# octree-nn/octfusion

Measured on AMD Instinct MI355X. Metric: denoising-steps/sec (depth-8 octree, batch 8), higher is better.
Workload: dtype f32 storage, fp16x3 products (fp16 hi + lo operand pairs = 22 significand bits, three fp16 MFMAs per product, fp32 accumulate)

## Files before the change

include/ofx.h:

```cpp
#ifndef OFX_H_
#define OFX_H_

#include <stddef.h>
#include <stdint.h>

#ifdef __cplusplus
extern "C" {
#endif

#define OFX_OK 0
#define OFX_EINVAL (-1)
#define OFX_ELAUNCH (-2)
#define OFX_ENODEV (-3)

#define OFX_ACT_NONE 0
#define OFX_ACT_SILU 1
#define OFX_ACT_GELU 2

#define OFX_MAX_DEPTH 16

int ofx_version(void);
const char* ofx_status_string(int status);
int ofx_device_check(void);
const char* ofx_build_hash(void);
// ... 72 lines not shown
int ofx_graphconv_bwd_weight(const float* x, int64_t ldx, int cin, int64_t n_nodes, const int32_t* nbr,
                             const int32_t* seg_ptr, const int32_t* col, const int32_t* nbr_ext,
                             const int32_t* multi_seg, int64_t n_multi, float* aux, const float* type_frac, int64_t ldt,
                             int nt_pad, const float* dy, int64_t ldy, int cout, float* dWp, int64_t Kp, void* ws,
                             size_t ws_bytes, void* stream);
int ofx_gn_backward(const float* x, int64_t ldx, const float* dy, int64_t ldy, int64_t n, int C,
                    const int32_t* batch_id, int batch_size, const float* count, int groups, float count_eps,
                    const float* mean, const float* rstd, const float* w, const float* bias, int act, double* sums,
                    float* coef, float* dx, int64_t lddx, float* dgamma, float* dbeta, void* stream);
int ofx_gemm_tn_f32(const float* P, int64_t ldp, const float* Q, int64_t ldq, int64_t rows, int64_t K, int64_t N,
                    float* out, void* ws, size_t ws_bytes, void* stream);
int ofx_table_reverse_count(const int32_t* nbr, int64_t n_out, int ndir, int64_t n_in, int32_t* rev_cnt, void* stream);
int ofx_table_reverse_fill(const int32_t* nbr, int64_t n_out, int ndir, int64_t n_in, const int32_t* rev_ptr,
                           int32_t* cursor, int32_t* rev_row, float* rev_w, void* stream);
int ofx_seg_primary_w(const int32_t* seg_ptr, const int32_t* col, const float* w, int64_t nseg, int32_t* nbr,
                      void* stream);
int ofx_seg_multi_flag_w(const int32_t* seg_ptr, const float* w, int64_t nseg, int32_t* flag, void* stream);
int ofx_seg_primary_ext_w(const int32_t* seg_ptr, const int32_t* col, const float* w, int64_t nseg, int64_t n_src,
                          const int32_t* rank, int32_t* nbr_ext, int32_t* multi_seg, void* stream);
int ofx_gridconv_bwd_data(const float* dy, int64_t ldy, int cout, int64_t n_out, int64_t n_in, const int32_t* nbr_rev,
                          const int32_t* rev_ptr, const int32_t* rev_row, const float* rev_w,
                          const int32_t* nbr_ext_rev, const int32_t* multi_seg, int64_t n_multi, float* aux,
                          const float* WpT, int cin, float* dx, int64_t ldx, void* ws, size_t ws_bytes, void* stream);
int ofx_gridconv_bwd_weight(const float* x, int64_t ldx, int cin, int64_t n_in, int64_t n_out, const int32_t* nbr27,
                            const int32_t* nbr27_ext, const float* zero_row, const float* dy, int64_t ldy, int cout,
                            float* dWp, void* ws, size_t ws_bytes, void* stream);
int ofx_adamw_step(float* param, const float* grad, float* exp_avg, float* exp_avg_sq, int64_t n, float lr,
                   float beta1, float beta2, float eps, float weight_decay, int step, void* stream);
int ofx_ema_update(float* ema, const float* param, int64_t n, float beta, void* stream);
typedef struct OfxAdamRow {
  float* param;
  const float* grad;
  float* exp_avg;
  float* exp_avg_sq;
  float* ema;
  int64_t n;
} OfxAdamRow;
int ofx_adamw_ema_multi(const OfxAdamRow* rows, int64_t n_rows, float lr, float beta1, float beta2, float eps,
                        float weight_decay, int step, float ema_beta, void* stream);
int ofx_adamw_ema_multi_chunk(void);
int ofx_adamw_ema_multi_rows(void);
int64_t ofx_mse_grad_partials(int64_t n);
int ofx_mse_grad(const float* y, const float* target, float* dy, double* partials, double* loss_out, int64_t n,
                 void* stream);
int ofx_mpu_eval(const ofx_tree_t* tree, int depth_start, int depth_end, const float* pts, int64_t n_pts,
                 const float* code, float* sdf, uint8_t* mask, void* stream);
int ofx_mpu_eval_grid(const ofx_tree_t* tree, int depth_start, int depth_end, const float* code, int size,
                      float step, float bbmin, int batch_index, int64_t head, int64_t count, float* sdf,
                      uint8_t* mask, void* stream);
int ofx_mpu_eval_grad(const ofx_tree_t* tree, int depth_start, int depth_end, const float* pts, int64_t n_pts,
                      const float* code, float* sdf, float* grad, uint8_t* mask, void* stream);
int ofx_mpu_backward(const ofx_tree_t* tree, int depth_start, int depth_end, const float* pts, int64_t n_pts,
                     const float* code, const float* dsdf, const float* dgrad, float* dcode, void* stream);
int ofx_octree_ce(const float* logits, int64_t ld, const int32_t* child, int64_t n, float dscale, double* sums,
                  float* dlogits, int64_t ldd, void* stream);
int ofx_sdf_reg_loss(const float* sdf, const float* grad, const float* sdf_gt, const float* grad_gt, int64_t n,
                     float w_sdf, float w_grad, double* sums, float* dsdf, float* dgrad, void* stream);
int ofx_kl_sample_fwd(const float* params, int64_t ld, const float* noise, int64_t n, int embed_dim, float* z,
                      double* kl_sum, void* stream);
int ofx_kl_sample_bwd(const float* params, int64_t ld, const float* noise, const float* dz, int64_t n,
                      int embed_dim, float kl_scale, float* dparams, int64_t ldp, void* stream);
int ofx_graph_multi_flag(const int32_t* seg_ptr, int64_t n_nodes, int32_t* flag, void* stream);
int ofx_graph_primary_ext(const int32_t* seg_ptr, const int32_t* col, int64_t n_nodes,
                          const int32_t* rank, int32_t* nbr_ext, int32_t* multi_seg, void* stream);
int ofx_graph_type_frac(const int32_t* seg_ptr, const int32_t* col, const uint8_t* node_type,
                        int64_t n_nodes, int nt, float* type_frac, int64_t ld, void* stream);

int ofx_set_precision(int mode);
int ofx_get_precision(void);
int64_t ofx_packed_floats(int64_t Kp, int64_t N);
int64_t ofx_packed_k(int64_t K);
int64_t ofx_graphconv_packed_k(int cin, int nt);
int ofx_pack_weights(const float* W, int64_t sk, int64_t sn, int64_t K, int64_t N,
                     int cin, int nt, float* Wp, int64_t Kp, void* stream);

int ofx_gemm_f32(const float* A, int64_t lda, const int32_t* a_rows, int64_t M, int64_t K,
                 const float* Wp, int64_t Kp, int64_t N, const float* bias,
                 const float* res, int64_t ldr, float* out, int64_t ldc,
                 const int32_t* out_rows, void* ws, size_t ws_bytes, void* stream);
int ofx_gemm_f32_planes(const float* A, int64_t lda, const int32_t* a_rows, int64_t M, int64_t K,
                        const float* Wp, int64_t Kp, int64_t N, const float* bias,
                        const float* res, int64_t ldr, float* out, int64_t ldc,
                        const int32_t* out_rows, void* ws, size_t ws_bytes, int out_mode, void* stream);

int ofx_graphconv_fwd(const float* x, int64_t ldx, int cin, int64_t n_nodes,
                      const int32_t* nbr, const int32_t* seg_ptr, const int32_t* col,
                      const int32_t* nbr_ext, const int32_t* multi_seg, int64_t n_multi, float* aux,
                      const float* type_frac, int64_t ldt, int nt_pad,
                      const float* Wp, int64_t Kp, int cout, const float* bias,
                      const float* emb, int64_t lde, const int32_t* batch_id,
                      const float* res, int64_t ldr, float* out, int64_t ldc,
                      double* stats , int64_t stats_ld,
                      void* ws, size_t ws_bytes, void* stream);

int ofx_graphconv_narrow_in(const float* x, int64_t ldx, int cin, int64_t n_nodes, const int32_t* seg_ptr,
                            const int32_t* col, const uint8_t* node_type, int nt, const float* W, int cout,
                            const float* bias, const int32_t* batch_id, float* out, int64_t ldc,
                            double* stats , int64_t stats_ld, void* ws, size_t ws_bytes, void* stream);
int ofx_graphconv_narrow_in_tab(const float* x, int64_t ldx, int cin, int64_t n_nodes, const int32_t* seg_ptr,
                                const int32_t* col, const int32_t* nbr_ext, const int32_t* multi_seg, int64_t n_multi,
                                void* aux, const uint8_t* node_type, int nt, const float* W, int cout, const float* bias,
                                const int32_t* batch_id, float* out, int64_t ldc, double* stats ,
                                int64_t stats_ld, void* ws, size_t ws_bytes, void* stream);
int ofx_narrow_out_pack(const float* W, int C, int nt, int cout, int pw, float* Wd, void* stream);
int ofx_narrow_out_type_term(const float* type_frac, int64_t ldt, int nt, int64_t n_nodes, const float* W, int C,
                             int cout, const float* bias, float* type_term, void* stream);
int ofx_graphconv_narrow_out(const float* P, int64_t ldp, int cout, int64_t n_nodes, const int32_t* seg_ptr,
                             const int32_t* col, const float* type_term , float* out, int64_t ldc,
                             void* stream);

int ofx_planes_split(const float* x, int64_t ldx, int64_t n, int C, int Cpad, int mode, void* out,
                     int64_t ldo_bytes, void* stream);
int ofx_planes_merge(const void* planes, int64_t ldp_bytes, int64_t n, int C, int mode, float* out, int64_t ldo,
                     void* stream);
int ofx_gn_apply_planes(const float* x, int64_t ldx, int64_t n, int C, const int32_t* batch_id, const float* mean,
                        const float* rstd, const double* sums, const float* count, int groups, float eps,
                        float count_eps, const float* w, const float* bias, int act, int mode, void* out,
                        int64_t ldo_bytes, const int32_t* seg_ptr, const int32_t* col, const int32_t* multi_seg,
                        int64_t n_multi, void* aux , const int32_t* aux_plan ,
                        int64_t aux_left, void* stream);
int ofx_gn_apply_planes_oct(const float* x, int64_t ldx, int64_t n, int C, const int32_t* batch_id, const float* mean,
                            const float* rstd, const double* sums, const float* count, int groups, float eps,
                            float count_eps, const float* w, const float* bias, int act, int mode, void* out,
                            int64_t ldo_bytes, int64_t n_multi, void* aux, const int32_t* oct_ptr,
                            const int32_t* oct_ent, int64_t n_own, int shift, const int32_t* left_head,
                            const int32_t* left_src, int64_t n_left, void* stream);
int ofx_gn_finalize_window(const double* sums, const float* count, int batch_size, int C, int groups, int c_lo,
                           int c_hi, float eps, float count_eps, float* mean, float* rstd, void* stream);
int ofx_gn_apply_planes_window(const float* x, int64_t ldx, int64_t n, int C, int c_lo, int c_hi,
                               const int32_t* batch_id, const float* mean, const float* rstd, const double* sums,
                               const float* count, int groups, float eps, float count_eps, const float* w,
                               const float* bias, int act, int mode, void* out, int64_t ldo_bytes,
                               const int32_t* seg_ptr, const int32_t* col, const int32_t* multi_seg, int64_t n_multi,
                               void* aux, const int32_t* aux_plan, int64_t aux_left, void* stream);
int ofx_gn_apply_planes_oct_window(const float* x, int64_t ldx, int64_t n, int C, int c_lo, int c_hi,
                                   const int32_t* batch_id, const float* mean, const float* rstd, const double* sums,
                                   const float* count, int groups, float eps, float count_eps, const float* w,
                                   const float* bias, int act, int mode, void* out, int64_t ldo_bytes, int64_t n_multi,
                                   void* aux, const int32_t* oct_ptr, const int32_t* oct_ent, int64_t n_own, int shift,
                                   const int32_t* left_head, const int32_t* left_src, int64_t n_left, void* stream);
int ofx_gn_apply_rows(void);
int64_t ofx_planes_packed_ktiles(int cin, int nt, int mode);
int64_t ofx_planes_packed_bytes(int cin, int nt, int cout, int mode);
int ofx_pack_weights_planes(const float* W, int64_t sk, int64_t sn, int cin, int nt, int cout, int mode, void* out,
                            void* stream);
int ofx_graphconv_fwd_planes(const void* xp, int64_t ldx_bytes, int cin, int64_t n_nodes, const int32_t* seg_ptr,
                             const int32_t* col, const int32_t* nbr_ext, const int32_t* multi_seg, int64_t n_multi,
                             void* aux, size_t aux_bytes, const void* tfp, int64_t ldt_bytes, int nt, const void* W2,
                             int cout, const float* bias, const float* emb, int64_t lde, const int32_t* batch_id,
                             const float* res, int64_t ldr, float* out, int64_t ldc, double* stats ,
                             int64_t stats_ld, void* ws, size_t ws_bytes, void* sync , size_t sync_bytes,
                             int mode, int aux_ready, void* stream);
int ofx_graphconv_fwd_planes_cus(const void* xp, int64_t ldx_bytes, int cin, int64_t n_nodes, const int32_t* seg_ptr,
                                 const int32_t* col, const int32_t* nbr_ext, const int32_t* multi_seg, int64_t n_multi,
                                 void* aux, size_t aux_bytes, const void* tfp, int64_t ldt_bytes, int nt,
                                 const void* W2, int cout, const float* bias, const float* emb, int64_t lde,
                                 const int32_t* batch_id, const float* res, int64_t ldr, float* out, int64_t ldc,
                                 double* stats , int64_t stats_ld, void* ws, size_t ws_bytes,
                                 void* sync , size_t sync_bytes, int mode, int aux_ready, int cus,
                                 void* stream);
int ofx_set_gconv_persistent(int on);
int64_t ofx_gemm_planes_packed_bytes(int K, int N, int mode);
int ofx_pack_gemm_planes(const float* W, int64_t sk, int64_t sn, int K, int N, int mode, void* out, void* stream);
int ofx_gemm_planes(const void* ap, int64_t lda_bytes, int64_t n_a, int64_t M, int K, const int32_t* row_tab,
                    const void* W2, int N, const float* bias, float* out, int64_t ldc, int out_mode, void* ws,
                    size_t ws_bytes, void* sync, size_t sync_bytes, int mode, void* stream);
int ofx_set_gconv_cus(int cus);
int ofx_gconv3_plan(int64_t n_rows, int cout, int nkt, int wm, int ni, int cus, int32_t* out, int64_t out_len);
int ofx_set_gconv2_tile(int wm);

int ofx_grid_conv_table(int mode, int depth_out, int batch_size, int32_t pad, int32_t* nbr27,
                        void* stream);
int64_t ofx_conv3d_packed_k(int cin);
int ofx_pack_conv3d(const float* W, int cin, int cout, float* Wp, void* stream);
int ofx_gridconv_fwd(const float* x, int64_t ldx, int cin, int64_t n_in, int64_t n_out,
                     const int32_t* nbr27 ,
                     const int32_t* nbr27_ext ,
                     const float* zero_row ,
                     const float* Wp, int cout, const float* bias, const float* emb, int64_t lde,
                     const int32_t* batch_id, const float* res, int64_t ldr, float* out,
                     int64_t ldc, void* ws, size_t ws_bytes, void* stream);
int ofx_gather_gemm_f32(const float* x, int64_t ldx, int cin, int ntap, int64_t n_src, int64_t n_out, const int32_t* tab,
                        const float* zero_row, const float* Wp, int64_t Kp, int cout, const float* bias,
                        const float* res, int64_t ldr, float* out, int64_t ldc, const int32_t* out_rows, void* ws,
                        size_t ws_bytes, int out_mode, void* stream);
int ofx_set_attention_split(int on);
int ofx_attention(const float* qkv, int64_t ldq, int batch_size, int T, int heads, int ch,
                  float* out, int64_t ldo, void* stream);

int ofx_attention_bwd(const float* qkv, int64_t ldq, const float* dout, int64_t ldo, int batch_size, int T, int heads,
                      int ch, float* rowstat, float* dqkv, int64_t ldd, void* stream);

int ofx_gather_mean(const float* x, int64_t ldx, int cin, int64_t n_nodes,
                    const int32_t* seg_ptr, const int32_t* col, float* col_data,
                    void* stream);

int ofx_gn_stats(const float* x, int64_t ldx, int64_t n, int C, const int32_t* batch_id,
                 int batch_size, double* sums, void* stream);
int ofx_gn_stats_acc(const float* x, int64_t ldx, int64_t n, int C, const int32_t* batch_id, int batch_size,
                     double* sums, void* stream);
int ofx_gn_finalize(const double* sums, const float* count, int batch_size, int C, int groups,
                    float eps, float count_eps, float* mean, float* rstd, void* stream);
int ofx_gn_apply(const float* x, int64_t ldx, int64_t n, int C, const int32_t* batch_id,
                 const float* mean , const float* rstd , const double* sums ,
                 const float* count, int groups, float eps, float count_eps, const float* w, const float* bias,
                 int act, float* out, int64_t ldo, void* stream);

int ofx_gn_fused_rows(const float* x, int64_t ldx, int rows_per_batch, int batch_size, int C, int groups, float eps,
                      float count_eps, const float* w, const float* bias, int act, float* out, int64_t ldo,
                      void* stream);

int ofx_set_gn_rows16(int on);

int ofx_rows_copy(const float* src, int64_t lds, const int32_t* smap, float* dst, int64_t ldd,
                  const int32_t* dmap, int64_t n, int C, void* stream);
int ofx_rows_copy_planes(const float* src, int64_t lds, const int32_t* smap, float* dst, int64_t ldd,
                         const int32_t* dmap, int64_t n, int C, int mode, void* stream);
int ofx_act(const float* x, float* y, int64_t n, int act, void* stream);
int ofx_timestep_embedding(const float* t, int batch_size, int dim, float max_period,
                           float* out, void* stream);
int ofx_learned_sinusoid(const float* t, const float* w, int batch_size, int half, float* out, void* stream);
int ofx_linear_small(const float* a, int64_t lda, int M, int K, const float* W, int64_t ldw, int N, const float* bias,
                     const float* res, int64_t ldr, int act_in, int act_out, float* out, int64_t ldo, void* stream);
int ofx_ddim_eps_update(float* x, const float* eps, const float* coef, float* x0_out, int64_t n,
                        void* stream);
int ofx_ddim_x0_update(float* x, const float* x0, const float* noise, const float* coef,
                       int64_t n, void* stream);

size_t ofx_mc_ws_bytes(int batch, int size);
int ofx_mc_count(const float* sdf, int batch, int size, float level, void* ws, int64_t* counts, void* stream);
int ofx_mc_emit(const float* sdf, int batch, int size, float level, float step, float bbmin, float scale, void* ws,
                const int64_t* vert_off, const int64_t* tri_off, float* verts, int32_t* faces, void* stream);
int ofx_mc_table_host(int8_t* tri_table, uint8_t* ntri);

size_t ofx_fieldmesh_classify_ws_bytes(int batch, int size);
size_t ofx_fieldmesh_ws_bytes(int64_t n_bricks);
int ofx_fieldmesh_classify(const ofx_tree_t* tree, int depth_end, int batch0, int batch, int size, float step,
                           float bbmin, int margin, void* cws, int64_t* counts, void* stream);
int ofx_fieldmesh_count(const ofx_tree_t* tree, int depth_start, int depth_end, const float* code, int batch0,
                        int batch, int size, float step, float bbmin, float level, const void* cws, int64_t n_bricks,
                        void* ws, int64_t* counts, void* stream);
int ofx_fieldmesh_emit(int batch, int size, float level, float step, float bbmin, float scale, const void* cws,
                       int64_t n_bricks, void* ws, const int64_t* vert_off, const int64_t* tri_off, float* verts,
                       int32_t* faces, void* stream);

size_t ofx_mesh_cc_ws_bytes(int64_t total_verts, int64_t total_faces, int batch);
int ofx_mesh_cc_label(const int32_t* faces, const int64_t* vert_off, const int64_t* tri_off, int batch,
                      int64_t total_verts, int64_t total_faces, int32_t* label, void* ws, int32_t* status,
                      void* stream);
int ofx_mesh_cc_table(const int32_t* faces, const int32_t* label, const int64_t* vert_off, const int64_t* tri_off,
                      int batch, int64_t total_verts, int64_t total_faces, int32_t* comp_of_vert, int32_t* comp_off,
                      void* ws, const int32_t* status, void* stream);
int ofx_mesh_cc_stats(const float* verts, const int32_t* faces, const int32_t* label, const int64_t* vert_off,
                      const int64_t* tri_off, int batch, int64_t total_verts, int64_t total_faces, int64_t n_comp,
                      int32_t* table, void* ws, const int32_t* status, void* stream);
int ofx_mesh_cc_select(const float* verts, const int32_t* faces, const int32_t* label, const int64_t* vert_off,
                       const int64_t* tri_off, int batch, int64_t total_verts, int64_t total_faces,
                       int32_t* winner_label, int64_t* keep_counts, void* ws, const int32_t* status, void* stream);
int ofx_mesh_cc_extract(const float* verts, const int32_t* faces, const int64_t* vert_off, const int64_t* tri_off,
                        int batch, int64_t total_verts, int64_t total_faces, const int64_t* new_vert_off,
                        const int64_t* new_tri_off, float* out_verts, int32_t* out_faces, void* ws,
                        const int32_t* status, void* stream);

int ofx_simplify_stages(void);
size_t ofx_simplify_ws_bytes(int64_t total_verts, int64_t total_faces, int batch);
int ofx_simplify_cluster(const float* verts, const int32_t* faces, const int64_t* vert_off, const int64_t* tri_off,
                         int batch, int64_t total_verts, int64_t total_faces, int cells, double cell_size, double reg,
                         int stages, int64_t* counts, void* ws, int32_t* status, void* stream);
// ... 103 lines not shown
```

octfusion_amd/_lib.py:

```python
import ctypes
import os

import torch

_HERE = os.path.dirname(os.path.abspath(__file__))
LIB_PATH = os.environ.get('OFX_LIB', os.path.join(_HERE, 'libofx.so'))

c_p = ctypes.c_void_p
c_i = ctypes.c_int
c_l = ctypes.c_int64
c_f = ctypes.c_float
c_d = ctypes.c_double
c_sz = ctypes.c_size_t
c_u64 = ctypes.c_uint64


class OfxTree(ctypes.Structure):
    _fields_ = [('depth', c_i), ('full_depth', c_i), ('batch_size', c_i),
                ('child_all', c_p), ('key_all', c_p), ('leafrank_all', c_p),
                ('nnum_host', c_p), ('nnum_nempty_host', c_p)]


class OfxAdamRow(ctypes.Structure):
    _fields_ = [('param', c_p), ('grad', c_p), ('exp_avg', c_p), ('exp_avg_sq', c_p), ('ema', c_p), ('n', c_l)]


_SIGS = {
    'ofx_version': (c_i, [], False),
    'ofx_status_string': (ctypes.c_char_p, [c_i], False),
    'ofx_device_check': (c_i, [], False),
    'ofx_build_hash': (ctypes.c_char_p, [], False),
    'ofx_probe_mfma_sustained': (c_i, [c_i, c_i, c_p, c_p, c_p], True),
    'ofx_scan_ws_bytes': (c_sz, [c_l], False),
    'ofx_scan_i32': (c_i, [c_p, c_p, c_l, c_p, c_p], True),
    'ofx_octree_full_layer': (c_i, [c_i, c_i, c_p, c_p, c_p], True),
    'ofx_octree_split': (c_i, [c_p, c_l, c_p, c_p, c_p, c_p], True),
    'ofx_octree_grow': (c_i, [c_p, c_p, c_l, c_p, c_p, c_p], True),
    'ofx_split_small_label0': (c_i, [c_p, c_i, c_i, c_p, c_p], True),
    'ofx_split_small_label1': (c_i, [c_p, c_i, c_i, c_p, c_p, c_p], True),
    'ofx_split_large_label0': (c_i, [c_p, c_l, c_p, c_p], True),
    'ofx_split_large_label1': (c_i, [c_p, c_l, c_p, c_p, c_p], True),
    'ofx_octree2voxel_cf': (c_i, [c_p, c_l, c_i, c_i, c_i, c_p, c_p], True),
    'ofx_voxel2octree_cf': (c_i, [c_p, c_i, c_i, c_i, c_p, c_l, c_p], True),
    'ofx_points_sort_ws_bytes': (c_sz, [c_l], False),
    'ofx_points_keys': (c_i, [c_p, c_l, c_p, c_i, c_l, c_i, c_p, c_p, c_p], True),
    'ofx_points_sort': (c_i, [c_p, c_p, c_l, c_p, c_p, c_p, c_sz, c_p], True),
    'ofx_octree_label_from_points': (c_i, [c_p, c_l, c_p, c_l, c_i, c_i, c_p, c_p], True),
    'ofx_octree_point_features': (c_i, [c_p, c_p, c_l, c_p, c_l, c_p, c_l, c_p, c_l, c_i, c_p, c_p, c_p, c_p], True),
    'ofx_tree_leafrank_ws_bytes': (c_sz, [c_l], False),
    'ofx_tree_leafrank': (c_i, [c_p, c_p, c_i, c_p, c_p, c_p], True),
    'ofx_graph_nodes': (c_i, [ctypes.POINTER(OfxTree), c_i, c_p, c_p, c_p, c_p, c_p], True),
    'ofx_graph_count': (c_i, [ctypes.POINTER(OfxTree), c_i, c_p, c_p], True),
    'ofx_graph_reverse_count': (c_i, [c_p, c_p, c_l, c_p, c_p], True),
    'ofx_graph_reverse_fill': (c_i, [c_p, c_p, c_l, c_p, c_p, c_p, c_p, c_p], True),
    'ofx_graph_primary_w': (c_i, [c_p, c_p, c_p, c_l, c_p, c_p], True),
    'ofx_graph_multi_flag_w': (c_i, [c_p, c_p, c_l, c_p, c_p], True),
    'ofx_graph_primary_ext_w': (c_i, [c_p, c_p, c_p, c_l, c_p, c_p, c_p, c_p], True),
    'ofx_graphconv_bwd_data': (c_i, [c_p, c_l, c_i, c_l, c_p, c_p, c_p, c_p, c_p, c_p, c_l, c_p, c_p, c_l, c_i, c_p,
                                     c_l, c_p, c_sz, c_p], True),
    'ofx_graphconv_bwd_weight': (c_i, [c_p, c_l, c_i, c_l, c_p, c_p, c_p, c_p, c_p, c_l, c_p, c_p, c_l, c_i, c_p, c_l,
                                       c_i, c_p, c_l, c_p, c_sz, c_p], True),
    'ofx_gn_backward': (c_i, [c_p, c_l, c_p, c_l, c_l, c_i, c_p, c_i, c_p, c_i, c_f, c_p, c_p, c_p, c_p, c_i, c_p, c_p,
                              c_p, c_l, c_p, c_p, c_p], True),
    'ofx_gemm_tn_f32': (c_i, [c_p, c_l, c_p, c_l, c_l, c_l, c_l, c_p, c_p, c_sz, c_p], True),
    'ofx_table_reverse_count': (c_i, [c_p, c_l, c_i, c_l, c_p, c_p], True),
    'ofx_table_reverse_fill': (c_i, [c_p, c_l, c_i, c_l, c_p, c_p, c_p, c_p, c_p], True),
    'ofx_seg_primary_w': (c_i, [c_p, c_p, c_p, c_l, c_p, c_p], True),
    'ofx_seg_multi_flag_w': (c_i, [c_p, c_p, c_l, c_p, c_p], True),
    'ofx_seg_primary_ext_w': (c_i, [c_p, c_p, c_p, c_l, c_l, c_p, c_p, c_p, c_p], True),
    'ofx_gridconv_bwd_data': (c_i, [c_p, c_l, c_i, c_l, c_l, c_p, c_p, c_p, c_p, c_p, c_p, c_l, c_p, c_p, c_i, c_p, c_l,
                                    c_p, c_sz, c_p], True),
    'ofx_gridconv_bwd_weight': (c_i, [c_p, c_l, c_i, c_l, c_l, c_p, c_p, c_p, c_p, c_l, c_i, c_p, c_p, c_sz, c_p], True),
    'ofx_attention_bwd': (c_i, [c_p, c_l, c_p, c_l, c_i, c_i, c_i, c_i, c_p, c_p, c_l, c_p], True),
    'ofx_adamw_step': (c_i, [c_p, c_p, c_p, c_p, c_l, c_f, c_f, c_f, c_f, c_f, c_i, c_p], True),
    'ofx_ema_update': (c_i, [c_p, c_p, c_l, c_f, c_p], True),
    'ofx_adamw_ema_multi': (c_i, [c_p, c_l, c_f, c_f, c_f, c_f, c_f, c_i, c_f, c_p], True),
    'ofx_adamw_ema_multi_chunk': (c_i, [], False),
    'ofx_adamw_ema_multi_rows': (c_i, [], False),
    'ofx_mse_grad_partials': (c_l, [c_l], False),
    'ofx_mse_grad': (c_i, [c_p, c_p, c_p, c_p, c_p, c_l, c_p], True),
    'ofx_gn_fused_rows': (c_i, [c_p, c_l, c_i, c_i, c_i, c_i, c_f, c_f, c_p, c_p, c_i, c_p, c_l, c_p], True),
    'ofx_set_gn_rows16': (c_i, [c_i], True),
    'ofx_mpu_eval': (c_i, [ctypes.POINTER(OfxTree), c_i, c_i, c_p, c_l, c_p, c_p, c_p, c_p], True),
    'ofx_mpu_eval_grid': (c_i, [ctypes.POINTER(OfxTree), c_i, c_i, c_p, c_i, c_f, c_f, c_i, c_l, c_l, c_p, c_p, c_p], True),
    'ofx_mpu_eval_grad': (c_i, [ctypes.POINTER(OfxTree), c_i, c_i, c_p, c_l, c_p, c_p, c_p, c_p, c_p], True),
    'ofx_mpu_backward': (c_i, [ctypes.POINTER(OfxTree), c_i, c_i, c_p, c_l, c_p, c_p, c_p, c_p, c_p], True),
    'ofx_octree_ce': (c_i, [c_p, c_l, c_p, c_l, c_f, c_p, c_p, c_l, c_p], True),
    'ofx_sdf_reg_loss': (c_i, [c_p, c_p, c_p, c_p, c_l, c_f, c_f, c_p, c_p, c_p, c_p], True),
    'ofx_kl_sample_fwd': (c_i, [c_p, c_l, c_p, c_l, c_i, c_p, c_p, c_p], True),
    'ofx_kl_sample_bwd': (c_i, [c_p, c_l, c_p, c_p, c_l, c_i, c_f, c_p, c_l, c_p], True),
    'ofx_graph_fill': (c_i, [ctypes.POINTER(OfxTree), c_i, c_p, c_p, c_p], True),
    'ofx_graph_expand': (c_i, [c_p, c_l, c_p, c_p, c_p, c_p, c_p], True),
    'ofx_graph_type_frac': (c_i, [c_p, c_p, c_p, c_l, c_i, c_p, c_l, c_p], True),
    'ofx_set_precision': (c_i, [c_i], True),
    'ofx_set_range_words': (c_i, [c_p], True),
    'ofx_get_precision': (c_i, [], False),
    'ofx_gn_apply_rows': (c_i, [], False),
    'ofx_set_attention_split': (c_i, [c_i], True),
    'ofx_gather_gemm_f32': (c_i, [c_p, c_l, c_i, c_i, c_l, c_l, c_p, c_p, c_p, c_l, c_i, c_p, c_p, c_l, c_p, c_l, c_p, c_p, c_sz, c_i, c_p], True),
    'ofx_graphconv_narrow_in_tab': (c_i, [c_p, c_l, c_i, c_l, c_p, c_p, c_p, c_p, c_l, c_p, c_p, c_i, c_p, c_i, c_p, c_p, c_p, c_l, c_p, c_l,
                                          c_p, c_sz, c_p], True),
    'ofx_graphconv_narrow_in': (c_i, [c_p, c_l, c_i, c_l, c_p, c_p, c_p, c_i, c_p, c_i, c_p, c_p, c_p, c_l, c_p, c_l, c_p, c_sz, c_p], True),
    'ofx_narrow_out_pack': (c_i, [c_p, c_i, c_i, c_i, c_i, c_p, c_p], True),
    'ofx_narrow_out_type_term': (c_i, [c_p, c_l, c_i, c_l, c_p, c_i, c_i, c_p, c_p, c_p], True),
    'ofx_graphconv_narrow_out': (c_i, [c_p, c_l, c_i, c_l, c_p, c_p, c_p, c_p, c_l, c_p], True),
    'ofx_packed_floats': (c_l, [c_l, c_l], False),
    'ofx_packed_k': (c_l, [c_l], False),
    'ofx_graphconv_packed_k': (c_l, [c_i, c_i], False),
    'ofx_pack_weights': (c_i, [c_p, c_l, c_l, c_l, c_l, c_i, c_i, c_p, c_l, c_p], True),
    'ofx_gemm_f32': (c_i, [c_p, c_l, c_p, c_l, c_l, c_p, c_l, c_l, c_p, c_p, c_l, c_p, c_l, c_p, c_p, c_sz, c_p], True),
    'ofx_gemm_f32_planes': (c_i, [c_p, c_l, c_p, c_l, c_l, c_p, c_l, c_l, c_p, c_p, c_l, c_p, c_l, c_p, c_p, c_sz, c_i, c_p], True),
    'ofx_graphconv_fwd': (c_i, [c_p, c_l, c_i, c_l, c_p, c_p, c_p, c_p, c_p, c_l, c_p, c_p, c_l, c_i, c_p, c_l,
                                c_i, c_p, c_p, c_l, c_p, c_p, c_l, c_p, c_l, c_p, c_l, c_p, c_sz, c_p], True),
    'ofx_planes_split': (c_i, [c_p, c_l, c_l, c_i, c_i, c_i, c_p, c_l, c_p], True),
    'ofx_planes_merge': (c_i, [c_p, c_l, c_l, c_i, c_i, c_p, c_l, c_p], True),
    'ofx_gn_apply_planes': (c_i, [c_p, c_l, c_l, c_i, c_p, c_p, c_p, c_p, c_p, c_i, c_f, c_f, c_p, c_p, c_i, c_i, c_p,
                                  c_l, c_p, c_p, c_p, c_l, c_p, c_p, c_l, c_p], True),
    'ofx_gn_apply_planes_oct': (c_i, [c_p, c_l, c_l, c_i, c_p, c_p, c_p, c_p, c_p, c_i, c_f, c_f, c_p, c_p, c_i, c_i, c_p,
                                      c_l, c_l, c_p, c_p, c_p, c_l, c_i, c_p, c_p, c_l, c_p], True),
    'ofx_planes_packed_ktiles': (c_l, [c_i, c_i, c_i], False),
    'ofx_planes_packed_bytes': (c_l, [c_i, c_i, c_i, c_i], False),
    'ofx_pack_weights_planes': (c_i, [c_p, c_l, c_l, c_i, c_i, c_i, c_i, c_p, c_p], True),
    'ofx_graphconv_fwd_planes': (c_i, [c_p, c_l, c_i, c_l, c_p, c_p, c_p, c_p, c_l, c_p, c_sz, c_p, c_l, c_i, c_p, c_i,
                                       c_p, c_p, c_l, c_p, c_p, c_l, c_p, c_l, c_p, c_l, c_p, c_sz, c_p, c_sz, c_i, c_i,
                                       c_p], True),
    'ofx_graphconv_fwd_planes_cus': (c_i, [c_p, c_l, c_i, c_l, c_p, c_p, c_p, c_p, c_l, c_p, c_sz, c_p, c_l, c_i, c_p,
                                           c_i, c_p, c_p, c_l, c_p, c_p, c_l, c_p, c_l, c_p, c_l, c_p, c_sz, c_p, c_sz,
                                           c_i, c_i, c_i, c_p], True),
    'ofx_gn_finalize_window': (c_i, [c_p, c_p, c_i, c_i, c_i, c_i, c_i, c_f, c_f, c_p, c_p, c_p], True),
    'ofx_gn_apply_planes_window': (c_i, [c_p, c_l, c_l, c_i, c_i, c_i, c_p, c_p, c_p, c_p, c_p, c_i, c_f, c_f, c_p, c_p,
                                         c_i, c_i, c_p, c_l, c_p, c_p, c_p, c_l, c_p, c_p, c_l, c_p], True),
    'ofx_gn_apply_planes_oct_window': (c_i, [c_p, c_l, c_l, c_i, c_i, c_i, c_p, c_p, c_p, c_p, c_p, c_i, c_f, c_f, c_p,
                                             c_p, c_i, c_i, c_p, c_l, c_l, c_p, c_p, c_p, c_l, c_i, c_p, c_p, c_l, c_p],
                                       True),
    'ofx_set_gconv_persistent': (c_i, [c_i], True),
    'ofx_set_gconv_cus': (c_i, [c_i], True),
    'ofx_gemm_planes_packed_bytes': (c_l, [c_i, c_i, c_i], False),
    'ofx_pack_gemm_planes': (c_i, [c_p, c_l, c_l, c_i, c_i, c_i, c_p, c_p], True),
    'ofx_gemm_planes': (c_i, [c_p, c_l, c_l, c_l, c_i, c_p, c_p, c_i, c_p, c_p, c_l, c_i, c_p, c_sz, c_p, c_sz, c_i, c_p], False),
    'ofx_gconv3_plan': (c_i, [c_l, c_i, c_i, c_i, c_i, c_i, c_p, c_l], False),
    'ofx_set_gconv2_tile': (c_i, [c_i], True),
    'ofx_graph_multi_flag': (c_i, [c_p, c_l, c_p, c_p], True),
    'ofx_graph_primary_ext': (c_i, [c_p, c_p, c_l, c_p, c_p, c_p, c_p], True),
    'ofx_graph_primary': (c_i, [c_p, c_p, c_l, c_p, c_p], True),
    'ofx_grid_conv_table': (c_i, [c_i, c_i, c_i, c_i, c_p, c_p], True),
    'ofx_conv3d_packed_k': (c_l, [c_i], False),
    'ofx_pack_conv3d': (c_i, [c_p, c_i, c_i, c_p, c_p], True),
    'ofx_gridconv_fwd': (c_i, [c_p, c_l, c_i, c_l, c_l, c_p, c_p, c_p, c_p, c_i, c_p, c_p, c_l, c_p, c_p, c_l, c_p,
                               c_l, c_p, c_sz, c_p], True),
    'ofx_attention': (c_i, [c_p, c_l, c_i, c_i, c_i, c_i, c_p, c_l, c_p], True),
    'ofx_gather_mean': (c_i, [c_p, c_l, c_i, c_l, c_p, c_p, c_p, c_p], True),
    'ofx_gn_stats': (c_i, [c_p, c_l, c_l, c_i, c_p, c_i, c_p, c_p], True),
    'ofx_gn_stats_acc': (c_i, [c_p, c_l, c_l, c_i, c_p, c_i, c_p, c_p], True),
    'ofx_gn_finalize': (c_i, [c_p, c_p, c_i, c_i, c_i, c_f, c_f, c_p, c_p, c_p], True),
    'ofx_gn_apply': (c_i, [c_p, c_l, c_l, c_i, c_p, c_p, c_p, c_p, c_p, c_i, c_f, c_f, c_p, c_p, c_i, c_p, c_l, c_p], True),
    'ofx_rows_copy': (c_i, [c_p, c_l, c_p, c_p, c_l, c_p, c_l, c_i, c_p], True),
    'ofx_rows_copy_planes': (c_i, [c_p, c_l, c_p, c_p, c_l, c_p, c_l, c_i, c_i, c_p], True),
    'ofx_act': (c_i, [c_p, c_p, c_l, c_i, c_p], True),
    'ofx_timestep_embedding': (c_i, [c_p, c_i, c_i, c_f, c_p, c_p], True),
    'ofx_learned_sinusoid': (c_i, [c_p, c_p, c_i, c_i, c_p, c_p], True),
    'ofx_linear_small': (c_i, [c_p, c_l, c_i, c_i, c_p, c_l, c_i, c_p, c_p, c_l, c_i, c_i, c_p, c_l, c_p], True),
    'ofx_ddim_eps_update': (c_i, [c_p, c_p, c_p, c_p, c_l, c_p], True),
    'ofx_ddim_x0_update': (c_i, [c_p, c_p, c_p, c_p, c_l, c_p], True),
    'ofx_mc_ws_bytes': (c_sz, [c_i, c_i], False),
    'ofx_mc_count': (c_i, [c_p, c_i, c_i, c_f, c_p, c_p, c_p], True),
    'ofx_mc_emit': (c_i, [c_p, c_i, c_i, c_f, c_f, c_f, c_f, c_p, c_p, c_p, c_p, c_p, c_p], True),
    'ofx_mc_table_host': (c_i, [c_p, c_p], True),
    'ofx_fieldmesh_classify_ws_bytes': (c_sz, [c_i, c_i], False),
    'ofx_fieldmesh_ws_bytes': (c_sz, [c_l], False),
    'ofx_fieldmesh_classify': (c_i, [ctypes.POINTER(OfxTree), c_i, c_i, c_i, c_i, c_f, c_f, c_i, c_p, c_p, c_p], True),
    'ofx_fieldmesh_count': (c_i, [ctypes.POINTER(OfxTree), c_i, c_i, c_p, c_i, c_i, c_i, c_f, c_f, c_f, c_p, c_l, c_p,
                                  c_p, c_p], True),
    'ofx_fieldmesh_emit': (c_i, [c_i, c_i, c_f, c_f, c_f, c_f, c_p, c_l, c_p, c_p, c_p, c_p, c_p, c_p], True),
    'ofx_mesh_cc_ws_bytes': (c_sz, [c_l, c_l, c_i], False),
    'ofx_mesh_cc_label': (c_i, [c_p, c_p, c_p, c_i, c_l, c_l, c_p, c_p, c_p, c_p], True),
    'ofx_mesh_cc_table': (c_i, [c_p, c_p, c_p, c_p, c_i, c_l, c_l, c_p, c_p, c_p, c_p, c_p], True),
    'ofx_mesh_cc_stats': (c_i, [c_p, c_p, c_p, c_p, c_p, c_i, c_l, c_l, c_l, c_p, c_p, c_p, c_p], True),
    'ofx_mesh_cc_select': (c_i, [c_p, c_p, c_p, c_p, c_p, c_i, c_l, c_l, c_p, c_p, c_p, c_p, c_p], True),
    'ofx_mesh_cc_extract': (c_i, [c_p, c_p, c_p, c_p, c_i, c_l, c_l, c_p, c_p, c_p, c_p, c_p, c_p, c_p], True),
    'ofx_simplify_stages': (c_i, [], False),
    'ofx_simplify_ws_bytes': (c_sz, [c_l, c_l, c_i], False),
    'ofx_simplify_cluster': (c_i, [c_p, c_p, c_p, c_p, c_i, c_l, c_l, c_i, c_d, c_d, c_i, c_p, c_p, c_p, c_p], True),
    'ofx_simplify_extract': (c_i, [c_p, c_p, c_p, c_i, c_l, c_l, c_p, c_p, c_p, c_p, c_p, c_p, c_p], True),
    'ofx_voxmesh_ws_bytes': (c_sz, [c_i, c_i, c_i], False),
    'ofx_voxmesh_mask_keys': (c_i, [c_p, c_l, c_i, c_i, c_i, c_p, c_p], True),
    'ofx_voxmesh_mask_dense': (c_i, [c_p, c_i, c_i, c_f, c_p, c_p], True),
    'ofx_voxmesh_count': (c_i, [c_i, c_i, c_i, c_p, c_p, c_p], True),
    'ofx_voxmesh_emit': (c_i, [c_i, c_i, c_i, c_p, c_p, c_p, c_p, c_p, c_p], True),
    'ofx_surface_sample_ws_bytes':(c_sz, [c_i, c_l], False),
    'ofx_surface_sample': (c_i, [c_p, c_p, c_p, c_p, c_i, c_l, c_i, c_u64, c_i, c_p, c_p, c_p], True),
    'ofx_surface_sample_oriented': (c_i, [c_p, c_p, c_p, c_p, c_i, c_l, c_i, c_u64, c_i, c_p, c_p, c_p, c_p], True),
    'ofx_nn_matrix': (c_i, [c_p, c_l, c_i, c_p, c_l, c_i, c_p, c_p], True),
    'ofx_emd_matrix': (c_i, [c_p, c_l, c_p, c_l, c_i, c_i, c_p, c_p], True),
    'ofx_metrics_hash': (c_u64, [c_u64, c_l, c_l, c_i], False),
    'ofx_nn_search_qpass': (c_i, [], False),
    'ofx_nn_search_tile': (c_i, [], False),
    'ofx_nn_search_splits': (c_i, [c_i, c_l, c_l], False),
    'ofx_nn_search_ws_bytes': (c_sz, [c_l], False),
    'ofx_nn_search': (c_i, [c_p, c_p, c_p, c_p, c_i, c_l, c_l, c_l, c_i, c_p, c_p, c_p, c_p], True),
    'ofx_knn_cells': (c_i, [c_l], False),
    'ofx_knn_ws_bytes': (c_sz, [c_i, c_l, c_l, c_i], False),
    'ofx_knn': (c_i, [c_p, c_p, c_i, c_l, c_l, c_i, c_i, c_p, c_p, c_p, c_p], True),
    'ofx_pca_normals': (c_i, [c_p, c_p, c_p, c_i, c_l, c_l, c_i, c_p, c_p, c_p, c_p], True),
    'ofx_orient_normals_ws_bytes': (c_sz, [c_i, c_l, c_i], False),
    'ofx_orient_normals': (c_i, [c_p, c_p, c_p, c_p, c_i, c_l, c_l, c_i, c_p, c_p, c_p, c_i, c_i, c_i, c_p, c_p, c_p,
                                 c_p, c_p], True),
    'ofx_sdf_sample_ws_bytes': (c_sz, [c_l, c_i], False),
    'ofx_sdf_sample_nodes': (c_i, [c_p, c_i, c_p, c_l, c_p, c_i, c_i, c_i, c_u64, c_l, c_p, c_f, c_p, c_p, c_p, c_p, c_p,
                                   c_p], True),
    'ofx_sdf_sample_occu': (c_i, [c_p, c_i, c_l, c_u64, c_l, c_p, c_f, c_p, c_p, c_p], True),
    'ofx_mesh_sdf_ws_bytes': (c_sz, [c_i, c_l, c_l, c_i], False),
# ... 124 lines not shown
```

octfusion_amd/csrc/ofx_gemm.hip:

```cpp
#include "ofx_gemm_common.h"

constexpr int BM = 128;
constexpr int BK = 32;
constexpr int A_LD = BK + 4;
constexpr int MODE_DENSE = 0;
constexpr int MODE_GATHER = 1;

struct TileCoords { int split, tm, tn; };
__device__ __forceinline__ TileCoords tile_coords(const GemmArgs& g) {
  const int ntile = g.ntm * g.ntn;
  int bid = ofx_xcd_swizzle(blockIdx.x, ntile * g.nsplit);
  const int split = bid / ntile;
  bid -= split * ntile;
  const int tm = bid / g.ntn;
  return {split, tm, bid - tm * g.ntn};
}

__device__ __forceinline__ void load_a_dense(const GemmArgs& g, int64_t m0, int64_t k0, float4 (&va)[4]) {
  const int c4 = threadIdx.x & 7, r0 = threadIdx.x >> 3;
  const int64_t k = k0 + c4 * 4;
  const bool vec = ((g.lda & 3) == 0) && (k + 3 < g.K) && ((((uintptr_t)g.A) & 15) == 0);
#pragma unroll
  for (int i = 0; i < 4; ++i) {
    const int64_t m = m0 + r0 + 32 * i;
    float4 v = f4zero();
    if (m < g.M) {
      const int64_t ar = g.a_rows ? (int64_t)g.a_rows[m] : m;
      const float* p = g.A + ar * g.lda + k;
      if (vec) {
        v = *reinterpret_cast<const float4*>(p);
      } else {
        if (k + 0 < g.K) v.x = p[0];
        if (k + 1 < g.K) v.y = p[1];
        if (k + 2 < g.K) v.z = p[2];
        if (k + 3 < g.K) v.w = p[3];
      }
    }
    va[i] = v;
  }
}

template <int BN>
__device__ __forceinline__ void load_b_tile(const GemmArgs& g, int64_t n0, int64_t k0, float4 (&vb)[BN / 32]) {
#pragma unroll
  for (int i = 0; i < BN / 32; ++i) {
    const int idx = threadIdx.x + 256 * i;
    const int kql = idx / BN, n = idx % BN;
    const int64_t nn = n0 + n;
    vb[i] = (nn < g.N) ? *reinterpret_cast<const float4*>(g.Wp + (((k0 >> 2) + kql) * g.N + nn) * 4) : f4zero();
  }
}

template <int WM, int WN, int MI, int NI>
__global__ void __launch_bounds__(256, 2) gemm_dense_generic_kernel(const GemmArgs g) {
  constexpr int BN = WN * NI * 32;
  static_assert(WM * MI * 32 == BM, "BM");
  extern __shared__ __attribute__((aligned(16))) float smem[];
  float* As = smem;
  float* Bs = smem + 2 * BM * A_LD;

  const TileCoords tc = tile_coords(g);
  const int split = tc.split;
  const int64_t m0 = (int64_t)tc.tm * BM, n0 = (int64_t)tc.tn * BN;

  const int lane = threadIdx.x & 63, wid = threadIdx.x >> 6;
  const int wm = wid / WN, wn = wid % WN;
  const int l31 = lane & 31, h = lane >> 5;
  const int c4 = threadIdx.x & 7, r0 = threadIdx.x >> 3;

  f32x16 acc[MI][NI];
#pragma unroll
  for (int i = 0; i < MI; ++i)
#pragma unroll
    for (int j = 0; j < NI; ++j)
#pragma unroll
      for (int r = 0; r < 16; ++r) acc[i][j][r] = 0.f;

  float4 va[4];
  float4 vb[BN / 32];
  const int nkt_all = (int)(g.Kp / BK);
  const int kt_begin = split * g.kt_per_split;
  const int kt_end = (kt_begin + g.kt_per_split < nkt_all) ? kt_begin + g.kt_per_split : nkt_all;

  auto store_tiles = [&](int buf) {
    float* a = As + buf * BM * A_LD;
#pragma unroll
    for (int i = 0; i < 4; ++i) *reinterpret_cast<float4*>(a + (r0 + 32 * i) * A_LD + c4 * 4) = va[i];
    float* b = Bs + buf * 8 * BN * 4;
#pragma unroll
    for (int i = 0; i < BN / 32; ++i) *reinterpret_cast<float4*>(b + (threadIdx.x + 256 * i) * 4) = vb[i];
  };

  if (kt_begin < kt_end) {
    load_a_dense(g, m0, (int64_t)kt_begin * BK, va);
    load_b_tile<BN>(g, n0, (int64_t)kt_begin * BK, vb);
    store_tiles(0);
  }
  __syncthreads();

  for (int kt = kt_begin; kt < kt_end; ++kt) {
    const int buf = (kt - kt_begin) & 1;
    if (kt + 1 < kt_end) {
      load_a_dense(g, m0, (int64_t)(kt + 1) * BK, va);
      load_b_tile<BN>(g, n0, (int64_t)(kt + 1) * BK, vb);
    }
    const float* a = As + buf * BM * A_LD + (wm * MI * 32 + l31) * A_LD + h * 16;
    const float* b = Bs + buf * 8 * BN * 4 + ((h * 4) * BN + wn * NI * 32 + l31) * 4;
#pragma unroll
    for (int q = 0; q < 4; ++q) {
      float4 fa[MI], fb[NI];
#pragma unroll
      for (int i = 0; i < MI; ++i) fa[i] = *reinterpret_cast<const float4*>(a + i * 32 * A_LD + q * 4);
#pragma unroll
      for (int j = 0; j < NI; ++j) fb[j] = *reinterpret_cast<const float4*>(b + (q * BN + j * 32) * 4);
#pragma unroll
      for (int i = 0; i < MI; ++i)
#pragma unroll
        for (int j = 0; j < NI; ++j) {
          acc[i][j] = __builtin_amdgcn_mfma_f32_32x32x2f32(fa[i].x, fb[j].x, acc[i][j], 0, 0, 0);
          acc[i][j] = __builtin_amdgcn_mfma_f32_32x32x2f32(fa[i].y, fb[j].y, acc[i][j], 0, 0, 0);
          acc[i][j] = __builtin_amdgcn_mfma_f32_32x32x2f32(fa[i].z, fb[j].z, acc[i][j], 0, 0, 0);
          acc[i][j] = __builtin_amdgcn_mfma_f32_32x32x2f32(fa[i].w, fb[j].w, acc[i][j], 0, 0, 0);
        }
    }
    if (kt + 1 < kt_end) store_tiles(buf ^ 1);
    __syncthreads();
  }

  epilogue_store<WM, WN, MI, NI>(g, acc, m0, n0, wm, wn, l31, h, split);
}


__device__ __forceinline__ uint64_t sgpr64(uint64_t v) {
  unsigned lo = __builtin_amdgcn_readfirstlane((unsigned)v), hi = __builtin_amdgcn_readfirstlane((unsigned)(v >> 32));
  asm volatile("" : "+s"(lo), "+s"(hi));
  return ((uint64_t)hi << 32) | lo;
}

typedef const float __attribute__((address_space(1)))* gfp;
typedef const int32_t __attribute__((address_space(1)))* gip;
__device__ __forceinline__ float4 ldg4(gfp p) {
  typedef float v4f __attribute__((ext_vector_type(4)));
  const v4f v = *reinterpret_cast<const v4f __attribute__((address_space(1)))*>(p);
  return make_float4(v.x, v.y, v.z, v.w);
}

template <int WM, int WN, int MI, int NI>
__device__ __forceinline__ void mfma_tile(const float* __restrict__ a, const float* __restrict__ b, f32x16 (&acc)[MI][NI]) {
  constexpr int BN = WN * NI * 32;
  float4 fa[2][MI], fb[2][NI];
#pragma unroll
  for (int i = 0; i < MI; ++i) fa[0][i] = *reinterpret_cast<const float4*>(a + i * 32 * A_LD);
#pragma unroll
  for (int j = 0; j < NI; ++j) fb[0][j] = *reinterpret_cast<const float4*>(b + (j * 32) * 4);
#pragma unroll
  for (int q = 0; q < 4; ++q) {
    const int cur = q & 1, nxt = cur ^ 1;
    if (q < 3) {
#pragma unroll
      for (int i = 0; i < MI; ++i) fa[nxt][i] = *reinterpret_cast<const float4*>(a + i * 32 * A_LD + (q + 1) * 4);
#pragma unroll
      for (int j = 0; j < NI; ++j) fb[nxt][j] = *reinterpret_cast<const float4*>(b + ((q + 1) * BN + j * 32) * 4);
    }
#pragma unroll
    for (int i = 0; i < MI; ++i)
#pragma unroll
      for (int j = 0; j < NI; ++j) {
        acc[i][j] = __builtin_amdgcn_mfma_f32_32x32x2f32(fa[cur][i].x, fb[cur][j].x, acc[i][j], 0, 0, 0);
        acc[i][j] = __builtin_amdgcn_mfma_f32_32x32x2f32(fa[cur][i].y, fb[cur][j].y, acc[i][j], 0, 0, 0);
        acc[i][j] = __builtin_amdgcn_mfma_f32_32x32x2f32(fa[cur][i].z, fb[cur][j].z, acc[i][j], 0, 0, 0);
        acc[i][j] = __builtin_amdgcn_mfma_f32_32x32x2f32(fa[cur][i].w, fb[cur][j].w, acc[i][j], 0, 0, 0);
      }
  }
}

__device__ __forceinline__ int64_t src_off(uint32_t id, int64_t ldx, int64_t n_src, int64_t aux_delta) {
  const int64_t i = (int64_t)(uint64_t)id;
  const int64_t mask = (n_src - 1 - i) >> 63;
  return i * ldx + (aux_delta & mask);
}

template <int MODE, int WM, int WN, int MI, int NI>
__global__ void __launch_bounds__(256, 2) gemm_fast_kernel(const GemmArgs g) {
  constexpr int BN = WN * NI * 32;
  constexpr int NB = BN / 32;
  static_assert(WM * MI * 32 == BM, "BM");
  extern __shared__ __attribute__((aligned(16))) float smem[];
  float* As = smem;
  float* Bs = smem + 2 * BM * A_LD;

  const TileCoords tc = tile_coords(g);
  const int split = tc.split;
  const int64_t m0 = (int64_t)tc.tm * BM, n0 = (int64_t)tc.tn * BN;

  const int lane = threadIdx.x & 63, wid = threadIdx.x >> 6;
  const int wm = wid / WN, wn = wid % WN;
  const int l31 = lane & 31, h = lane >> 5;
  const int c4 = threadIdx.x & 7, r0 = threadIdx.x >> 3;

  const gfp xp = (gfp)sgpr64((uint64_t)(MODE == MODE_DENSE ? g.A : g.x));
  const gfp tfp = (gfp)sgpr64((uint64_t)g.tf);
  const gfp wp = (gfp)sgpr64((uint64_t)g.Wp);
  const gip tab = (gip)sgpr64((uint64_t)g.nbr_ext);
  const int64_t ldx = (int64_t)sgpr64((uint64_t)(MODE == MODE_DENSE ? g.lda : g.ldx));
  const int64_t ldt = (int64_t)sgpr64((uint64_t)g.ldt), n_src = (int64_t)sgpr64((uint64_t)g.n_src);
  const int64_t Ncols = (int64_t)sgpr64((uint64_t)g.N);
  const int64_t aux_delta = (int64_t)sgpr64((uint64_t)((g.aux - g.x) - g.n_src * g.ldx));
  const int ndir = g.ndir;

  f32x16 acc[MI][NI];
#pragma unroll
  for (int i = 0; i < MI; ++i)
#pragma unroll
    for (int j = 0; j < NI; ++j)
#pragma unroll
      for (int r = 0; r < 16; ++r) acc[i][j][r] = 0.f;

  const int nkt_all = (int)(g.Kp / BK);
  const int kt_begin = split * g.kt_per_split;
  const int kt_end = (kt_begin + g.kt_per_split < nkt_all) ? kt_begin + g.kt_per_split : nkt_all;
  const int tpd = MODE == MODE_DENSE ? nkt_all : g.cin / BK;
  const int nkt_g = MODE == MODE_DENSE ? nkt_all : ndir * tpd;
  const int g_begin = kt_begin < nkt_g ? kt_begin : nkt_g;
  const int g_end = kt_end < nkt_g ? kt_end : nkt_g;
  const int t_begin = kt_begin > nkt_g ? kt_begin : nkt_g;

  int64_t m_0 = m0 + r0, m_1 = m_0 + 32, m_2 = m_0 + 64, m_3 = m_0 + 96;
  const int64_t mmax = g.M - 1;
  m_0 = m_0 < mmax ? m_0 : mmax; m_1 = m_1 < mmax ? m_1 : mmax;
  m_2 = m_2 < mmax ? m_2 : mmax; m_3 = m_3 < mmax ? m_3 : mmax;
  const gip t0 = tab + m_0 * ndir;
  const gip t1 = tab + m_1 * ndir;
  const gip t2 = tab + m_2 * ndir;
  const gip t3 = tab + m_3 * ndir;
  int64_t dr0 = m_0, dr1 = m_1, dr2 = m_2, dr3 = m_3;
  if (MODE == MODE_DENSE && g.a_rows) { dr0 = g.a_rows[m_0]; dr1 = g.a_rows[m_1]; dr2 = g.a_rows[m_2]; dr3 = g.a_rows[m_3]; }
  const gfp dp0 = xp + dr0 * ldx, dp1 = xp + dr1 * ldx, dp2 = xp + dr2 * ldx, dp3 = xp + dr3 * ldx;
  const int kclamp = (int)g.K - 4;
  int64_t bo0 = 0, bo1 = 0, bo2 = 0, bo3 = 0;
  {
    auto boff = [&](int i) {
      const int idx = threadIdx.x + 256 * i;
      int64_t nn = n0 + idx % BN;
      nn = nn < Ncols ? nn : Ncols - 1;
      return ((int64_t)(idx / BN) * Ncols + nn) * 4;
    };
    bo0 = boff(0);
    if (NB > 1) bo1 = boff(1);
    if (NB > 2) { bo2 = boff(2); bo3 = boff(3); }
  }
  float* const a_st = As + r0 * A_LD + c4 * 4;
  float* const b_st = Bs + threadIdx.x * 4;
  const float* const a_ld = As + (wm * MI * 32 + l31) * A_LD + h * 16;
  const float* const b_ld = Bs + ((h * 4) * BN + wn * NI * 32 + l31) * 4;

  float4 va0, va1, va2, va3, vb0, vb1, vb2, vb3;
  vb1 = vb2 = vb3 = f4zero();
  auto load_w = [&](gfp wk) {
    vb0 = ldg4(wk + bo0);
    if (NB > 1) vb1 = ldg4(wk + bo1);
    if (NB > 2) { vb2 = ldg4(wk + bo2); vb3 = ldg4(wk + bo3); }
  };
  auto stage = [&](float* as, float* bs) {
    *reinterpret_cast<float4*>(as) = va0;
    *reinterpret_cast<float4*>(as + 32 * A_LD) = va1;
    *reinterpret_cast<float4*>(as + 64 * A_LD) = va2;
    *reinterpret_cast<float4*>(as + 96 * A_LD) = va3;
    *reinterpret_cast<float4*>(bs) = vb0;
    if (NB > 1) *reinterpret_cast<float4*>(bs + 1024) = vb1;
    if (NB > 2) { *reinterpret_cast<float4*>(bs + 2048) = vb2; *reinterpret_cast<float4*>(bs + 3072) = vb3; }
  };

  if (g_begin < g_end) {
// ... 25 lines not shown
    for (int kt = g_begin; kt < g_end; ++kt) {
      const int buf = (kt - g_begin) & 1;
      const int ktn = kt + 1 < nkt_g ? kt + 1 : nkt_g - 1;
      const int dn = ktn % ndir;
      const int d2 = (kt + 2 < nkt_g ? kt + 2 : nkt_g - 1) % ndir;
      if (MODE == MODE_DENSE) {
        int cc = ktn * BK + c4 * 4;
        cc = cc < kclamp ? cc : kclamp;
        va0 = ldg4(dp0 + cc); va1 = ldg4(dp1 + cc); va2 = ldg4(dp2 + cc); va3 = ldg4(dp3 + cc);
      } else {
        ib0 = t0[d2]; ib1 = t1[d2]; ib2 = t2[d2]; ib3 = t3[d2];
        const int cc = (ktn / ndir) * BK + c4 * 4;
        va0 = ldg4(xp + src_off(ia0, ldx, n_src, aux_delta) + cc);
        va1 = ldg4(xp + src_off(ia1, ldx, n_src, aux_delta) + cc);
        va2 = ldg4(xp + src_off(ia2, ldx, n_src, aux_delta) + cc);
        va3 = ldg4(xp + src_off(ia3, ldx, n_src, aux_delta) + cc);
      }
      const int ktw = MODE == MODE_DENSE ? ktn : dn * tpd + ktn / ndir;
      load_w(wp + (int64_t)ktw * 8 * Ncols * 4);
      __builtin_amdgcn_sched_barrier(0);
      mfma_tile<WM, WN, MI, NI>(a_ld + buf * BM * A_LD, b_ld + buf * 8 * BN * 4, acc);
      __builtin_amdgcn_sched_barrier(0);
      stage(a_st + (buf ^ 1) * BM * A_LD, b_st + (buf ^ 1) * 8 * BN * 4);
      ia0 = ib0; ia1 = ib1; ia2 = ib2; ia3 = ib3;
      __syncthreads();
    }
  }

  for (int kt = t_begin; kt < kt_end; ++kt) {
    const int cc = (kt - nkt_g) * BK + c4 * 4;
    va0 = ldg4(tfp + m_0 * ldt + cc);
    va1 = ldg4(tfp + m_1 * ldt + cc);
    va2 = ldg4(tfp + m_2 * ldt + cc);
    va3 = ldg4(tfp + m_3 * ldt + cc);
    load_w(wp + (int64_t)kt * 8 * Ncols * 4);
    stage(a_st, b_st);
    __syncthreads();
    mfma_tile<WM, WN, MI, NI>(a_ld, b_ld, acc);
    __syncthreads();
  }

  epilogue_store<WM, WN, MI, NI>(g, acc, m0, n0, wm, wn, l31, h, split);
}


typedef __bf16 bf16x8_t __attribute__((ext_vector_type(8)));
typedef _Float16 f16x8h_t __attribute__((ext_vector_type(8)));
typedef unsigned u32x4h __attribute__((ext_vector_type(4)));

template <int H16>
__device__ __forceinline__ void split16x4(const float4& v, uint2& hi, uint2& lo) {
  if constexpr (H16 == 0) {
    hi.x = g2_pk_bf16(v.x, v.y);
    hi.y = g2_pk_bf16(v.z, v.w);
    const float hx = g2_bf16_lo(hi.x), hy = g2_bf16_hi(hi.x);
    const float hz = g2_bf16_lo(hi.y), hw = g2_bf16_hi(hi.y);
    lo.x = g2_pk_bf16(v.x - hx, v.y - hy);
    lo.y = g2_pk_bf16(v.z - hz, v.w - hw);
  } else {
    hi.x = g2_pk_f16(v.x, v.y);
    hi.y = g2_pk_f16(v.z, v.w);
    lo.x = g2_pk_f16(v.x - g2_f16_lo(hi.x), v.y - g2_f16_hi(hi.x));
    lo.y = g2_pk_f16(v.z - g2_f16_lo(hi.y), v.w - g2_f16_hi(hi.y));
  }
}
template <int H16>
__device__ __forceinline__ f32x16 mfma16(u32x4h a, u32x4h b, f32x16 c) {
  if constexpr (H16 == 0)
    return __builtin_amdgcn_mfma_f32_32x32x16_bf16(__builtin_bit_cast(bf16x8_t, a), __builtin_bit_cast(bf16x8_t, b), c, 0, 0, 0);
  else
    return __builtin_amdgcn_mfma_f32_32x32x16_f16(__builtin_bit_cast(f16x8h_t, a), __builtin_bit_cast(f16x8h_t, b), c, 0, 0, 0);
}

template <int MODE, int WM, int WN, int MI, int NI, int H16>
__global__ void __launch_bounds__(256, 2) gemm_pairs_x3_kernel(const GemmArgs g) {
  constexpr int BN = WN * NI * 32;
  constexpr int A_BYTES = BM * 80;
  constexpr int BUF_BYTES = 2 * A_BYTES;
  static_assert(WM * MI * 32 == BM, "BM");
  extern __shared__ __attribute__((aligned(16))) char smem8[];
  typedef unsigned u32x4 __attribute__((ext_vector_type(4)));
  typedef const u32x4 __attribute__((address_space(1)))* gqp;

  const TileCoords tc = tile_coords(g);
  const int split = tc.split;
  const int64_t m0 = (int64_t)tc.tm * BM, n0 = (int64_t)tc.tn * BN;

  const int lane = threadIdx.x & 63, wid = threadIdx.x >> 6;
  const int wm = wid / WN, wn = wid % WN;
  const int l31 = lane & 31, h = lane >> 5;
  const int c4 = threadIdx.x & 7;
  const int r0 = ((threadIdx.x >> 4) & 3) + 8 * (threadIdx.x >> 6) + 4 * ((threadIdx.x >> 3) & 1);

  const gfp xp = (gfp)sgpr64((uint64_t)(MODE == MODE_DENSE ? g.A : g.x));
  const gfp tfp = (gfp)sgpr64((uint64_t)g.tf);
  const gqp w16 = (gqp)sgpr64((uint64_t)g.W16);
  const gip tab = (gip)sgpr64((uint64_t)g.nbr_ext);
  const int64_t ldx = (int64_t)sgpr64((uint64_t)(MODE == MODE_DENSE ? g.lda : g.ldx));
  const int64_t ldt = (int64_t)sgpr64((uint64_t)g.ldt), n_src = (int64_t)sgpr64((uint64_t)g.n_src);
  const int64_t Ncols = (int64_t)sgpr64((uint64_t)g.N);
  const int64_t lo_off = (int64_t)sgpr64((uint64_t)(g.Kp / 8 * g.N));
  const int64_t aux_delta = (int64_t)sgpr64((uint64_t)((g.aux - g.x) - g.n_src * g.ldx));
  const int ndir = g.ndir;

  f32x16 acc[MI][NI];
#pragma unroll
  for (int i = 0; i < MI; ++i)
#pragma unroll
    for (int j = 0; j < NI; ++j)
#pragma unroll
      for (int r = 0; r < 16; ++r) acc[i][j][r] = 0.f;

  const int nkt_all = (int)(g.Kp / BK);
  const int kt_begin = split * g.kt_per_split;
  const int kt_end = (kt_begin + g.kt_per_split < nkt_all) ? kt_begin + g.kt_per_split : nkt_all;
  const int tpd = MODE == MODE_DENSE ? nkt_all : g.cin / BK;
  const int nkt_g = MODE == MODE_DENSE ? nkt_all : ndir * tpd;
  const int g_begin = kt_begin < nkt_g ? kt_begin : nkt_g;
  const int g_end = kt_end < nkt_g ? kt_end : nkt_g;
  const int t_begin = kt_begin > nkt_g ? kt_begin : nkt_g;

  int64_t m_0 = m0 + r0, m_1 = m_0 + 32, m_2 = m_0 + 64, m_3 = m_0 + 96;
  const int64_t mmax = g.M - 1;
  m_0 = m_0 < mmax ? m_0 : mmax; m_1 = m_1 < mmax ? m_1 : mmax;
  m_2 = m_2 < mmax ? m_2 : mmax; m_3 = m_3 < mmax ? m_3 : mmax;
  const gip t0 = tab + m_0 * ndir;
  const gip t1 = tab + m_1 * ndir;
  const gip t2 = tab + m_2 * ndir;
  const gip t3 = tab + m_3 * ndir;
  int64_t dr0 = m_0, dr1 = m_1, dr2 = m_2, dr3 = m_3;
  if (MODE == MODE_DENSE && g.a_rows) { dr0 = g.a_rows[m_0]; dr1 = g.a_rows[m_1]; dr2 = g.a_rows[m_2]; dr3 = g.a_rows[m_3]; }
  const gfp dp0 = xp + dr0 * ldx, dp1 = xp + dr1 * ldx, dp2 = xp + dr2 * ldx, dp3 = xp + dr3 * ldx;
  const int kclamp = (int)g.K - 4;

  int64_t bcol[NI];
#pragma unroll
  for (int j = 0; j < NI; ++j) {
    int64_t nn = n0 + (wn * NI + j) * 32 + l31;
    bcol[j] = (nn < Ncols ? nn : Ncols - 1) + (int64_t)h * Ncols;
  }
  char* const a_st = smem8 + (r0 * 80 + c4 * 8);
  const char* const a_ld = smem8 + ((wm * MI * 32 + l31) * 80 + 16 * h);

  struct BFrag { u32x4 h[2][NI], l[2][NI]; };
  struct RegSet { float4 a0, a1, a2, a3; };
  struct IdxSet { uint32_t i0, i1, i2, i3; };

  auto load_bfrag = [&](int ktw, BFrag& F) {
    const gqp wk = w16 + (int64_t)ktw * 4 * Ncols;
#pragma unroll
    for (int c = 0; c < 2; ++c)
#pragma unroll
      for (int j = 0; j < NI; ++j) {
        F.h[c][j] = wk[(int64_t)(2 * c) * Ncols + bcol[j]];
        F.l[c][j] = wk[lo_off + (int64_t)(2 * c) * Ncols + bcol[j]];
      }
  };
  auto store_a = [&](int buf, const RegSet& R) {
    char* a = a_st + buf * BUF_BYTES;
    uint2 hi, lo;
    split16x4<H16>(R.a0, hi, lo);
    *reinterpret_cast<uint2*>(a) = hi; *reinterpret_cast<uint2*>(a + A_BYTES) = lo;
    split16x4<H16>(R.a1, hi, lo);
    *reinterpret_cast<uint2*>(a + 32 * 80) = hi; *reinterpret_cast<uint2*>(a + 32 * 80 + A_BYTES) = lo;
    split16x4<H16>(R.a2, hi, lo);
    *reinterpret_cast<uint2*>(a + 64 * 80) = hi; *reinterpret_cast<uint2*>(a + 64 * 80 + A_BYTES) = lo;
// ... 208 lines not shown
                                                         const int32_t* __restrict__ multi_seg, int64_t V,
                                                         float* __restrict__ aux, int64_t ldaux,
                                                         const float* __restrict__ w) {
  const int c4n = cin >> 2;
  const int64_t total = (V + 1) * c4n;
  for (int64_t t = (int64_t)blockIdx.x * blockDim.x + threadIdx.x; t < total; t += (int64_t)gridDim.x * blockDim.x) {
    const int64_t v = t / c4n;
    const int c = (int)(t - v * c4n) * 4;
    float4 acc = f4zero();
    if (v > 0) {
      const int64_t s = multi_seg[v - 1];
      const int32_t a = seg_ptr[s], e = seg_ptr[s + 1];
      if (w) {
        for (int32_t p = a; p < e; ++p) {
          const float wp = w[p];
          const float4 xv = *reinterpret_cast<const float4*>(x + (int64_t)col[p] * ldx + c);
          acc.x += wp * xv.x; acc.y += wp * xv.y; acc.z += wp * xv.z; acc.w += wp * xv.w;
        }
      } else {
        for (int32_t p = a; p < e; ++p) f4add(acc, *reinterpret_cast<const float4*>(x + (int64_t)col[p] * ldx + c));
        const float inv = 1.f / (float)(e - a);
        acc.x *= inv; acc.y *= inv; acc.z *= inv; acc.w *= inv;
      }
    }
    *reinterpret_cast<float4*>(aux + v * ldaux + c) = acc;
  }
}

__global__ void __launch_bounds__(256) splitk_reduce_kernel(const GemmArgs g) {
  const int64_t total = g.M * g.N;
  for (int64_t t = (int64_t)blockIdx.x * blockDim.x + threadIdx.x; t < total; t += (int64_t)gridDim.x * blockDim.x) {
    const int64_t m = t / g.N, n = t - m * g.N;
    float v = 0.f;
    for (int s = 0; s < g.nsplit; ++s) v += g.ws[(int64_t)s * total + t];
    if (g.oscale_p) v *= *g.oscale_p;
    if (g.bias) v += g.bias[n];
    if (g.emb) v += g.emb[(int64_t)g.bid[m] * g.lde + n];
    if (g.res) v += g.res[m * g.ldr + n];
    int64_t om = m;
    if (g.out_rows) { om = g.out_rows[m]; if (om < 0) continue; }
    g.out[om * g.ldc + n] = v;
  }
}

__global__ void __launch_bounds__(256) splitk_reduce_v4_kernel(const GemmArgs g) {
  const int64_t n4 = g.N >> 2, total4 = g.M * n4, total = g.M * g.N;
  for (int64_t t = (int64_t)blockIdx.x * blockDim.x + threadIdx.x; t < total4; t += (int64_t)gridDim.x * blockDim.x) {
    const int64_t m = t / n4, n = (t - m * n4) * 4;
    const float* p = g.ws + m * g.N + n;
    float4 v = f4zero();
    int s = 0;
    for (; s + 7 < g.nsplit; s += 8) {
      float4 a[8];
#pragma unroll
      for (int u = 0; u < 8; ++u) a[u] = *reinterpret_cast<const float4*>(p + (int64_t)(s + u) * total);
#pragma unroll
      for (int u = 0; u < 8; ++u) f4add(v, a[u]);
    }
    for (; s + 3 < g.nsplit; s += 4) {
      const float4 a0 = *reinterpret_cast<const float4*>(p + (int64_t)s * total);
      const float4 a1 = *reinterpret_cast<const float4*>(p + (int64_t)(s + 1) * total);
      const float4 a2 = *reinterpret_cast<const float4*>(p + (int64_t)(s + 2) * total);
      const float4 a3 = *reinterpret_cast<const float4*>(p + (int64_t)(s + 3) * total);
      f4add(v, a0); f4add(v, a1); f4add(v, a2); f4add(v, a3);
    }
    for (; s < g.nsplit; ++s) f4add(v, *reinterpret_cast<const float4*>(p + (int64_t)s * total));
    if (g.oscale_p) { const float osc = *g.oscale_p; v.x *= osc; v.y *= osc; v.z *= osc; v.w *= osc; }
    if (g.bias) f4add(v, *reinterpret_cast<const float4*>(g.bias + n));
    if (g.emb) f4add(v, *reinterpret_cast<const float4*>(g.emb + (int64_t)g.bid[m] * g.lde + n));
    if (g.res) f4add(v, *reinterpret_cast<const float4*>(g.res + m * g.ldr + n));
    int64_t om = m;
    if (g.out_rows) { om = g.out_rows[m]; if (om < 0) continue; }
    if (g.out_planes) ofx_store_planes4(g.out, om * g.ldc + n, v, g.out_planes);
    else *reinterpret_cast<float4*>(g.out + om * g.ldc + n) = v;
  }
}

template <void (*KERNEL)(const GemmArgs), size_t LDS>
static int launch_tiled(GemmArgs& g, hipStream_t st) {
  static bool attr_set[OFX_MAX_DEVICES] = {};
  if (LDS > 64 * 1024 &&
      !ofx_raise_lds_limit(reinterpret_cast<const void*>(KERNEL), (int)LDS, attr_set))
    return OFX_ELAUNCH;
  KERNEL<<<g.ntm * g.ntn * g.nsplit, 256, LDS, st>>>(g);
  return OFX_OK;
}
template <int MODE, int WM, int WN, int MI, int NI>
static int launch_cfg(GemmArgs& g, int flavour, hipStream_t st) {
  constexpr size_t lds_f32 = (2 * BM * A_LD + 2 * 8 * (WN * NI * 32) * 4) * sizeof(float);
  constexpr size_t lds_16 = 2 * (2 * BM * 80);
  switch (flavour) {
    case 3: return launch_tiled<gemm_pairs_x3_kernel<MODE, WM, WN, MI, NI, 1>, lds_16>(g, st);
    case 2: return launch_tiled<gemm_pairs_x3_kernel<MODE, WM, WN, MI, NI, 0>, lds_16>(g, st);
    case 1: return launch_tiled<gemm_fast_kernel<MODE, WM, WN, MI, NI>, lds_f32>(g, st);
  }
  if constexpr (MODE == MODE_DENSE) return launch_tiled<gemm_dense_generic_kernel<WM, WN, MI, NI>, lds_f32>(g, st);
  return OFX_EINVAL;
}

__global__ void __launch_bounds__(256) stats_reduce_kernel(const float* __restrict__ part, int64_t nwr, int wr_rows,
                                                            int64_t N, const int32_t* __restrict__ bid,
                                                            double* __restrict__ stats, int64_t stats_ld) {
  __shared__ double red[3][64][2];
  const int c = threadIdx.x & 63, rg = threadIdx.x >> 6;
  const int64_t n = (int64_t)blockIdx.y * 64 + c;
  const int64_t w0 = (int64_t)blockIdx.x * 64;
  const int64_t nc = n < N ? n : N - 1;
  int b[16];
  float2 v[16];
#pragma unroll
  for (int i = 0; i < 16; ++i) {
    const int64_t w = w0 + rg * 16 + i;
    const int64_t wc = w < nwr ? w : nwr - 1;
    b[i] = bid[wc * wr_rows];
    v[i] = *reinterpret_cast<const float2*>(part + (wc * N + nc) * 2);
    if (w >= nwr) { b[i] = -1; v[i] = make_float2(0.f, 0.f); }
  }
  const int bfirst = bid[w0 * wr_rows];
  bool ok = true;
#pragma unroll
  for (int i = 0; i < 16; ++i) ok = ok && (b[i] == bfirst || b[i] < 0);
  const bool uni = __syncthreads_and(ok);
  auto flush = [&](int bb, double s, double q) {
    double* o = stats + ((int64_t)bb * stats_ld + n) * 2;
    unsafeAtomicAdd(o, s); unsafeAtomicAdd(o + 1, q);
  };
  if (uni) {
    double s = 0.0, q = 0.0;
#pragma unroll
    for (int i = 0; i < 16; ++i) { s += (double)v[i].x; q += (double)v[i].y; }
    if (rg > 0) { red[rg - 1][c][0] = s; red[rg - 1][c][1] = q; }
    __syncthreads();
    if (rg == 0 && n < N) {
#pragma unroll
      for (int r = 0; r < 3; ++r) { s += red[r][c][0]; q += red[r][c][1]; }
      flush(bfirst, s, q);
    }
  } else if (n < N) {
    double s = 0.0, q = 0.0;
    int sb = -1;
#pragma unroll
    for (int i = 0; i < 16; ++i) {
      if (b[i] < 0) continue;
      if (b[i] != sb) {
        if (sb >= 0) flush(sb, s, q);
        sb = b[i]; s = 0.0; q = 0.0;
      }
      s += (double)v[i].x; q += (double)v[i].y;
    }
    if (sb >= 0) flush(sb, s, q);
  }
}

int ofx_launch_stats_reduce(const GemmArgs& g, int wr_rows, hipStream_t st) {
  const int64_t nwr = ofx_cdiv(g.M, wr_rows);
  stats_reduce_kernel<<<dim3((unsigned)ofx_cdiv(nwr, 64), (unsigned)ofx_cdiv(g.N, 64)), 256, 0, st>>>(
      g.stats_part, nwr, wr_rows, g.N, g.bid, g.stats, g.stats_ld);
  OFX_LAUNCH_CHECK();
  return OFX_OK;
}

template <int MODE>
static int launch_gemm(GemmArgs& g, float* ws, size_t ws_bytes, hipStream_t st) {
  if (g.M <= 0 || g.N <= 0) return OFX_OK;
  if (MODE == MODE_GATHER && !(g.fast && g.nbr_ext && g.aux && (!g.out_rows || g.gather_out_rows))) return OFX_EINVAL;
  {
    auto al16 = [](const void* p) { return (reinterpret_cast<uintptr_t>(p) & 15) == 0; };
// ... 50 lines not shown
}

static inline int64_t pad32(int64_t v) { return (v + 31) / 32 * 32; }

extern "C" int64_t ofx_packed_k(int64_t K) { return pad32(K); }
extern "C" int64_t ofx_graphconv_packed_k(int cin, int nt) {
  return pad32(7 * (int64_t)cin) + (nt > 1 ? pad32(7 * (int64_t)nt) : 0);
}

__global__ void pack_weights_kernel(const float* __restrict__ W, int64_t sk, int64_t sn, int64_t K, int64_t N, int cin,
                                    int nt, float* __restrict__ Wp, int64_t Kp) {
  const int64_t total = (Kp / 4) * N;
  const int ntc = nt > 1 ? nt : 0;
  const int64_t Kf = (7 * (int64_t)cin + 31) / 32 * 32;
  for (int64_t t = (int64_t)blockIdx.x * blockDim.x + threadIdx.x; t < total; t += (int64_t)gridDim.x * blockDim.x) {
    const int64_t kq = t / N, n = t - kq * N;
    float v[4];
#pragma unroll
    for (int kk = 0; kk < 4; ++kk) {
      const int64_t k = kq * 4 + kk;
      int64_t src = -1;
      if (cin > 0) {
        if (k < 7 * (int64_t)cin) {
          const int64_t dir = k / cin, c = k - dir * cin;
          src = dir * (cin + ntc) + c;
        } else if (k >= Kf && ntc > 0 && k - Kf < 7 * (int64_t)ntc) {
          const int64_t kt = k - Kf, dir = kt / ntc, ty = kt - dir * ntc;
          src = dir * (cin + ntc) + cin + ty;
        }
      } else if (k < K) {
        src = k;
      }
      v[kk] = src >= 0 ? W[src * sk + n * sn] : 0.f;
    }
    *reinterpret_cast<float4*>(Wp + t * 4) = make_float4(v[0], v[1], v[2], v[3]);
  }
}

extern "C" int ofx_pack_weights(const float* W, int64_t sk, int64_t sn, int64_t K, int64_t N, int cin, int nt,
                                float* Wp, int64_t Kp, void* stream) {
  if (!W || !Wp || K < 1 || N < 1 || (Kp & 31) || cin < 0 || nt < 0) return OFX_EINVAL;
  if (cin > 0) {
    if (Kp != ofx_graphconv_packed_k(cin, nt) || K != 7 * (int64_t)(cin + (nt > 1 ? nt : 0))) return OFX_EINVAL;
  } else if (Kp != pad32(K)) {
    return OFX_EINVAL;
  }
  if (((uintptr_t)Wp & 15) != 0) return OFX_EINVAL;
  pack_weights_kernel<<<ofx_grid((Kp / 4) * N, 256), 256, 0, ofx_stream(stream)>>>(W, sk, sn, K, N, cin, nt, Wp, Kp);
  if (int rc = pack_bf16x3(Wp, Kp, N, ofx_stream(stream))) return rc;
  OFX_LAUNCH_CHECK();
  return OFX_OK;
}

__global__ void pack_conv3d_kernel(const float* __restrict__ W, int cin, int64_t N, float* __restrict__ Wp, int64_t Kp) {
  const int64_t total = (Kp / 4) * N;
  for (int64_t t = (int64_t)blockIdx.x * blockDim.x + threadIdx.x; t < total; t += (int64_t)gridDim.x * blockDim.x) {
    const int64_t kq = t / N, n = t - kq * N;
    float v[4];
#pragma unroll
    for (int kk = 0; kk < 4; ++kk) {
      const int64_t k = kq * 4 + kk;
      float w = 0.f;
      if (k < 27 * (int64_t)cin) {
        const int64_t tap = k / cin, c = k - tap * cin;
        w = W[(n * cin + c) * 27 + tap];
      }
      v[kk] = w;
    }
    *reinterpret_cast<float4*>(Wp + t * 4) = make_float4(v[0], v[1], v[2], v[3]);
  }
}

extern "C" int64_t ofx_conv3d_packed_k(int cin) { return pad32(27 * (int64_t)cin); }

extern "C" int ofx_pack_conv3d(const float* W, int cin, int cout, float* Wp, void* stream) {
  if (!W || !Wp || cin < 1 || cout < 1 || ((uintptr_t)Wp & 15)) return OFX_EINVAL;
  const int64_t Kp = ofx_conv3d_packed_k(cin);
  pack_conv3d_kernel<<<ofx_grid((Kp / 4) * cout, 256), 256, 0, ofx_stream(stream)>>>(W, cin, cout, Wp, Kp);
  if (int rc = pack_bf16x3(Wp, Kp, cout, ofx_stream(stream))) return rc;
  OFX_LAUNCH_CHECK();
  return OFX_OK;
}

extern "C" int ofx_gemm_f32_planes(const float* A, int64_t lda, const int32_t* a_rows, int64_t M, int64_t K,
                                   const float* Wp, int64_t Kp, int64_t N, const float* bias, const float* res, int64_t ldr,
                                   float* out, int64_t ldc, const int32_t* out_rows, void* ws, size_t ws_bytes,
                                   int out_mode, void* stream) {
  if (M == 0 && K >= 1 && N >= 1) return OFX_OK;
  if (M < 0 || K < 1 || N < 1 || !Wp || !out || (M > 0 && !A) || Kp != pad32(K) || lda < K || ldc < N ||
      (res && ldr < N) || ((uintptr_t)Wp & 15))
    return OFX_EINVAL;
  if (out_mode != 0 && out_mode != 2 && out_mode != 3) return OFX_EINVAL;
  if (out_mode && ((N & 3) || (ldc & 31) || ((uintptr_t)out & 127) || (res && ((ldr & 3) || ((uintptr_t)res & 15))) ||
                   (bias && ((uintptr_t)bias & 15)) || ((uintptr_t)ws & 15)))
    return OFX_EINVAL;
  GemmArgs g = {};
  g.A = A; g.lda = lda; g.a_rows = a_rows;
  g.M = M; g.K = K; g.Wp = Wp; g.Kp = Kp; g.N = N; g.bias = bias;
  g.res = res; g.ldr = ldr; g.out = out; g.ldc = ldc; g.out_rows = out_rows; g.out_planes = out_mode;
  return launch_gemm<MODE_DENSE>(g, (float*)ws, ws_bytes, ofx_stream(stream));
}
extern "C" int ofx_gemm_f32(const float* A, int64_t lda, const int32_t* a_rows, int64_t M, int64_t K, const float* Wp,
                            int64_t Kp, int64_t N, const float* bias, const float* res, int64_t ldr, float* out,
                            int64_t ldc, const int32_t* out_rows, void* ws, size_t ws_bytes, void* stream) {
  return ofx_gemm_f32_planes(A, lda, a_rows, M, K, Wp, Kp, N, bias, res, ldr, out, ldc, out_rows, ws, ws_bytes, 0, stream);
}

static int gather_common(GemmArgs& g, const float* x, int64_t ldx, int cin, int ndir, int64_t n_rows,
                         const int32_t* nbr, const int32_t* seg_ptr, const int32_t* col, const float* Wp, int64_t Kp,
                         int cout, const float* bias, const float* emb, int64_t lde, const int32_t* batch_id,
                         const float* res, int64_t ldr, float* out, int64_t ldc) {
  if (n_rows < 0 || cin < 1 || cout < 1 || !x || !nbr || !Wp || !out || ldx < cin || ldc < cout ||
      (res && ldr < cout) || (emb && (!batch_id || lde < cout)) || ((uintptr_t)Wp & 15))
    return OFX_EINVAL;
  g.x = x; g.ldx = ldx; g.cin = cin; g.ndir = ndir;
  g.fast = (cin % 32 == 0) && ((ldx & 3) == 0) && (((uintptr_t)x & 15) == 0);
  g.nbr = nbr; g.seg_ptr = seg_ptr; g.col = col;
  g.Kf = pad32((int64_t)ndir * cin);
  g.M = n_rows; g.K = Kp; g.Wp = Wp; g.Kp = Kp; g.N = cout; g.bias = bias;
  g.emb = emb; g.lde = lde; g.bid = batch_id; g.res = res; g.ldr = ldr; g.out = out; g.ldc = ldc;
  return OFX_OK;
}

__device__ __forceinline__ float gather_elem(const GemmArgs& g, int64_t row, int64_t k) {
  if (k >= (int64_t)g.ndir * g.cin) return 0.f;
  const int dir = (int)(k / g.cin), c = (int)(k - (int64_t)dir * g.cin);
  const int32_t nb = g.nbr[row * g.ndir + dir];
  if (nb >= 0) return g.x[(int64_t)nb * g.ldx + c];
  if (nb == -1) return 0.f;
  const int64_t s = row * g.ndir + dir;
  const int32_t a = g.seg_ptr[s], e = g.seg_ptr[s + 1];
  float acc = 0.f;
  if (g.edge_w) {
    for (int32_t p = a; p < e; ++p) acc += g.edge_w[p] * g.x[(int64_t)g.col[p] * g.ldx + c];
    return acc;
  }
  for (int32_t p = a; p < e; ++p) acc += g.x[(int64_t)g.col[p] * g.ldx + c];
  if (e - a > 1) acc /= (float)(e - a);
  return acc;
}
__global__ void __launch_bounds__(256) col_rows_kernel(const GemmArgs g, int64_t row0, int64_t rows,
                                                       float* __restrict__ colbuf) {
  const int64_t k4n = g.Kp >> 2, total = rows * k4n;
  for (int64_t t = (int64_t)blockIdx.x * blockDim.x + threadIdx.x; t < total; t += (int64_t)gridDim.x * blockDim.x) {
    const int64_t r = t / k4n, k = (t - r * k4n) * 4;
    const int64_t row = row0 + r;
    float v[4];
#pragma unroll
    for (int kk = 0; kk < 4; ++kk)
      v[kk] = (k + kk < g.Kf) ? gather_elem(g, row, k + kk) : g.tf[row * g.ldt + (k + kk - g.Kf)];
    *reinterpret_cast<float4*>(colbuf + t * 4) = make_float4(v[0], v[1], v[2], v[3]);
  }
}

static int launch_gather_via_col(const GemmArgs& g, float* ws, size_t ws_bytes, hipStream_t st) {
  if (!ws || (((uintptr_t)ws) & 15)) return OFX_EINVAL;
  size_t tail = ws_bytes / 8;
  if (tail > (size_t(16) << 20)) tail = size_t(16) << 20;
  tail &= ~size_t(15);
  const size_t row_bytes = (size_t)g.Kp * sizeof(float);
  int64_t chunk = (int64_t)((ws_bytes - tail) / row_bytes) / 128 * 128;
  if (chunk < 128) return OFX_EINVAL;
  float* tail_ws = reinterpret_cast<float*>(reinterpret_cast<char*>(ws) + (ws_bytes - tail));
  for (int64_t r0 = 0; r0 < g.M; r0 += chunk) {
    const int64_t rows = g.M - r0 < chunk ? g.M - r0 : chunk;
    col_rows_kernel<<<ofx_grid(rows * (g.Kp >> 2), 256), 256, 0, st>>>(g, r0, rows, ws);
    GemmArgs d = {};
    d.A = ws; d.lda = g.Kp; d.M = rows; d.K = g.Kp; d.Wp = g.Wp; d.Kp = g.Kp; d.N = g.N; d.bias = g.bias;
    d.emb = g.emb; d.lde = g.lde; d.bid = g.bid ? g.bid + r0 : nullptr;
    d.res = g.res ? g.res + r0 * g.ldr : nullptr; d.ldr = g.ldr;
    d.out = g.out + r0 * g.ldc; d.ldc = g.ldc;
    d.stats = g.stats; d.stats_ld = g.stats_ld;
    if (g.stats) { d.stats_part = tail_ws; d.stats_part_bytes = tail; }
    const int rc = launch_gemm<MODE_DENSE>(d, g.stats ? nullptr : tail_ws, tail, st);
    if (rc) return rc;
  }
  return OFX_OK;
}

extern "C" int ofx_graphconv_fwd(const float* x, int64_t ldx, int cin, int64_t n_nodes, const int32_t* nbr,
                                 const int32_t* seg_ptr, const int32_t* col, const int32_t* nbr_ext,
                                 const int32_t* multi_seg, int64_t n_multi, float* aux, const float* type_frac,
                                 int64_t ldt, int nt_pad, const float* Wp, int64_t Kp, int cout, const float* bias,
// ... 335 lines not shown
    a.rows_per_slice = ofx_cdiv(ofx_cdiv(n_out, slices), 32) * 32;
    slices = (int)ofx_cdiv(n_out, a.rows_per_slice);
    launch_tn<false>(a, dim3((unsigned)ofx_cdiv(Kp, 128), (unsigned)ofx_cdiv(cout, 128), (unsigned)slices), st);
    tn_reduce_kernel<<<ofx_grid(total, 256), 256, 0, st>>>(a.part, slices, total, dWp, 0);
    OFX_LAUNCH_CHECK();
    return OFX_OK;
  }
  if (!nbr27) return OFX_EINVAL;
  GemmArgs g = {};
  g.x = x; g.ldx = ldx; g.cin = cin; g.ndir = 27; g.nbr = nbr27; g.tf = x; g.ldt = ldx; g.Kf = Kp; g.Kp = Kp; g.M = n_out;
  int slices = (int)ofx_cdiv(512, tiles);
  if (slices > 64) slices = 64;
  const size_t part_bytes = ((size_t)slices * total * sizeof(float) + 255) & ~size_t(255);
  if (part_bytes >= ws_bytes) return OFX_EINVAL;
  int64_t chunk = (int64_t)((ws_bytes - part_bytes) / ((size_t)Kp * sizeof(float))) / 32 * 32;
  if (chunk < 32) return OFX_EINVAL;
  float* colbuf = reinterpret_cast<float*>(reinterpret_cast<char*>(ws) + part_bytes);
  a.P = colbuf; a.ldp = Kp;
  int first = 1;
  for (int64_t r0 = 0; r0 < n_out; r0 += chunk) {
    const int64_t rows = n_out - r0 < chunk ? n_out - r0 : chunk;
    col_rows_kernel<<<ofx_grid(rows * (Kp >> 2), 256), 256, 0, st>>>(g, r0, rows, colbuf);
    a.Q = dy + r0 * ldy; a.rows = rows; a.row0 = r0;
    a.rows_per_slice = ofx_cdiv(ofx_cdiv(rows, slices), 32) * 32;
    const int sl = (int)ofx_cdiv(rows, a.rows_per_slice);
    launch_tn<true>(a, dim3((unsigned)ofx_cdiv(Kp, 128), (unsigned)ofx_cdiv(cout, 128), (unsigned)sl), st);
    tn_reduce_kernel<<<ofx_grid(total, 256), 256, 0, st>>>(a.part, sl, total, dWp, first ? 0 : 1);
    first = 0;
  }
  OFX_LAUNCH_CHECK();
  return OFX_OK;
}

extern "C" int ofx_gemm_tn_f32(const float* P, int64_t ldp, const float* Q, int64_t ldq, int64_t rows, int64_t K,
                               int64_t N, float* out, void* ws, size_t ws_bytes, void* stream) {
  if (rows < 0 || K < 4 || N < 4 || (K & 3) || (N & 3) || !out || !ws || ldp < K || ldq < N || ((ldp | ldq) & 3) ||
      (rows > 0 && (!P || !Q)) || (((uintptr_t)P | (uintptr_t)Q | (uintptr_t)ws) & 15))
    return OFX_EINVAL;
  hipStream_t st = ofx_stream(stream);
  const int64_t total = K * N;
  if (rows == 0) {
    if (hipMemsetAsync(out, 0, (size_t)total * sizeof(float), st) != hipSuccess) return OFX_ELAUNCH;
    return OFX_OK;
  }
  const int tiles = (int)(ofx_cdiv(K, 128) * ofx_cdiv(N, 128));
  int slices = (int)ofx_cdiv(1024, tiles);
  if (slices > 256) slices = 256;
  if (slices > (int)ofx_cdiv(rows, 32)) slices = (int)ofx_cdiv(rows, 32);
  while (slices > 1 && (size_t)slices * total * sizeof(float) > ws_bytes) --slices;
  if ((size_t)slices * total * sizeof(float) > ws_bytes) return OFX_EINVAL;
  TnArgs a = {};
  a.P = P; a.ldp = ldp; a.Q = Q; a.ldq = ldq; a.Kp = K; a.N = N; a.Kf = K; a.rows = rows; a.row0 = 0;
  a.rows_per_slice = ofx_cdiv(ofx_cdiv(rows, slices), 32) * 32;
  slices = (int)ofx_cdiv(rows, a.rows_per_slice);
  a.part = (float*)ws;
  launch_tn<true>(a, dim3((unsigned)ofx_cdiv(K, 128), (unsigned)ofx_cdiv(N, 128), (unsigned)slices), st);
  tn_reduce_kernel<<<ofx_grid(total, 256), 256, 0, st>>>(a.part, slices, total, out, 0);
  OFX_LAUNCH_CHECK();
  return OFX_OK;
}

extern "C" int ofx_gridconv_fwd(const float* x, int64_t ldx, int cin, int64_t n_in, int64_t n_out,
                                const int32_t* nbr27, const int32_t* nbr27_ext, const float* zero_row,
                                const float* Wp, int cout,
                                const float* bias, const float* emb, int64_t lde, const int32_t* batch_id,
                                const float* res, int64_t ldr, float* out, int64_t ldc, void* ws, size_t ws_bytes,
                                void* stream) {
  if (n_out == 0 && cin >= 1 && cout >= 1) return OFX_OK;
  GemmArgs g = {};
  const int64_t Kp = ofx_conv3d_packed_k(cin);
  int rc = gather_common(g, x, ldx, cin, 27, n_out, nbr27 ? nbr27 : nbr27_ext, nullptr, nullptr, Wp, Kp, cout, bias,
                         emb, lde, batch_id, res, ldr, out, ldc);
  if (rc) return rc;
  if (n_in < 1) return OFX_EINVAL;
  if (g.fast && nbr27_ext && zero_row && (((uintptr_t)zero_row & 15) == 0)) {
    g.nbr_ext = nbr27_ext; g.aux = zero_row; g.ldaux = ldx; g.n_src = n_in;
    g.tf = x; g.ldt = ldx;
    return launch_gemm<MODE_GATHER>(g, (float*)ws, ws_bytes, ofx_stream(stream));
  }
  if (!nbr27) return OFX_EINVAL;
  return launch_gather_via_col(g, (float*)ws, ws_bytes, ofx_stream(stream));
}

extern "C" int ofx_gather_gemm_f32(const float* x, int64_t ldx, int cin, int ntap, int64_t n_src, int64_t n_out,
                                   const int32_t* tab, const float* zero_row, const float* Wp, int64_t Kp, int cout,
                                   const float* bias, const float* res, int64_t ldr, float* out, int64_t ldc,
                                   const int32_t* out_rows, void* ws, size_t ws_bytes, int out_mode, void* stream) {
  if (n_out == 0 && cin >= 1 && cout >= 1) return OFX_OK;
  if (ntap < 1 || ntap > 64 || n_src < 1 || !tab || !zero_row || ((uintptr_t)zero_row & 15) || (cin & 31) || (ldx & 3) ||
      ((uintptr_t)x & 15) || Kp != pad32((int64_t)ntap * cin))
    return OFX_EINVAL;
  if (out_mode != 0 && out_mode != 2 && out_mode != 3) return OFX_EINVAL;
  if (out_mode && ((cout & 3) || (ldc & 31) || ((uintptr_t)out & 127) || (res && ((ldr & 3) || ((uintptr_t)res & 15))) ||
                   (bias && ((uintptr_t)bias & 15)) || ((uintptr_t)ws & 15)))
    return OFX_EINVAL;
  GemmArgs g = {};
  int rc = gather_common(g, x, ldx, cin, ntap, n_out, tab, nullptr, nullptr, Wp, Kp, cout, bias, nullptr, 0, nullptr, res,
                         ldr, out, ldc);
  if (rc) return rc;
  if (!g.fast) return OFX_EINVAL;
  g.nbr_ext = tab; g.aux = zero_row; g.ldaux = ldx; g.n_src = n_src;
  g.tf = x; g.ldt = ldx;
  g.out_rows = out_rows; g.gather_out_rows = 1; g.out_planes = out_mode;
  return launch_gemm<MODE_GATHER>(g, (float*)ws, ws_bytes, ofx_stream(stream));
}

__global__ void __launch_bounds__(256) gather_mean_kernel(const float* __restrict__ x, int64_t ldx, int cin, int64_t nseg,
                                                          const int32_t* __restrict__ seg_ptr,
                                                          const int32_t* __restrict__ col, float* __restrict__ out) {
  const int c4n = cin >> 2;
  const int64_t total = nseg * c4n;
  for (int64_t t = (int64_t)blockIdx.x * blockDim.x + threadIdx.x; t < total; t += (int64_t)gridDim.x * blockDim.x) {
    const int64_t s = t / c4n;
    const int c = (int)(t - s * c4n) * 4;
    const int32_t a = seg_ptr[s], e = seg_ptr[s + 1];
    float4 acc = f4zero();
    for (int32_t p = a; p < e; ++p) f4add(acc, *reinterpret_cast<const float4*>(x + (int64_t)col[p] * ldx + c));
    if (e - a > 1) {
      const float inv = 1.f / (float)(e - a);
      acc.x *= inv; acc.y *= inv; acc.z *= inv; acc.w *= inv;
    }
    *reinterpret_cast<float4*>(out + s * cin + c) = acc;
  }
}
__global__ void __launch_bounds__(256) gather_mean_scalar_kernel(const float* __restrict__ x, int64_t ldx, int cin,
                                                                 int64_t nseg, const int32_t* __restrict__ seg_ptr,
                                                                 const int32_t* __restrict__ col,
                                                                 float* __restrict__ out) {
  const int64_t total = nseg * cin;
  for (int64_t t = (int64_t)blockIdx.x * blockDim.x + threadIdx.x; t < total; t += (int64_t)gridDim.x * blockDim.x) {
    const int64_t s = t / cin;
    const int c = (int)(t - s * cin);
    const int32_t a = seg_ptr[s], e = seg_ptr[s + 1];
    float acc = 0.f;
    for (int32_t p = a; p < e; ++p) acc += x[(int64_t)col[p] * ldx + c];
    if (e - a > 1) acc /= (float)(e - a);
    out[t] = acc;
  }
}

extern "C" int ofx_gather_mean(const float* x, int64_t ldx, int cin, int64_t n_nodes, const int32_t* seg_ptr,
                               const int32_t* col, float* col_data, void* stream) {
  if (!x || !seg_ptr || !col || !col_data || cin < 1 || ldx < cin || n_nodes < 0) return OFX_EINVAL;
  const int64_t nseg = n_nodes * 7;
  hipStream_t st = ofx_stream(stream);
  const bool vec = (cin % 4 == 0) && ((ldx & 3) == 0) && (((uintptr_t)x & 15) == 0) && (((uintptr_t)col_data & 15) == 0);
  if (vec)
    gather_mean_kernel<<<ofx_grid(nseg * (cin / 4), 256), 256, 0, st>>>(x, ldx, cin, nseg, seg_ptr, col, col_data);
  else
    gather_mean_scalar_kernel<<<ofx_grid(nseg * cin, 256), 256, 0, st>>>(x, ldx, cin, nseg, seg_ptr, col, col_data);
  OFX_LAUNCH_CHECK();
  return OFX_OK;
}
```

octfusion_amd/csrc/ofx_gemm_common.h:

```cpp
#pragma once
#include "ofx_common.h"

typedef float f32x16 __attribute__((ext_vector_type(16)));

struct GemmArgs {
  const float* A; int64_t lda; const int32_t* a_rows;
  const float* x; int64_t ldx; int cin; int ndir; int fast;
  const int32_t* nbr;
  const int32_t* seg_ptr; const int32_t* col;
  const float* edge_w;
  const float* tf; int64_t ldt; int64_t Kf;
  const int32_t* nbr_ext;
  const float* aux; int64_t ldaux; int64_t n_src;
  int64_t M, K;
  const float* Wp; int64_t Kp, N;
  const uint16_t* W16;
  const float* oscale_p;
  const float* bias;
  const float* emb; int64_t lde; const int32_t* bid;
  const float* res; int64_t ldr;
  float* out; int64_t ldc; const int32_t* out_rows;
  int gather_out_rows;
  int out_planes;
  double* stats; int64_t stats_ld;
  int ntm, ntn, nsplit, kt_per_split;
  float* ws;
  int vec4;
  float* stats_part; size_t stats_part_bytes;
};

static __global__ void __launch_bounds__(256) weight_absmax_kernel(const float* __restrict__ W, int64_t sk, int64_t sn, int64_t K,
                                                            int64_t N, unsigned* __restrict__ acc) {
  __shared__ float red[256];
  float m = 0.f;
  for (int64_t t = (int64_t)blockIdx.x * 256 + threadIdx.x; t < K * N; t += (int64_t)gridDim.x * 256) {
    const float a = fabsf(W[(t / N) * sk + (t % N) * sn]);
    if (a <= 3.0e38f) m = fmaxf(m, a);
  }
  red[threadIdx.x] = m;
  __syncthreads();
  for (int o = 128; o > 0; o >>= 1) {
    if ((int)threadIdx.x < o) red[threadIdx.x] = fmaxf(red[threadIdx.x], red[threadIdx.x + o]);
    __syncthreads();
  }
  if (threadIdx.x == 0) atomicMax(acc, __float_as_uint(red[0]));
}
static __global__ void weight_scale_finish_kernel(int fp16_operands, float* __restrict__ scale) {
  const float mx = __uint_as_float(reinterpret_cast<const unsigned*>(scale)[0]);
  float s = 1.f;
  if (fp16_operands && mx > 0.f) {
    int e;
    frexpf(mx, &e);
    int sh = 15 - e;
    sh = sh < -60 ? -60 : (sh > 60 ? 60 : sh);
    s = ldexpf(1.f, sh);
  }
  scale[0] = 1.f / s;
  scale[1] = s;
}
static inline int ofx_launch_weight_scale(const float* W, int64_t sk, int64_t sn, int64_t K, int64_t N, int fp16_operands,
                                          float* scale, hipStream_t st) {
  if (hipMemsetAsync(scale, 0, sizeof(float), st) != hipSuccess) return OFX_ELAUNCH;
  int64_t nb = (K * N + 256 * 16 - 1) / (256 * 16);
  nb = nb < 1 ? 1 : (nb > 1024 ? 1024 : nb);
  weight_absmax_kernel<<<(unsigned)nb, 256, 0, st>>>(W, sk, sn, K, N, reinterpret_cast<unsigned*>(scale));
  if (hipGetLastError() != hipSuccess) return OFX_ELAUNCH;
  weight_scale_finish_kernel<<<1, 1, 0, st>>>(fp16_operands, scale);
  if (hipGetLastError() != hipSuccess) return OFX_ELAUNCH;
  return OFX_OK;
}


__device__ __forceinline__ unsigned g2_pk_bf16(float a, float b) {
  unsigned r;
  asm("v_cvt_pk_bf16_f32 %0, %1, %2" : "=v"(r) : "v"(a), "v"(b));
  return r;
}
__device__ __forceinline__ unsigned g2_pk_f16(float a, float b) {
  const _Float16 x = (_Float16)a, y = (_Float16)b;
  return (unsigned)__builtin_bit_cast(unsigned short, x) | ((unsigned)__builtin_bit_cast(unsigned short, y) << 16);
}
__device__ __forceinline__ float g2_bf16_lo(unsigned p) { return __uint_as_float(p << 16); }
__device__ __forceinline__ float g2_bf16_hi(unsigned p) { return __uint_as_float(p & 0xffff0000u); }
__device__ __forceinline__ float g2_f16_lo(unsigned p) { return (float)__builtin_bit_cast(_Float16, (unsigned short)(p & 0xffffu)); }
__device__ __forceinline__ float g2_f16_hi(unsigned p) { return (float)__builtin_bit_cast(_Float16, (unsigned short)(p >> 16)); }
__device__ __forceinline__ float g2_sat16(float v) { return fminf(fmaxf(v, -65504.f), 65504.f); }
__device__ __forceinline__ void g2_split2(int mode, float a, float b, unsigned& hi, unsigned& lo) {
  if (mode == 3) {
    hi = g2_pk_f16(a, b);
    lo = g2_pk_f16(a - g2_f16_lo(hi), b - g2_f16_hi(hi));
  } else {
    hi = g2_pk_bf16(a, b);
    lo = g2_pk_bf16(a - g2_bf16_lo(hi), b - g2_bf16_hi(hi));
  }
}
__device__ __forceinline__ void g2_join2(int mode, unsigned hi, unsigned lo, float& a, float& b) {
  if (mode == 3) { a = g2_f16_lo(hi) + g2_f16_lo(lo); b = g2_f16_hi(hi) + g2_f16_hi(lo); }
  else { a = g2_bf16_lo(hi) + g2_bf16_lo(lo); b = g2_bf16_hi(hi) + g2_bf16_hi(lo); }
}
__host__ __device__ static inline bool g2_pairs(int mode) { return mode == 2 || mode == 3; }

__device__ __forceinline__ void ofx_store_planes4(float* base, int64_t f, const float4& v, int mode) {
  unsigned h0, h1, l0, l1;
  g2_split2(mode, v.x, v.y, h0, l0);
  g2_split2(mode, v.z, v.w, h1, l1);
  char* o = reinterpret_cast<char*>(base) + (f >> 5) * 128 + (f & 31) * 2;
  *reinterpret_cast<uint2*>(o) = make_uint2(h0, h1);
  *reinterpret_cast<uint2*>(o + 64) = make_uint2(l0, l1);
}

__device__ __forceinline__ int ofx_xcd_swizzle(int bid, int n) {
  const int q = n / 8, r = n % 8, xcd = bid % 8, j = bid / 8;
  return (xcd < r ? xcd * (q + 1) : r * (q + 1) + (xcd - r) * q) + j;
}

__device__ __forceinline__ float4 f4zero() { return make_float4(0.f, 0.f, 0.f, 0.f); }
__device__ __forceinline__ void f4add(float4& a, const float4& b) { a.x += b.x; a.y += b.y; a.z += b.z; a.w += b.w; }

template <int WM, int WN, int MI, int NI>
__device__ __forceinline__ void epilogue_store_scalar(const GemmArgs& g, f32x16 (&acc)[MI][NI], int64_t m0, int64_t n0,
                                                      int wm, int wn, int l31, int h, int split) {
#pragma unroll
  for (int j = 0; j < NI; ++j) {
    const int64_t n = n0 + (wn * NI + j) * 32 + l31;
    if (n >= g.N) continue;
    if (g.nsplit > 1) {
#pragma unroll
      for (int i = 0; i < MI; ++i)
#pragma unroll
        for (int r = 0; r < 16; ++r) {
          const int64_t m = m0 + (wm * MI + i) * 32 + (r & 3) + 8 * (r >> 2) + 4 * h;
          if (m < g.M) g.ws[((int64_t)split * g.M + m) * g.N + n] = acc[i][j][r];
        }
      continue;
    }
    const float bv = g.bias ? g.bias[n] : 0.f;
    const float osc = g.oscale_p ? *g.oscale_p : 1.f;
    int sb = -1;
    float ssum = 0.f, ssq = 0.f;
#pragma unroll
    for (int i = 0; i < MI; ++i) {
#pragma unroll
      for (int r = 0; r < 16; ++r) {
        const int64_t m = m0 + (wm * MI + i) * 32 + (r & 3) + 8 * (r >> 2) + 4 * h;
        if (m >= g.M) continue;
        float v = fmaf(acc[i][j][r], osc, bv);
        int b = 0;
        if (g.emb || g.stats) b = g.bid[m];
        if (g.emb) v += g.emb[(int64_t)b * g.lde + n];
        if (g.res) v += g.res[m * g.ldr + n];
        if (g.stats) {
          if (b != sb) {
            if (sb >= 0) {
              double* o = g.stats + ((int64_t)sb * g.stats_ld + n) * 2;
              unsafeAtomicAdd(o, (double)ssum);
              unsafeAtomicAdd(o + 1, (double)ssq);
            }
            sb = b; ssum = 0.f; ssq = 0.f;
          }
          ssum += v; ssq += v * v;
        }
        int64_t om = m;
        if (g.out_rows) { om = g.out_rows[m]; if (om < 0) continue; }
        g.out[om * g.ldc + n] = v;
      }
    }
    if (g.stats && sb >= 0) {
      double* o = g.stats + ((int64_t)sb * g.stats_ld + n) * 2;
      unsafeAtomicAdd(o, (double)ssum);
      unsafeAtomicAdd(o + 1, (double)ssq);
    }
  }
}

__device__ __forceinline__ float dpp_xor1(float v) {
  return __builtin_bit_cast(float, __builtin_amdgcn_mov_dpp(__builtin_bit_cast(int, v), 0xB1, 0xf, 0xf, true));
}
__device__ __forceinline__ float dpp_xor2(float v) {
  return __builtin_bit_cast(float, __builtin_amdgcn_mov_dpp(__builtin_bit_cast(int, v), 0x4E, 0xf, 0xf, true));
}
__device__ __forceinline__ void quad_transpose(float& v0, float& v1, float& v2, float& v3, bool q0, bool q1) {
  float r = dpp_xor1(q0 ? v0 : v1);
  if (q0) v0 = r; else v1 = r;
  r = dpp_xor1(q0 ? v2 : v3);
  if (q0) v2 = r; else v3 = r;
  r = dpp_xor2(q1 ? v0 : v2);
  if (q1) v0 = r; else v2 = r;
  r = dpp_xor2(q1 ? v1 : v3);
  if (q1) v1 = r; else v3 = r;
}

// ... 105 lines not shown
```

octfusion_amd/csrc/ofx_misc.hip:

```cpp
#include "ofx_gemm_common.h"
#include "ofx_optim.h"

extern "C" int ofx_version(void) { return 1; }

extern "C" const char* ofx_status_string(int status) {
  switch (status) {
    case OFX_OK: return "ok";
    case OFX_EINVAL: return "invalid argument";
    case OFX_ELAUNCH: return "HIP launch/runtime error";
    case OFX_ENODEV: return "no gfx950 device";
    default: return "unknown status";
  }
}

extern "C" int ofx_device_check(void) {
  int n = 0;
  if (hipGetDeviceCount(&n) != hipSuccess || n < 1) return OFX_ENODEV;
  int cur = 0;
  if (hipGetDevice(&cur) != hipSuccess) return OFX_ENODEV;
  hipDeviceProp_t p;
  if (hipGetDeviceProperties(&p, cur) != hipSuccess) return OFX_ENODEV;
  const char* a = p.gcnArchName;
  for (int i = 0; a[i]; ++i)
    if (a[i] == 'g' && a[i + 1] == 'f' && a[i + 2] == 'x' && a[i + 3] == '9' && a[i + 4] == '5' && a[i + 5] == '0')
      return OFX_OK;
  return OFX_ENODEV;
}

static uint32_t* g_range_words[OFX_MAX_DEVICES] = {};
extern "C" int ofx_set_range_words(uint32_t* words) {
  int dev = 0;
  if (hipGetDevice(&dev) != hipSuccess || dev < 0 || dev >= OFX_MAX_DEVICES) return OFX_ENODEV;
  if (words && ((uintptr_t)words & 3)) return OFX_EINVAL;
  g_range_words[dev] = words;
  return OFX_OK;
}
uint32_t* ofx_range_words() {
  int dev = 0;
  if (hipGetDevice(&dev) != hipSuccess || dev < 0 || dev >= OFX_MAX_DEVICES) return nullptr;
  return g_range_words[dev];
}

__global__ void __launch_bounds__(256) rows_copy_v4(const float* __restrict__ src, int64_t lds, const int32_t* __restrict__ smap,
                                                    float* __restrict__ dst, int64_t ldd, const int32_t* __restrict__ dmap,
                                                    int64_t n, int C4) {
  const int64_t total = n * C4;
  for (int64_t t = (int64_t)blockIdx.x * blockDim.x + threadIdx.x; t < total; t += (int64_t)gridDim.x * blockDim.x) {
    const int64_t i = t / C4;
    const int c = (int)(t - i * C4) * 4;
    const int64_t sr = smap ? (int64_t)smap[i] : i;
    const int64_t dr = dmap ? (int64_t)dmap[i] : i;
    if (sr < 0 || dr < 0) continue;
    *reinterpret_cast<float4*>(dst + dr * ldd + c) = *reinterpret_cast<const float4*>(src + sr * lds + c);
  }
}
__global__ void __launch_bounds__(256) rows_copy_s(const float* __restrict__ src, int64_t lds, const int32_t* __restrict__ smap,
                                                   float* __restrict__ dst, int64_t ldd, const int32_t* __restrict__ dmap,
                                                   int64_t n, int C) {
  const int64_t total = n * C;
  for (int64_t t = (int64_t)blockIdx.x * blockDim.x + threadIdx.x; t < total; t += (int64_t)gridDim.x * blockDim.x) {
    const int64_t i = t / C;
    const int c = (int)(t - i * C);
    const int64_t sr = smap ? (int64_t)smap[i] : i;
    const int64_t dr = dmap ? (int64_t)dmap[i] : i;
    if (sr < 0 || dr < 0) continue;
    dst[dr * ldd + c] = src[sr * lds + c];
  }
}

__global__ void __launch_bounds__(256) rows_copy_planes_v4(const float* __restrict__ src, int64_t lds,
                                                           const int32_t* __restrict__ smap, float* __restrict__ dst,
                                                           int64_t ldd, const int32_t* __restrict__ dmap, int64_t n, int C4,
                                                           int mode) {
  const int64_t total = n * C4;
  for (int64_t t = (int64_t)blockIdx.x * blockDim.x + threadIdx.x; t < total; t += (int64_t)gridDim.x * blockDim.x) {
    const int64_t i = t / C4;
    const int c = (int)(t - i * C4) * 4;
    const int64_t sr = smap ? (int64_t)smap[i] : i;
    const int64_t dr = dmap ? (int64_t)dmap[i] : i;
    if (sr < 0 || dr < 0) continue;
    ofx_store_planes4(dst, dr * ldd + c, *reinterpret_cast<const float4*>(src + sr * lds + c), mode);
  }
}
extern "C" int ofx_rows_copy_planes(const float* src, int64_t lds, const int32_t* smap, float* dst, int64_t ldd,
                                    const int32_t* dmap, int64_t n, int C, int mode, void* stream) {
  if (n < 0 || C < 32 || (C & 31) || (mode != 2 && mode != 3) || (n > 0 && (!src || !dst)) || lds < C || ldd < C ||
      (lds & 3) || (ldd & 31) || ((uintptr_t)src & 15) || ((uintptr_t)dst & 127))
    return OFX_EINVAL;
  if (n == 0) return OFX_OK;
  rows_copy_planes_v4<<<ofx_grid(n * (C / 4), 256), 256, 0, ofx_stream(stream)>>>(src, lds, smap, dst, ldd, dmap, n,
                                                                                  C / 4, mode);
  OFX_LAUNCH_CHECK();
  return OFX_OK;
}

extern "C" int ofx_rows_copy(const float* src, int64_t lds, const int32_t* smap, float* dst, int64_t ldd,
                             const int32_t* dmap, int64_t n, int C, void* stream) {
  if (n < 0 || C < 1 || (n > 0 && (!src || !dst)) || lds < C || ldd < C) return OFX_EINVAL;
  if (n == 0) return OFX_OK;
  hipStream_t st = ofx_stream(stream);
  const bool vec = (C % 4 == 0) && (lds % 4 == 0) && (ldd % 4 == 0) && (((uintptr_t)src & 15) == 0) &&
                   (((uintptr_t)dst & 15) == 0);
  if (vec)
    rows_copy_v4<<<ofx_grid(n * (C / 4), 256), 256, 0, st>>>(src, lds, smap, dst, ldd, dmap, n, C / 4);
  else
    rows_copy_s<<<ofx_grid(n * C, 256), 256, 0, st>>>(src, lds, smap, dst, ldd, dmap, n, C);
  OFX_LAUNCH_CHECK();
  return OFX_OK;
}

__global__ void timestep_embedding_kernel(const float* __restrict__ t, int B, int dim, float max_period,
                                          float* __restrict__ out) {
  const int half = dim / 2;
  for (int i = blockIdx.x * blockDim.x + threadIdx.x; i < B * dim; i += gridDim.x * blockDim.x) {
    const int b = i / dim, j = i - b * dim;
    float v = 0.f;
    if (j < 2 * half) {
      const int k = j < half ? j : j - half;
      const float f = expf(-logf(max_period) * (float)k / (float)half);
      const float a = t[b] * f;
      v = j < half ? cosf(a) : sinf(a);
    }
    out[i] = v;
  }
}
extern "C" int ofx_timestep_embedding(const float* t, int batch_size, int dim, float max_period, float* out,
                                      void* stream) {
  if (!t || !out || batch_size < 1 || dim < 2) return OFX_EINVAL;
  timestep_embedding_kernel<<<ofx_grid((int64_t)batch_size * dim, 256), 256, 0, ofx_stream(stream)>>>(
      t, batch_size, dim, max_period, out);
  OFX_LAUNCH_CHECK();
  return OFX_OK;
}

__global__ void learned_sinusoid_kernel(const float* __restrict__ t, const float* __restrict__ w, int B, int half,
                                        float* __restrict__ out) {
  const int dim = 2 * half + 1;
  for (int i = blockIdx.x * blockDim.x + threadIdx.x; i < B * dim; i += gridDim.x * blockDim.x) {
    const int b = i / dim, j = i - b * dim;
    const float x = t[b];
    float v = x;
    if (j > 0) {
      const float f = x * w[(j - 1) % half] * 2.f * 3.14159265358979323846f;
      v = j <= half ? sinf(f) : cosf(f);
    }
    out[i] = v;
  }
}
extern "C" int ofx_learned_sinusoid(const float* t, const float* w, int batch_size, int half, float* out, void* stream) {
  if (!t || !w || !out || batch_size < 1 || half < 1) return OFX_EINVAL;
  learned_sinusoid_kernel<<<ofx_grid((int64_t)batch_size * (2 * half + 1), 256), 256, 0, ofx_stream(stream)>>>(
      t, w, batch_size, half, out);
  OFX_LAUNCH_CHECK();
  return OFX_OK;
}

__device__ __forceinline__ float ls_act(float v, int act) {
  if (act == OFX_ACT_SILU) return v / (1.f + __expf(-v));
  if (act == OFX_ACT_GELU) return 0.5f * v * (1.f + erff(v * 0.70710678118654752440f));
  return v;
}
template <int MB>
__global__ void __launch_bounds__(256) linear_small_kernel(const float* __restrict__ a, int64_t lda, int M, int K,
                                                           const float* __restrict__ W, int64_t ldw, int N,
                                                           const float* __restrict__ bias, const float* __restrict__ res,
// ... 151 lines not shown
```

octfusion_amd/csrc/ofx_norm.hip:

```cpp
#include "ofx_planes.h"

constexpr int GN_ROWS_PER_BLOCK = 64;

static inline int64_t gn_stats_rows(int64_t n, int batch_size, int C = 128) {
  const int64_t chunks = (n + GN_ROWS_PER_BLOCK - 1) / GN_ROWS_PER_BLOCK;
  const int64_t bytes_per_batch = n * (int64_t)C * 4 / (batch_size > 0 ? batch_size : 1);
  int64_t per_batch = bytes_per_batch / (512 << 10);
  per_batch = per_batch < 8 ? 8 : (per_batch > 128 ? 128 : per_batch);
  int64_t cap = per_batch * (int64_t)batch_size;
  if (cap < 64) cap = 64;
  return chunks <= cap ? GN_ROWS_PER_BLOCK : GN_ROWS_PER_BLOCK * ((chunks + cap - 1) / cap);
}

__global__ void __launch_bounds__(256) gn_stats_kernel(const float* __restrict__ x, int64_t ldx, int64_t n, int C,
                                                       const int32_t* __restrict__ bid, double* __restrict__ sums,
                                                       int64_t rpb) {
  __shared__ int sb[256];
  __shared__ float sv[256][8];
  const int CT = C >> 2;
  const int RP = 256 / CT;
  const int cl = threadIdx.x % CT, rl = threadIdx.x / CT;
  int cb = -1;
  float s[4] = {0, 0, 0, 0}, q[4] = {0, 0, 0, 0};
  auto flush_direct = [&](int b, const float* ps, const float* pq) {
    if (b < 0) return;
    double* o = sums + ((int64_t)b * C + cl * 4) * 2;
#pragma unroll
    for (int k = 0; k < 4; ++k) {
      unsafeAtomicAdd(o + 2 * k, (double)ps[k]);
      unsafeAtomicAdd(o + 2 * k + 1, (double)pq[k]);
    }
  };
  auto accum = [&](int b, const float4& v) {
    if (b != cb) {
      flush_direct(cb, s, q);
      cb = b;
      s[0] = s[1] = s[2] = s[3] = 0.f;
      q[0] = q[1] = q[2] = q[3] = 0.f;
    }
    s[0] += v.x; s[1] += v.y; s[2] += v.z; s[3] += v.w;
    q[0] += v.x * v.x; q[1] += v.y * v.y; q[2] += v.z * v.z; q[3] += v.w * v.w;
  };
  const int64_t r_begin = (int64_t)blockIdx.x * rpb;
  const int64_t r_end = r_begin + rpb < n ? r_begin + rpb : n;
  if (rl < RP) {
    int64_t r = r_begin + rl;
    for (; r + 3 * (int64_t)RP < r_end; r += 4 * (int64_t)RP) {
      const int b0 = bid[r], b1 = bid[r + RP], b2 = bid[r + 2 * RP], b3 = bid[r + 3 * RP];
      const float4 v0 = *reinterpret_cast<const float4*>(x + r * ldx + cl * 4);
      const float4 v1 = *reinterpret_cast<const float4*>(x + (r + RP) * ldx + cl * 4);
      const float4 v2 = *reinterpret_cast<const float4*>(x + (r + 2 * RP) * ldx + cl * 4);
      const float4 v3 = *reinterpret_cast<const float4*>(x + (r + 3 * RP) * ldx + cl * 4);
      accum(b0, v0); accum(b1, v1); accum(b2, v2); accum(b3, v3);
    }
    for (; r < r_end; r += RP) accum(bid[r], *reinterpret_cast<const float4*>(x + r * ldx + cl * 4));
  }
  sb[threadIdx.x] = (rl < RP) ? cb : -1;
#pragma unroll
  for (int k = 0; k < 4; ++k) { sv[threadIdx.x][k] = s[k]; sv[threadIdx.x][4 + k] = q[k]; }
  __syncthreads();
  if (rl == 0) {
    double ds[4] = {0, 0, 0, 0}, dq[4] = {0, 0, 0, 0};
    for (int j = 0; j < RP; ++j) {
      const int t = j * CT + cl;
      const int b = sb[t];
      if (b < 0) continue;
      if (b == cb) {
#pragma unroll
        for (int k = 0; k < 4; ++k) { ds[k] += (double)sv[t][k]; dq[k] += (double)sv[t][4 + k]; }
      } else {
        flush_direct(b, &sv[t][0], &sv[t][4]);
      }
    }
    if (cb >= 0) {
      double* o = sums + ((int64_t)cb * C + cl * 4) * 2;
#pragma unroll
      for (int k = 0; k < 4; ++k) { unsafeAtomicAdd(o + 2 * k, ds[k]); unsafeAtomicAdd(o + 2 * k + 1, dq[k]); }
    }
  }
}

extern "C" int ofx_gn_stats(const float* x, int64_t ldx, int64_t n, int C, const int32_t* batch_id, int batch_size,
                            double* sums, void* stream) {
  if (!x || !batch_id || !sums || n < 0 || C < 4 || (C & 3) || C > 1024 || ldx < C || (ldx & 3) ||
      ((uintptr_t)x & 15) || batch_size < 1)
    return OFX_EINVAL;
  hipStream_t st = ofx_stream(stream);
  if (hipMemsetAsync(sums, 0, sizeof(double) * 2 * (size_t)batch_size * C, st) != hipSuccess) return OFX_ELAUNCH;
  if (n > 0) gn_stats_kernel<<<(int)ofx_cdiv(n, gn_stats_rows(n, batch_size, C)), 256, 0, st>>>(x, ldx, n, C, batch_id, sums,
                                                                                             gn_stats_rows(n, batch_size, C));
  OFX_LAUNCH_CHECK();
  return OFX_OK;
}

extern "C" int ofx_gn_stats_acc(const float* x, int64_t ldx, int64_t n, int C, const int32_t* batch_id, int batch_size,
                                double* sums, void* stream) {
  if (!x || !batch_id || !sums || n < 0 || C < 4 || (C & 3) || C > 1024 || ldx < C || (ldx & 3) ||
      ((uintptr_t)x & 15) || batch_size < 1)
    return OFX_EINVAL;
  if (n > 0) gn_stats_kernel<<<(int)ofx_cdiv(n, gn_stats_rows(n, batch_size, C)), 256, 0, ofx_stream(stream)>>>(
      x, ldx, n, C, batch_id, sums, gn_stats_rows(n, batch_size, C));
  OFX_LAUNCH_CHECK();
  return OFX_OK;
}

__global__ void gn_finalize_kernel(const double* __restrict__ sums, const float* __restrict__ count, int B, int C, int G,
                                   int ld, float eps, float count_eps, float* __restrict__ mean,
                                   float* __restrict__ rstd) {
  const int cpg = C / G;
  for (int t = blockIdx.x * blockDim.x + threadIdx.x; t < B * G; t += gridDim.x * blockDim.x) {
    const int b = t / G, g = t - b * G;
    double S = 0, SS = 0;
    for (int c = g * cpg; c < (g + 1) * cpg; ++c) {
      S += sums[((int64_t)b * ld + c) * 2];
      SS += sums[((int64_t)b * ld + c) * 2 + 1];
    }
    const float cnt = count[b] * (float)cpg;
    const float inv = 1.0f / (cnt + count_eps);
    const double m = S * (double)inv;
    const double ssd = SS - 2.0 * m * S + (double)cnt * m * m;
    const double var = (ssd > 0 ? ssd : 0) * (double)inv;
    const float rs = (float)(1.0 / sqrt(var + (double)eps));
    for (int c = g * cpg; c < (g + 1) * cpg; ++c) {
      mean[(int64_t)b * ld + c] = (float)m;
      rstd[(int64_t)b * ld + c] = rs;
    }
  }
}

extern "C" int ofx_gn_finalize(const double* sums, const float* count, int batch_size, int C, int groups, float eps,
                               float count_eps, float* mean, float* rstd, void* stream) {
  if (!sums || !count || !mean || !rstd || batch_size < 1 || C < 1 || groups < 1 || C % groups) return OFX_EINVAL;
  gn_finalize_kernel<<<ofx_grid((int64_t)batch_size * groups, 64), 64, 0, ofx_stream(stream)>>>(
      sums, count, batch_size, C, groups, C, eps, count_eps, mean, rstd);
  OFX_LAUNCH_CHECK();
  return OFX_OK;
}

static bool gn_window_ok(int C, int groups, int c_lo, int c_hi, int chunk = 32) {
  if (C < 1 || groups < 1 || C % groups) return false;
  const int cpg = C / groups;
  return c_lo >= 0 && c_lo < c_hi && c_hi <= C && c_lo % chunk == 0 && c_hi % chunk == 0 && c_lo % cpg == 0 &&
         c_hi % cpg == 0;
}

extern "C" int ofx_gn_finalize_window(const double* sums, const float* count, int batch_size, int C, int groups,
                                      int c_lo, int c_hi, float eps, float count_eps, float* mean, float* rstd,
                                      void* stream) {
  if (!sums || !count || !mean || !rstd || batch_size < 1 || !gn_window_ok(C, groups, c_lo, c_hi)) return OFX_EINVAL;
  const int gw = (c_hi - c_lo) / (C / groups);
  gn_finalize_kernel<<<ofx_grid((int64_t)batch_size * gw, 64), 64, 0, ofx_stream(stream)>>>(
      sums + 2 * (int64_t)c_lo, count, batch_size, c_hi - c_lo, gw, C, eps, count_eps, mean + c_lo, rstd + c_lo);
  OFX_LAUNCH_CHECK();
  return OFX_OK;
}

__device__ __forceinline__ float ofx_apply_act(float v, int act) {
  if (act == OFX_ACT_SILU) return v / (1.f + __expf(-v));
  if (act == OFX_ACT_GELU) return 0.5f * v * (1.f + erff(v * 0.70710678118654752440f));
  return v;
}

constexpr int GN_APPLY_ROWS = 64;
struct GnFin { const double* sums; const float* count; int G; float eps, count_eps; int ld; };
__device__ __forceinline__ void gn_group_stats(const GnFin& f, int b, int g, int C, float& mean, float& rstd) {
  const int cpg = C / f.G;
  double S = 0, SS = 0;
  for (int c = g * cpg; c < (g + 1) * cpg; ++c) {
    S += f.sums[((int64_t)b * f.ld + c) * 2];
    SS += f.sums[((int64_t)b * f.ld + c) * 2 + 1];
  }
  const float cnt = f.count[b] * (float)cpg;
  const float inv = 1.0f / (cnt + f.count_eps);
  const double m = S * (double)inv;
  const double ssd = SS - 2.0 * m * S + (double)cnt * m * m;
  const double var = (ssd > 0 ? ssd : 0) * (double)inv;
  mean = (float)m;
  rstd = (float)(1.0 / sqrt(var + (double)f.eps));
}
template <int MODE, bool FIN>
__global__ void __launch_bounds__(256) gn_apply_kernel(const float* __restrict__ x, int64_t ldx, int64_t n, int C,
                                                       const int32_t* __restrict__ bid, const float* __restrict__ mean,
                                                       const float* __restrict__ rstd, const GnFin fin,
                                                       const float* __restrict__ w,
                                                       const float* __restrict__ bias, int act, char* __restrict__ out,
                                                       int64_t ldo, int64_t aux_blocks,
                                                       const int32_t* __restrict__ seg_ptr,
                                                       const int32_t* __restrict__ col,
                                                       const int32_t* __restrict__ multi_seg, int64_t n_multi,
                                                       char* __restrict__ aux, const int32_t* __restrict__ aux_plan) {
  const int CT = C >> 2, RP = 256 / CT;
  const int cl = threadIdx.x % CT, rl = threadIdx.x / CT;
  __shared__ float fin_ms[FIN ? 2 * 2 * 1024 : 1];
  constexpr int AUX_LDS = 64;
  __shared__ int aux_v[AUX_LDS], aux_n[AUX_LDS], aux_src[AUX_LDS][4];
  int fb0 = -1, fb1 = -1;
  const int64_t gT = gridDim.x;
  const int64_t a_before = aux_blocks > 0 ? ((int64_t)blockIdx.x * aux_blocks) / gT : 0;
  const bool is_aux = aux_blocks > 0 && (((int64_t)blockIdx.x + 1) * aux_blocks) / gT > a_before;
  const int64_t aux_id = a_before, main_id = (int64_t)blockIdx.x - a_before;
  const int64_t r_begin0 = main_id * GN_APPLY_ROWS;
  const int64_t r_end0 = r_begin0 + GN_APPLY_ROWS < n ? r_begin0 + GN_APPLY_ROWS : n;
  const bool pre = FIN && !is_aux && rl < RP && r_begin0 + rl + 3 * (int64_t)RP < r_end0;
  float4 pv0, pv1, pv2, pv3;
  int pb0 = 0, pb1 = 0, pb2 = 0, pb3 = 0;
  if (pre) {
    const int64_t r = r_begin0 + rl;
    const int c_ = cl * 4;
    pb0 = bid[r]; pb1 = bid[r + RP]; pb2 = bid[r + 2 * RP]; pb3 = bid[r + 3 * RP];
    pv0 = *reinterpret_cast<const float4*>(x + r * ldx + c_);
    pv1 = *reinterpret_cast<const float4*>(x + (r + RP) * ldx + c_);
    pv2 = *reinterpret_cast<const float4*>(x + (r + 2 * RP) * ldx + c_);
    pv3 = *reinterpret_cast<const float4*>(x + (r + 3 * RP) * ldx + c_);
  }
  if (FIN) {
    if (!is_aux) {
      fb0 = bid[r_begin0];
      fb1 = bid[r_end0 - 1];
    } else {
      const int64_t v0 = aux_id * RP, v1e = v0 + RP - 1 < n_multi ? v0 + RP - 1 : n_multi;
      if (n_multi > 0) {
        fb0 = bid[multi_seg[(v0 > 0 ? v0 : 1) - 1] / 7];
        fb1 = bid[multi_seg[(v1e > 0 ? v1e : 1) - 1] / 7];
      }
    }
    const int cpg = C / fin.G;
    for (int t = threadIdx.x; t < 2 * fin.G && fb0 >= 0; t += 256) {
      const int slot = t / fin.G, g = t - slot * fin.G;
      if (slot == 1 && fb1 == fb0) continue;
      float mm, rr;
      gn_group_stats(fin, slot ? fb1 : fb0, g, C, mm, rr);
      for (int cc = g * cpg; cc < (g + 1) * cpg; ++cc) {
        fin_ms[(slot * 2 + 0) * 1024 + cc] = mm;
        fin_ms[(slot * 2 + 1) * 1024 + cc] = rr;
      }
// ... 883 lines not shown
```

octfusion_amd/modules.py:

```python
import math

import torch
import torch.nn as nn

from . import ops


def _gn_groups(channels, group=32):
    if channels <= 32:
        group = channels // 4
    elif channels % group != 0:
        group = 30
    assert channels % group == 0
    return group


class GraphConv(nn.Module):

    def __init__(self, in_channels, out_channels, n_edge_type=7, avg_degree=7, n_node_type=0,
                 use_bias=False):
        super().__init__()
        assert n_edge_type == 7, 'the dual octree graph has 7 edge types'
        self.in_channels = in_channels
        self.out_channels = out_channels
# ... 125 lines not shown
            delattr(data, ops.STATS_ATTR)
        return y

    def extra_repr(self):
        return 'in_channels={}, group={}, nempty={}'.format(self.in_channels, self.group, self.nempty)


class _Linear(nn.Module):

    def __init__(self, cin, cout, bias=True):
        super().__init__()
        self.in_features, self.out_features = cin, cout
        self.weight = nn.Parameter(torch.empty(cout, cin))
        self.bias = nn.Parameter(torch.empty(cout)) if bias else None
        nn.init.kaiming_uniform_(self.weight, a=math.sqrt(5))
        if bias:
            bound = 1 / math.sqrt(cin)
            nn.init.uniform_(self.bias, -bound, bound)
        self._pw = ops.PackedWeight()

    @torch.no_grad()
    def forward(self, x, res=None, out=None, act_in=None, act_out=None):
        if ops.LINEAR_SMALL and x.dim() == 2 and x.shape[0] <= 16:
            return ops.linear_small(x, self.weight, self.bias, res, act_in, act_out, out)
        if act_in is not None:
            x = ops.act(x, act_in)
        y = ops.gemm(x, self._pw.get(self.weight, 'nk'), self.bias, res, out)
        return ops.act(y, act_out, out=y) if act_out is not None else y


class Conv1x1(nn.Module):

    def __init__(self, channel_in, channel_out, use_bias=False):
        super().__init__()
        self.linear = _Linear(channel_in, channel_out, use_bias)

    def forward(self, x, res=None):
        return self.linear(x, res)


class Conv1x1Gn(nn.Module):

    def __init__(self, channel_in, channel_out):
        super().__init__()
        self.conv = Conv1x1(channel_in, channel_out, use_bias=False)
        self.gn = DualOctreeGroupNorm(channel_out)

    def forward(self, x, doctree, depth):
        return self.gn(self.conv(x), doctree, depth)


class Conv1x1GnGelu(nn.Module):

    def __init__(self, channel_in, channel_out):
        super().__init__()
        self.conv = Conv1x1(channel_in, channel_out, use_bias=False)
        self.gn = DualOctreeGroupNorm(channel_out)
        self.gelu = nn.GELU()

    def forward(self, x, doctree, depth):
        return self.gn(self.conv(x), doctree, depth, act='gelu')


class Conv1x1GnGeluSequential(Conv1x1GnGelu):

    def forward(self, data):
        x, doctree, depth = data
        return super().forward(x, doctree, depth)


class Downsample(nn.Module):

    def __init__(self, channels):
        super().__init__()
        self.channels = channels
        self.weights = nn.Parameter(torch.empty(channels, channels, 8))
        nn.init.xavier_uniform_(self.weights)
        self._pw = ops.PackedWeight()

    def packed(self):
        return self._pw.get(self.weights.view(self.channels, self.channels * 8), 'nk')

    @torch.no_grad()
    def forward(self, x, out=None, out_rows=None, out_planes=0):
        C = self.channels
        if (x.stride(0) != C and x.stride(1) == 1 and C % 32 == 0 and x.shape[0] % 8 == 0 and x.shape[0]
                and x.stride(0) % 4 == 0 and x.data_ptr() % 16 == 0 and ops.zero_row(x.device).numel() >= C):
            n = x.shape[0] // 8
            tab = _child_table(n, x.device)
            return ops.gather_gemm(x, tab, 8, self.packed(), n, out=out, out_rows=out_rows, out_planes=out_planes)
        return ops.gemm(x.reshape(-1, C * 8), self.packed(), out=out, out_rows=out_rows, out_planes=out_planes)

    def extra_repr(self):
        return 'channels={}'.format(self.channels)


_CHILD_TABLES = {}


def _child_table(n, device):
    key = (n, device.type, device.index)
    t = _CHILD_TABLES.get(key)
    if t is None:
        if len(_CHILD_TABLES) > 64:
            _CHILD_TABLES.clear()
        t = _CHILD_TABLES[key] = torch.arange(8 * n + 8, dtype=torch.int32, device=device)
    return t


class Upsample(nn.Module):

    def __init__(self, channels):
        super().__init__()
        self.channels = channels
        self.weights = nn.Parameter(torch.empty(channels, channels, 8))
        nn.init.xavier_uniform_(self.weights)
        self._pw = ops.PackedWeight()
        self._pgp = ops.PackedGemmPlanes()

    def packed(self):
        return self._pw.get(self.weights.view(self.channels, self.channels * 8), 'kn')

    @torch.no_grad()
    def forward(self, x, a_rows=None, out=None, out_planes=0):
        C = self.channels
        mode = ops.planes_mode()
        if (ops.GEMM_PLANES and out is not None and a_rows is not None and ops.planes_pairs(mode) and out_planes == mode
                and C % 32 == 0 and C >= 256 and a_rows.numel() >= 256):
            M = a_rows.numel()
            xa = torch.empty(M, C, dtype=torch.float32, device=x.device)
            ops.rows_copy(x, xa, M, smap=a_rows, planes=mode)
            setattr(xa, ops.PLANES_ATTR, mode)
            if ops.gemm_planes(xa, self._pgp.get(self.weights.view(C, C * 8), mode), out, out_planes):
                return out
        y = ops.gemm(x, self.packed(), out=out, a_rows=a_rows, out_planes=out_planes)
        return y.view(-1, self.channels) if out is None else out

    def extra_repr(self):
        return 'channels={}'.format(self.channels)


def _planes_dst(n, C, planes, device):
    out = torch.empty(n, C, dtype=torch.float32, device=device)
    ok = ops.planes_pairs(planes) and C % 32 == 0 and out.data_ptr() % 128 == 0
    return out, (planes if ok else 0)


def pool_nodes(x, doctree, d, downsample, planes=0):
    copy_src, gemm_rows, n_out = doctree.pool_maps(d)
    C = x.shape[1]
    numd = int(doctree.nnum[d])
    out, planes = _planes_dst(n_out, C, planes, x.device)
    ops.rows_copy(x, out, n_out, smap=copy_src, planes=planes)
    downsample(x[x.shape[0] - numd:], out=out, out_rows=gemm_rows, out_planes=planes)
    if planes:
        setattr(out, ops.PLANES_ATTR, planes)
    return out


def unpool_nodes(x, doctree, d, upsample, planes=0):
    copy_src, a_rows, n_copy = doctree.unpool_maps(d)
    C = x.shape[1]
    n_ne = a_rows.numel()
    out, planes = _planes_dst(n_copy + 8 * n_ne, C, planes, x.device)
    if planes and n_ne and out[n_copy:].data_ptr() % 128:
        planes = 0
    ops.rows_copy(x, out, n_copy, smap=copy_src, planes=planes)
    if n_ne:
        upsample(x, a_rows=a_rows, out=out[n_copy:].view(n_ne, 8 * C), out_planes=planes)
    if planes:
        setattr(out, ops.PLANES_ATTR, planes)
    return out


class GraphDownsample(nn.Module):

    def __init__(self, channels_in, channels_out, n_edge_type, avg_degree, n_node_type):
        super().__init__()
        self.channels_in = channels_in
        self.channels_out = channels_out
        self.downsample = Downsample(channels_in)
        self.conv = GraphConv(channels_in, channels_out, n_edge_type, avg_degree, n_node_type)

    def forward(self, x, doctree, d, out=None):
        return self.conv(pool_nodes(x, doctree, d, self.downsample, planes=self.conv.planes_mode(doctree, d - 1)),
                         doctree, d - 1, out=out, split_input=True)


class GraphUpsample(nn.Module):

    def __init__(self, channels_in, channels_out, n_edge_type, avg_degree, n_node_type):
        super().__init__()
        self.channels_in = channels_in
        self.channels_out = channels_out
        self.upsample = Upsample(channels_in)
        self.conv = GraphConv(channels_in, channels_out, n_edge_type, avg_degree, n_node_type)

    def forward(self, x, doctree, d, out=None):
        return self.conv(unpool_nodes(x, doctree, d, self.upsample, planes=self.conv.planes_mode(doctree, d + 1)),
                         doctree, d + 1, out=out, split_input=True)


def graphnormalization(channels):
    return DualOctreeGroupNorm(channels, min(32, channels))


class TimestepBlock(nn.Module):
    pass


def skip_window(c_h, c_skip, groups):
    C = c_h + c_skip
    if groups < 1 or C % groups:
        return None
    step = math.lcm(C // groups, 32)
    c_lo = (c_h + step - 1) // step * step
    if C % 32 or C - c_lo < 32:
        return None
    return c_lo, C


class GraphResBlockEmbed(TimestepBlock):

    def __init__(self, channels, emb_channels, dropout, out_channels, n_edge_type, avg_degree,
                 n_node_type, use_conv=False, use_scale_shift_norm=False, dims=2,
                 use_checkpoint=False, up=False, down=False):
        super().__init__()
        if use_scale_shift_norm or use_conv:
            raise NotImplementedError('use_scale_shift_norm / use_conv are dead in the reference')
        self.channels = channels
        self.emb_channels = emb_channels
        self.out_channels = channels if out_channels is None else out_channels
        self.use_checkpoint = use_checkpoint
        self.block1_norm = graphnormalization(self.channels)
        self.silu = nn.SiLU()
        self.conv1 = GraphConv(self.channels, self.out_channels, n_edge_type, avg_degree, n_node_type)
        self.emb_layers = nn.Sequential(nn.SiLU(), _Linear(emb_channels, self.out_channels))
        self.block2_norm = graphnormalization(self.out_channels)
        self.dropout = nn.Dropout(p=dropout)
        self.conv2 = GraphConv(self.out_channels, self.out_channels, n_edge_type, avg_degree, n_node_type)
        for p in self.conv2.parameters():
            p.detach().zero_()
        if self.out_channels == channels:
            self.skip_connection = nn.Identity()
        else:
            self.skip_connection = Conv1x1(self.channels, self.out_channels)
        self._pw2_win = {}
        self._ahead = None

    def _window_pack(self, part, mode, window):
        conv = self.conv1
        w = conv.weights
        nt = conv.n_node_type if conv.n_node_type > 1 else 0
        key = (w.data_ptr(), w._version, tuple(w.shape))
        hit = self._pw2_win.get((part, mode, window))
        if hit is not None and hit[0] == key:
            return hit[1]
        c_lo, c_hi = window
        w3 = w.detach().view(7, conv.in_channels + nt, conv.out_channels)
        if part == 'early':
            ww, cin_w, nt_w = w3[:, c_lo:c_hi], c_hi - c_lo, 0
        else:
            ww, cin_w, nt_w = torch.cat([w3[:, :c_lo], w3[:, conv.in_channels:]], dim=1), c_lo, conv.n_node_type
        ww = ww.contiguous().view(-1, conv.out_channels)
        pw = ops.PackedPlanes().get(ww, cin_w, nt_w, mode)
        self._pw2_win[(part, mode, window)] = (key, pw)
        return pw

    @torch.no_grad()
    def prepare_skip(self, x_cat, doctree, depth, cus=0, c_h=None, skip_stats=None):
        self._ahead = None
        conv, norm = self.conv1, self.block1_norm
        C = self.channels
        mode = conv.planes_mode(doctree, depth)
        win = skip_window(c_h, C - c_h, norm.group) if c_h is not None and 0 < c_h < C else None
        if (win is None or skip_stats is None or not ops.planes_pairs(mode) or x_cat.shape[1] != C
                or (win[1] - win[0]) < ops.SKIP_AHEAD_MIN_SHARE * C):
            return False
        n, dev, B = x_cat.shape[0], x_cat.device, doctree.batch_size
        seg_ptr, col, _, _ = doctree.csr(depth)
        _, multi_seg, n_multi = doctree.ext(depth)
        oct_plan = doctree.oct_plan(depth) if ops.AUX_PLAN == 'oct' else None
        block_plan = doctree.aux_plan(depth) if ops.AUX_PLAN and oct_plan is None else None
        g = ops.AuxGraph(seg_ptr, col, multi_seg, n_multi, oct_plan, block_plan)
        hp = torch.empty(n, C, dtype=torch.float32, device=dev)
        if not ops.planes_ok(hp, mode):
            return False
        aux = torch.empty((n_multi + 2) * C * 4, dtype=torch.uint8, device=dev)
        sums = torch.empty(B, C, 2, dtype=torch.float64, device=dev)
        sums[:, c_h:].copy_(skip_stats.view(B, C - c_h, 2))
        mean = rstd = None
        if ops._gn_launch(mode, g, n * C, C // norm.group)[1]:
            mean = torch.empty(B * C, dtype=torch.float32, device=dev)
            rstd = torch.empty(B * C, dtype=torch.float32, device=dev)
        ops.group_norm_window(x_cat, doctree.batch_id32(depth), doctree.count(depth), B, norm.weights, norm.bias,
                              norm.group, win, sums.view(-1), hp, aux, mode, g, norm.eps, 'silu', mean, rstd)
        part = ops.graphconv_planes(hp, mode, seg_ptr, col, doctree.ext(depth), self._window_pack('early', mode, win),
                                    win[1] - win[0], 0, window=win, cus=cus)
        self._ahead = dict(buf=x_cat.data_ptr(), c_h=c_h, win=win, mode=mode, g=g, hp=hp, aux=aux, sums=sums, mean=mean,
                           rstd=rstd, part=part, depth=depth)
        return True

    def ahead_pending(self, x_cat, h_stats=None):
        a = self._ahead
        if a is None or a['buf'] != x_cat.data_ptr():
            return False
        a['h_stats'] = h_stats
        return True

    def _finish_ahead(self, x, doctree, depth, emb_out):
        a, self._ahead = self._ahead, None
        conv, norm = self.conv1, self.block1_norm
        c_h, (c_lo, c_hi), mode, B = a['c_h'], a['win'], a['mode'], doctree.batch_size
        bid = doctree.batch_id32(depth)
        st, st_c = a.get('h_stats'), c_h
        if st is None:
            st, st_c = ops.get_stats(x), self.channels
        if st is not None:
            a['sums'][:, :c_h].copy_(st.view(B, st_c, 2)[:, :c_h])
        else:
            a['sums'][:, :c_h].copy_(ops.gn_sums(x[:, :c_h], bid, B).view(B, c_h, 2))
        hp = ops.group_norm_window(x, bid, doctree.count(depth), B, norm.weights, norm.bias, norm.group, (0, c_lo),
                                   a['sums'].view(-1), a['hp'], a['aux'], mode, a['g'], norm.eps, 'silu', a['mean'],
                                   a['rstd'])
        nt = conv.n_node_type if conv.n_node_type > 1 else 0
        seg_ptr, col, N, _ = doctree.csr(depth)
        stats = None
        if conv.emit_stats and N * conv.out_channels >= (1 << 14) and conv.out_channels % 4 == 0:
            stats = ops.stats_zeros(B * conv.out_channels * 2, x.device)
        y = ops.graphconv_planes(hp, mode, seg_ptr, col, doctree.ext(depth), self._window_pack('late', mode, a['win']),
                                 c_lo, nt, doctree.type_frac_planes(depth, nt, mode) if nt else None,
                                 conv.bias if conv.use_bias else None, emb_out, bid,
                                 a['part'], None, stats=stats, window=(0, c_lo))
        if stats is not None:
            setattr(y, ops.STATS_ATTR, stats)
        return y

    @torch.no_grad()
    def forward(self, x, emb, doctree, depth, emb_act=None, out=None, emb_out=None):
        ahead = self._ahead
        if ahead is not None and (ahead['buf'] != x.data_ptr() or ahead['depth'] != depth or x.shape[1] != self.channels):
            ahead = self._ahead = None
        skip, side = x, None
        if not isinstance(self.skip_connection, nn.Identity):
            if ops.SIDE_STREAM:
                main, side = torch.cuda.current_stream(x.device), ops.side_stream(x.device)
                side.wait_stream(main)
                with torch.cuda.stream(side):
                    skip = self.skip_connection(x)
            else:
                skip = self.skip_connection(x)
        if emb_out is None:
            if emb_act is None:
                emb_act = ops.act(emb, 'silu')
            emb_out = self.emb_layers[1](emb_act)
        assert doctree.batch_size == emb_out.shape[0]
        if ahead is not None:
            h = self._finish_ahead(x, doctree, depth, emb_out)
        else:
            h = self.block1_norm(x, doctree, depth, act='silu', planes=self.conv1.planes_mode(doctree, depth))
            h = self.conv1(h, doctree, depth, emb=emb_out)
        h = self.block2_norm(h, doctree, depth, act='silu', out=h, planes=self.conv2.planes_mode(doctree, depth))
        if side is not None:
            main.wait_stream(side)
        return self.conv2(h, doctree, depth, res=skip, out=out)


class GraphResBlock(nn.Module):

    def __init__(self, channel_in, channel_out, dropout, n_edge_type=7, avg_degree=7, n_node_type=0,
                 use_checkpoint=False):
        super().__init__()
        self.channel_in = channel_in
        self.channel_out = channel_out
        self.use_checkpoint = use_checkpoint
        self.norm1 = DualOctreeGroupNorm(channel_in)
        self.conv1 = GraphConv(channel_in, channel_out, n_edge_type, avg_degree, n_node_type)
        self.norm2 = DualOctreeGroupNorm(channel_out)
        self.dropout = nn.Dropout(dropout)
        self.conv2 = GraphConv(channel_out, channel_out, n_edge_type, avg_degree, n_node_type)
        if channel_in != channel_out:
            self.conv1x1c = Conv1x1Gn(channel_in, channel_out)

    @torch.no_grad()
    def forward(self, x, doctree, depth):
        h = self.norm1(x, doctree, depth, act='silu', planes=self.conv1.planes_mode(doctree, depth))
        h = self.conv1(h, doctree, depth)
        h = self.norm2(h, doctree, depth, act='silu', out=h, planes=self.conv2.planes_mode(doctree, depth))
        if self.channel_in != self.channel_out:
            x = self.conv1x1c(x, doctree, depth)
        return self.conv2(h, doctree, depth, res=x)


class GraphResBlocks(nn.Module):

    def __init__(self, channel_in, channel_out, dropout, resblk_num, n_edge_type=7, avg_degree=7,
                 n_node_type=0, use_checkpoint=False):
        super().__init__()
        self.resblk_num = resblk_num
        channels = [channel_in] + [channel_out] * resblk_num
        self.resblks = nn.ModuleList([
            GraphResBlock(channels[i], channels[i + 1], dropout, n_edge_type, avg_degree, n_node_type,
                          use_checkpoint) for i in range(resblk_num)])

    def forward(self, data, doctree, depth):
        for blk in self.resblks:
            data = blk(data, doctree, depth)
# ... 2 lines not shown
```

octfusion_amd/ops.py:

```python
import contextlib
import os
from typing import NamedTuple

import torch

from . import _lib
from ._lib import call, call_may_decline, ptr, stream

ACT = {None: 0, 'none': 0, 'silu': 1, 'gelu': 2}

GRAPHCONV_PROFILE = None
_NO_BRACKET = contextlib.nullcontext()


@contextlib.contextmanager
def _timed_layer(prof, *rec):
    e0 = torch.cuda.Event(enable_timing=True)
    e1 = torch.cuda.Event(enable_timing=True)
    e0.record()
    yield
    e1.record()
    prof.append((e0, e1) + rec)


# ... 190 lines not shown
        ntc = nt if nt > 1 else 0
        assert K == 7 * (cin + ntc)
        k_logical, cin_logical = K, cin
        if cin_pad != cin:
            wp = torch.zeros(7, cin_pad + ntc, N, dtype=torch.float32, device=w.device)
            w3 = w.view(7, cin + ntc, N)
            wp[:, :cin] = w3[:, :cin]
            wp[:, cin_pad:] = w3[:, cin:]
            w = wp.view(7 * (cin_pad + ntc), N)
            cin, K = cin_pad, 7 * (cin_pad + ntc)
        L = _lib.lib()
        out = torch.empty(L.ofx_planes_packed_bytes(cin, nt, N, mode), dtype=torch.uint8, device=w.device)
        call('ofx_pack_weights_planes', ptr(w), N, 1, cin, nt, N, mode, ptr(out), stream())
        self.t, self.key, self.N, self.K, self.cin, self.nt = out, key, N, k_logical, cin_logical, nt
        self.nkt = L.ofx_planes_packed_ktiles(cin, nt, mode)
        return self


def graphconv_planes(xp, mode, seg_ptr, col, ext, pw, cin, nt, tf_planes=None, bias=None, emb=None, batch_id=None,
                     res=None, out=None, stats=None, window=None, cus=0):
    assert planes_of(xp) == mode
    N = xp.shape[0]
    bpc = 4 if planes_pairs(mode) else 2
    ldx = xp.stride(0) * bpc if N > 1 else xp.shape[1] * bpc
    c_lo = 0
    if window is not None:
        c_lo, c_hi = window
        assert planes_pairs(mode) and c_lo % 32 == 0 and c_hi % 32 == 0 and 0 <= c_lo < c_hi <= xp.shape[1]
        assert cin == c_hi - c_lo
    else:
        assert xp.shape[1] == cin
    off = c_lo * bpc
    out, ldc = _out2d(out, N, pw.N, xp.device)
    nbr_ext, multi_seg, n_multi = ext
    aux = getattr(xp, AUX_ATTR, None)
    aux_ready = 1 if aux is not None else 0
    if aux is None:
        assert window is None
        aux = torch.empty((n_multi + 1) * ldx, dtype=torch.uint8, device=xp.device)
    assert aux.numel() - off >= (n_multi + 1) * ldx
    emb, lde = _row_major(emb)
    if emb is not None or stats is not None:
        _chk(batch_id, torch.int32)
    res, ldr = _row_major(res)
    ldt = tf_planes.stride(0) * bpc if tf_planes is not None else 0
    _chk(bias)
    _chk(stats, torch.float64)
    E = col.numel()
    flops = 2.0 * N * pw.K * pw.N
    nbytes = bpc * (E * pw.cin + pw.K * pw.N) + 4.0 * N * pw.N + 8.0 * E
    with _layer_bracket(flops, nbytes, pw.N, ('graph2' if planes_pairs(mode) else 'graph2h', N, pw.cin, pw.N)):
        ws = workspace(xp.device)
        sync = sync_words(xp.device)
        _meta('graphconv', flops, 0, (N, pw.cin, pw.N, 'planes', 'emb' if emb is not None else '',
                                      'res' if res is not None else '', 'stats' if stats is not None else ''))
        args = (ptr(xp) + off, ldx, cin, N, ptr(seg_ptr), ptr(col), ptr(nbr_ext), ptr(multi_seg), n_multi, ptr(aux) + off,
                aux.numel() * aux.element_size() - off, ptr(tf_planes), ldt, nt, ptr(pw.t), pw.N, ptr(bias), ptr(emb), lde,
                ptr(batch_id) if (emb is not None or stats is not None) else None, ptr(res), ldr, ptr(out), ldc,
                ptr(stats), pw.N, ptr(ws), ws.numel(), ptr(sync), sync.numel() * 4, mode, aux_ready)
        if cus:
            call('ofx_graphconv_fwd_planes_cus', *args, int(cus), stream())
        else:
            call('ofx_graphconv_fwd_planes', *args, stream())
    return out


SKIP_AHEAD = os.environ.get('OFX_SKIP_AHEAD', '1') == '1'
SKIP_AHEAD_CUS = int(os.environ.get('OFX_SKIP_AHEAD_CUS', '128'))
SKIP_AHEAD_MIN_SHARE = float(os.environ.get('OFX_SKIP_AHEAD_MIN_SHARE', '0'))


def skip_ahead_stream(device):
    if device.type != 'cuda':
        return None, None
    s = _scratch('skip_ahead', device, False, lambda: torch.cuda.Stream(device))
    main = torch.cuda.current_stream(device)
    if main.cuda_stream == s.cuda_stream:
        return None, None
    s.wait_stream(main)
    return main, s


SIDE_STREAM = os.environ.get('OFX_SIDE_STREAM', '0') == '1'


LANE_CUS = 0


def set_lane_cus(cus):
    global LANE_CUS
    call('ofx_set_gconv_cus', int(cus))
    LANE_CUS = int(cus)


def side_stream(device):
    return _scratch('side', device, False, lambda: torch.cuda.Stream(device))


FORK = int(os.environ.get('OFX_FORK', '0'))


def fork_stream(device, level=1):
    if FORK < level or device.type != 'cuda':
        return None, None
    s = _scratch('fork', device, False, lambda: torch.cuda.Stream(device))
    main = torch.cuda.current_stream(device)
    if main.cuda_stream == s.cuda_stream:
        return None, None
    s.wait_stream(main)
    return main, s


SYNC_WORDS = 4096


def sync_words(device):
    def make():
        _no_capture('the flag words')
        return torch.zeros(SYNC_WORDS, dtype=torch.int32, device=device)
    return _scratch('sync', device, True, make)


def sync_error(device):
    return any(int(t.abs().sum().item()) != 0 for t in _scratch_all('sync', device))


def raise_on_sync_error(device):
    if not sync_error(device):
        return
    for t in _scratch_all('sync', device):
        t.zero_()
    call('ofx_set_gconv_persistent', 0)
    raise _lib.OfxError('a flag wait of the persistent GraphConv launch gave up on %s: the results of this call are '
                        'invalid; the process now uses the one-tile-per-block launch (ofx_set_gconv_persistent(0))' % device)


AUTO_RANGE_FALLBACK = True


class OfxRangeError(_lib.OfxError):
    """An operand left the range the fp16-pair contraction covers (include/ofx.h, fp16x3 range guard)."""


def range_words(device):
    def make():
        with torch.cuda.device(_dev_key(device)[1]):
            t = torch.zeros(4, dtype=torch.int32, device=device)
            call('ofx_set_range_words', ptr(t))
        return t
    return _scratch('range', device, False, make)


def reset_range_words(device):
    t = _SCRATCH.get(_scratch_key('range', device))
    if t is not None:
        t.zero_()


def range_error(device, result=None):
    t = _SCRATCH.get(_scratch_key('range', device))
    n = int(t[0].item()) if t is not None else 0
    bad = result is not None and not bool(torch.isfinite(result).all())
    return {'operands_beyond_fp16': n, 'result_non_finite': bad} if (n or bad) else None


def raise_on_range_error(device, result=None):
    err = range_error(device, result)
    if err is None:
        return
    range_words(device).zero_()
    was = get_precision()
    if was not in ('fp16x3', 'fp16'):
        raise _lib.OfxError('non-finite result on %s in precision %s (%s)' % (device, was, err))
    if AUTO_RANGE_FALLBACK and was == 'fp16x3':
        set_precision('bf16x3')
    raise OfxRangeError('fp16x3 range guard on %s: %s -- operands beyond +-65504 do not fit the fp16 operand pairs; the '
                        'results of this call are invalid%s' % (device, err, '; the process now computes in bf16x3: call again'
                                                               if AUTO_RANGE_FALLBACK and was == 'fp16x3' else ''))


def workspace(device, nbytes=96 << 20):
    def make():
        _no_capture('the split-K / hand-off workspace')
        return torch.empty(nbytes, dtype=torch.uint8, device=device)
    t = _scratch('ws', device, True, make)
    if t.numel() < nbytes:
        t = _SCRATCH[_scratch_key('ws', device, True)] = make()
    return t


def scan_i32(x):
    _chk(x, torch.int32)
    n = x.numel()
    out = torch.empty(n + 1, dtype=torch.int32, device=x.device)
    ws = torch.empty(_lib.lib().ofx_scan_ws_bytes(n), dtype=torch.uint8, device=x.device)
    call('ofx_scan_i32', ptr(x), ptr(out), n, ptr(ws), stream())
    return out


class PackedWeight:

    def __init__(self):
        self.t = None
        self.key = None
        self.K = self.N = self.Kp = 0

    def get(self, w, mode, cin=0, nt=0):
        key = (w.data_ptr(), w._version, tuple(w.shape), mode, cin, nt, _lib.lib().ofx_get_precision() == 3)
        if key == self.key:
            return self
        _chk(w)
        w = w.detach()
        if not w.is_contiguous():
            w = w.contiguous()
        L = _lib.lib()
        if mode == 'kn' or mode == 'graphconv':
            K, N = w.shape
            sk, sn = N, 1
        elif mode == 'nk':
            N, K = w.shape
            sk, sn = 1, K
        else:
            raise ValueError(mode)
        if mode == 'graphconv':
            Kp = L.ofx_graphconv_packed_k(cin, nt)
        else:
            cin = nt = 0
            Kp = L.ofx_packed_k(K)
        out = torch.empty(L.ofx_packed_floats(Kp, N), dtype=torch.float32, device=w.device)
        call('ofx_pack_weights', ptr(w), sk, sn, K, N, cin, nt, ptr(out), Kp, stream())
        self.t, self.key, self.K, self.N, self.Kp = out, key, K, N, Kp
        return self


def gemm(a, pw, bias=None, res=None, out=None, a_rows=None, out_rows=None, m=None, out_planes=0):
    a, lda = _row_major(a)
    M = m if m is not None else (a_rows.numel() if a_rows is not None else a.shape[0])
    if a.shape[1] != pw.K:
        raise ValueError('K mismatch: %d vs %d' % (a.shape[1], pw.K))
    out, ldc = _out2d(out, M, pw.N, a.device)
    res, ldr = _row_major(res)
    _chk(bias)
    _chk(a_rows, torch.int32)
    _chk(out_rows, torch.int32)
    ws = workspace(a.device)
    _meta('dense_gemm', 2.0 * M * pw.K * pw.N, 4.0 * (M * pw.K + pw.K * pw.N + M * pw.N * (2 if res is not None else 1)),
          (M, pw.K, pw.N))
    if out_planes:
        args = ('ofx_gemm_f32_planes', ptr(a), lda, ptr(a_rows), M, pw.K, ptr(pw.t), pw.Kp, pw.N, ptr(bias),
                ptr(res), ldr, ptr(out), ldc, ptr(out_rows), ptr(ws), ws.numel(), out_planes, stream())
    else:
        args = ('ofx_gemm_f32', ptr(a), lda, ptr(a_rows), M, pw.K, ptr(pw.t), pw.Kp, pw.N, ptr(bias),
                ptr(res), ldr, ptr(out), ldc, ptr(out_rows), ptr(ws), ws.numel(), stream())
    if pw.N <= 64 or pw.K <= 64:
        with policy_scope('small_gemm'):
            call(*args)
    else:
        call(*args)
    return out


def gather_gemm(x, tab, ntap, pw, n_out, bias=None, res=None, out=None, out_rows=None, out_planes=0):
    x, ldx = _row_major(x)
    cin = x.shape[1]
    assert pw.K == ntap * cin and cin % 32 == 0
    _chk(tab, torch.int32)
    out, ldc = _out2d(out, n_out, pw.N, x.device)
    res, ldr = _row_major(res)
    _chk(bias)
    _chk(out_rows, torch.int32)
    ws = workspace(x.device)
    _meta('dense_gemm', 2.0 * n_out * pw.K * pw.N, 4.0 * (n_out * pw.K + pw.K * pw.N + n_out * pw.N), (n_out, pw.K, pw.N))
    call('ofx_gather_gemm_f32', ptr(x), ldx, cin, ntap, x.shape[0], n_out, ptr(tab), ptr(zero_row(x.device)), ptr(pw.t), pw.Kp,
         pw.N, ptr(bias), ptr(res), ldr, ptr(out), ldc, ptr(out_rows), ptr(ws), ws.numel(), out_planes, stream())
    return out


GEMM_PLANES = os.environ.get('OFX_GEMM_PLANES', '0') == '1'


class PackedGemmPlanes:

    def __init__(self):
        self.t = None
        self.key = None

    def get(self, w2d, mode):
        key = (w2d.data_ptr(), w2d._version, tuple(w2d.shape), tuple(w2d.stride()), mode)
        if key != self.key:
            _chk(w2d)
            K, N = w2d.shape
            nb = _lib.lib().ofx_gemm_planes_packed_bytes(K, N, mode)
            assert nb > 0
            t = torch.empty(nb, dtype=torch.uint8, device=w2d.device)
            assert t.data_ptr() % 128 == 0
            call('ofx_pack_gemm_planes', ptr(w2d.detach()), w2d.stride(0), w2d.stride(1), K, N, mode, ptr(t), stream())
            self.t, self.key, self.K, self.N = t, key, K, N
        return self


def gemm_planes(a_planes, pgp, out, out_planes=0, bias=None):
    mode = planes_of(a_planes)
    M, K = a_planes.shape
    assert planes_pairs(mode) and K == pgp.K and a_planes.stride(1) == 1
    dev = a_planes.device
    out, ldc = _out2d(out, M, pgp.N, dev)
    tabs = _scratch('row_tab', dev, False, dict)
    tab = tabs.get(M)
    if tab is None:
        if len(tabs) > 64:
            tabs.clear()
        _no_capture('the row table of a dense planes GEMM')
        tab = torch.zeros(M * 7 + 4, dtype=torch.int32, device=dev)
        tab[:M * 7].view(M, 7)[:, 0] = torch.arange(M, dtype=torch.int32, device=dev)
        tabs[M] = tab
    ws = workspace(dev)
    sync = sync_words(dev)
    _meta('dense_gemm', 2.0 * M * K * pgp.N, 4.0 * (M * K + K * pgp.N + M * pgp.N), (M, K, pgp.N, 'planes'))
    return call_may_decline('ofx_gemm_planes', ptr(a_planes), a_planes.stride(0) * 4, M, M, K, ptr(tab), ptr(pgp.t), pgp.N,
                            ptr(bias), ptr(out), ldc, out_planes, ptr(ws), ws.numel(), ptr(sync), sync.numel() * 4, mode,
                            stream())


LINEAR_SMALL = True


def linear_small(a, weight, bias=None, res=None, act_in=None, act_out=None, out=None):
    a, lda = _row_major(a)
    w, ldw = _row_major(weight.detach())
    M, K = a.shape
    N = w.shape[0]
    assert w.shape[1] == K and M <= 16
    out, ldo = _out2d(out, M, N, a.device)
    res, ldr = _row_major(res)
    _chk(bias)
    _meta('small_linear', 2.0 * M * K * N, 4.0 * (N * K + M * K + M * N), (M, K, N))
    call('ofx_linear_small', ptr(a), lda, M, K, ptr(w), ldw, N, ptr(bias.detach() if bias is not None else None), ptr(res),
         ldr, ACT[act_in], ACT[act_out], ptr(out), ldo, stream())
    return out


def learned_sinusoid(t, w):
    _chk(t), _chk(w)
    t, w = t.contiguous(), w.detach().contiguous()
    out = torch.empty(t.shape[0], 2 * w.shape[0] + 1, dtype=torch.float32, device=t.device)
    _meta('elementwise', 0, 4.0 * out.numel(), (out.numel(),))
    call('ofx_learned_sinusoid', ptr(t), ptr(w), t.shape[0], w.shape[0], ptr(out), stream())
    return out


def zero_row(device, n=4096):
    return _scratch('zeros', device, False, lambda: torch.zeros(n, dtype=torch.float32, device=device))


def graphconv(x, nbr, seg_ptr, col, pw, cin, type_frac=None, bias=None, emb=None, batch_id=None,
              res=None, out=None, ext=None, stats=None):
    x, ldx = _row_major(x)
# ... 350 lines not shown
        return ('oct' if finalize or oct_fin else 'plain'), finalize
    return ('block' if block_plan is not None else 'plain'), finalize


def group_norm(x, batch_id, count, batch_size, weight, bias, groups, eps=1e-5, act=None, out=None,
               count_eps=None, stats=None, rows_per_batch=None, planes=0, aux_graph=None):
    if count_eps is None:
        count_eps = eps
    x, ldx = _row_major(x)
    n, C = x.shape
    dev = x.device
    range_words(dev)
    if (rows_per_batch is not None and stats is None and not planes and rows_per_batch * (C // groups) <= (1 << 16)
            and rows_per_batch < GN_ROWS_TWO_KERNELS):
        assert n == rows_per_batch * batch_size
        out, ldo = _out2d(out, n, C, dev)
        _meta('gn_fused_rows', 0, 8.0 * n * C, (n, C))
        call('ofx_gn_fused_rows', ptr(x), ldx, rows_per_batch, batch_size, C, groups, eps, count_eps,
             ptr(weight.detach().reshape(-1)), ptr(bias.detach().reshape(-1)), ACT[act], ptr(out), ldo, stream())
        return out
    if stats is not None:
        _chk(stats, torch.float64)
        assert stats.numel() == batch_size * C * 2
        sums = stats
    else:
        _meta('gn_stats', 0, 4.0 * n * C, (n, C))
        if stats_pool_has_room(batch_size * C * 2, dev):
            sums = stats_zeros(batch_size * C * 2, dev)
            call('ofx_gn_stats_acc', ptr(x), ldx, n, C, ptr(batch_id), batch_size, ptr(sums), stream())
        else:
            sums = torch.empty(batch_size * C * 2, dtype=torch.float64, device=dev)
            call('ofx_gn_stats', ptr(x), ldx, n, C, ptr(batch_id), batch_size, ptr(sums), stream())
    w = weight.detach().reshape(-1)
    b = bias.detach().reshape(-1)
    mean = rstd = None
    launch, finalize = _gn_launch(planes, aux_graph, n * C, C // groups)
    if finalize:
        mean = torch.empty(batch_size * C, dtype=torch.float32, device=dev)
        rstd = torch.empty(batch_size * C, dtype=torch.float32, device=dev)
        _meta('gn_finalize', 0, 24.0 * batch_size * C, (batch_size, C))
        call('ofx_gn_finalize', ptr(sums), ptr(count), batch_size, C, groups, eps, count_eps, ptr(mean), ptr(rstd),
             stream())
    if planes:
        if aux_graph is not None and out is not None and out.data_ptr() == x.data_ptr():
            out = None
        out, ldo = _planes_out(n, C, planes, dev, out if planes_pairs(planes) else None)
        aux = seg_ptr = col = multi_seg = None
        n_multi = 0
        if aux_graph is not None:
            seg_ptr, col, multi_seg, n_multi = aux_graph[:4]
            aux = torch.empty((n_multi + 1) * ldo, dtype=torch.uint8, device=dev)
            setattr(out, AUX_ATTR, aux)
        setattr(out, PLANES_ATTR, planes)
        _meta('gn_apply', 0, 8.0 * n * C + (n_multi + 1) * float(ldo), (n, C, 'planes+aux' if aux is not None else 'planes'))
        if launch == 'oct':
            op, shift, n_own, n_left, (o_ptr, o_ent, o_head, o_src) = aux_graph.oct_plan
            base = op.data_ptr()
            call('ofx_gn_apply_planes_oct', ptr(x), ldx, n, C, ptr(batch_id), ptr(mean), ptr(rstd), ptr(sums), ptr(count),
                 groups, eps, count_eps, ptr(w), ptr(b), ACT[act], planes, ptr(out), ldo, n_multi, ptr(aux), base + 4 * o_ptr,
                 base + 4 * o_ent, n_own, shift, base + 4 * o_head, base + 4 * o_src, n_left, stream())
        else:
            plan, n_left = aux_graph.block_plan if launch == 'block' else (None, 0)
            call('ofx_gn_apply_planes', ptr(x), ldx, n, C, ptr(batch_id), ptr(mean), ptr(rstd), ptr(sums), ptr(count), groups,
                 eps, count_eps, ptr(w), ptr(b), ACT[act], planes, ptr(out), ldo, ptr(seg_ptr), ptr(col), ptr(multi_seg),
                 n_multi, ptr(aux), ptr(plan), n_left, stream())
        return out
    out, ldo = _out2d(out, n, C, dev)
    _meta('gn_apply', 0, 8.0 * n * C, (n, C, 'fp32'))
    call('ofx_gn_apply', ptr(x), ldx, n, C, ptr(batch_id), ptr(mean), ptr(rstd), ptr(sums), ptr(count), groups, eps, count_eps,
         ptr(w), ptr(b), ACT[act], ptr(out), ldo, stream())
    return out


def gn_sums(x, batch_id, batch_size):
    x, ldx = _row_major(x)
    n, C = x.shape
    sums = torch.empty(batch_size * C * 2, dtype=torch.float64, device=x.device)
    _meta('gn_stats', 0, 4.0 * n * C, (n, C))
    call('ofx_gn_stats', ptr(x), ldx, n, C, ptr(batch_id), batch_size, ptr(sums), stream())
    return sums


def group_norm_window(x, batch_id, count, batch_size, weight, bias, groups, window, sums, out, aux, planes, aux_graph,
                      eps=1e-5, act=None, mean=None, rstd=None, count_eps=None):
    if count_eps is None:
        count_eps = eps
    x, ldx = _row_major(x)
    n, C = x.shape
    c_lo, c_hi = window
    assert planes_pairs(planes) and aux_graph is not None and out.shape == (n, C) and out.data_ptr() != x.data_ptr()
    _chk(sums, torch.float64)
    assert sums.numel() == batch_size * C * 2
    range_words(x.device)
    w = weight.detach().reshape(-1)
    b = bias.detach().reshape(-1)
    launch, finalize = _gn_launch(planes, aux_graph, n * C, C // groups)
    if finalize:
        assert mean is not None and rstd is not None and mean.numel() == batch_size * C == rstd.numel()
        _meta('gn_finalize', 0, 24.0 * batch_size * (c_hi - c_lo), (batch_size, c_hi - c_lo))
        call('ofx_gn_finalize_window', ptr(sums), ptr(count), batch_size, C, groups, c_lo, c_hi, eps, count_eps,
             ptr(mean), ptr(rstd), stream())
    else:
        mean = rstd = None
    out, ldo = _planes_out(n, C, planes, x.device, out)
    seg_ptr, col, multi_seg, n_multi = aux_graph[:4]
    assert aux.numel() >= (n_multi + 1) * ldo
    _meta('gn_apply', 0, (8.0 * n + 4.0 * (n_multi + 1)) * (c_hi - c_lo), (n, c_hi - c_lo, 'planes+aux window'))
    if launch == 'oct':
        op, shift, n_own, n_left, (o_ptr, o_ent, o_head, o_src) = aux_graph.oct_plan
        base = op.data_ptr()
        call('ofx_gn_apply_planes_oct_window', ptr(x), ldx, n, C, c_lo, c_hi, ptr(batch_id), ptr(mean), ptr(rstd),
             ptr(sums), ptr(count), groups, eps, count_eps, ptr(w), ptr(b), ACT[act], planes, ptr(out), ldo, n_multi,
             ptr(aux), base + 4 * o_ptr, base + 4 * o_ent, n_own, shift, base + 4 * o_head, base + 4 * o_src, n_left,
             stream())
    else:
        plan, n_left = aux_graph.block_plan if launch == 'block' else (None, 0)
        call('ofx_gn_apply_planes_window', ptr(x), ldx, n, C, c_lo, c_hi, ptr(batch_id), ptr(mean), ptr(rstd), ptr(sums),
             ptr(count), groups, eps, count_eps, ptr(w), ptr(b), ACT[act], planes, ptr(out), ldo, ptr(seg_ptr), ptr(col),
             ptr(multi_seg), n_multi, ptr(aux), ptr(plan), n_left, stream())
    setattr(out, AUX_ATTR, aux)
    setattr(out, PLANES_ATTR, planes)
    return out


def group_norm_backward(x, dy, batch_id, count, batch_size, weight, bias, groups, eps=1e-5, act=None, count_eps=None):
    if count_eps is None:
        count_eps = eps
    x, ldx = _row_major(x)
    dy, ldy = _row_major(dy)
    _chk(x), _chk(dy)
    n, C = x.shape
    dev = x.device
    mean = torch.empty(batch_size * C, dtype=torch.float32, device=dev)
    rstd = torch.empty(batch_size * C, dtype=torch.float32, device=dev)
    sums = torch.empty(batch_size * C * 2, dtype=torch.float64, device=dev)
    call('ofx_gn_stats', ptr(x), ldx, n, C, ptr(batch_id), batch_size, ptr(sums), stream())
    call('ofx_gn_finalize', ptr(sums), ptr(count), batch_size, C, groups, eps, count_eps, ptr(mean), ptr(rstd),
         stream())
    w = weight.detach().reshape(-1).contiguous()
    b = bias.detach().reshape(-1).contiguous()
    coef = torch.empty(batch_size * C * 3, dtype=torch.float32, device=dev)
    dx = torch.empty(n, C, dtype=torch.float32, device=dev)
    dgamma = torch.empty(C, dtype=torch.float32, device=dev)
    dbeta = torch.empty(C, dtype=torch.float32, device=dev)
    call('ofx_gn_backward', ptr(x), ldx, ptr(dy), ldy, n, C, ptr(batch_id), batch_size, ptr(count), groups, count_eps,
         ptr(mean), ptr(rstd), ptr(w), ptr(b), ACT[act], ptr(sums), ptr(coef), ptr(dx), C, ptr(dgamma), ptr(dbeta),
         stream())
    return dx, dgamma, dbeta


STATS_ATTR = '_ofx_gn_stats'


class _StatsPool:
    SIZE = 1 << 19

    def __init__(self):
        self.buf = None
        self.cur = 0
        self.depth = 0
        self.gen = 0


def _stats_pool_of(device):
    return _scratch('stats', device, True, _StatsPool)


@contextlib.contextmanager
def stats_scope(device):
    p = _stats_pool_of(device)
    if p.depth == 0:
        if p.buf is None:
            _no_capture('the GroupNorm statistics pool')
            p.buf = torch.empty(p.SIZE, dtype=torch.float64, device=device)
        p.buf.zero_()
        p.cur = 0
        p.gen += 1
    p.depth += 1
    try:
        yield
    finally:
        p.depth -= 1


# ... 97 lines not shown
```

Before: 122.6.

## Fuse row-copy segments into GEMM launches and fold stats copy into GN finalize

Adds extra thread blocks to the dense and gather GEMM kernels that perform the row-copy segment for octree pool/unpool, so the separate rows_copy launch can be skipped. This path is gated behind OFX_COPY_SEGMENT, which defaults off. Separately, GN window finalize can now read the h-channel stats directly from the source stats buffer instead of a prior torch copy, and that path is on by default. Both changes aim to cut kernel launches and small copies, at the cost of more launch arguments and extra blocks competing with the GEMM tiles.

Result: no change. 122.5 (-0.1%).

```diff
diff --git a/include/ofx.h b/include/ofx.h
--- a/include/ofx.h
+++ b/include/ofx.h
@@ -178,6 +178,12 @@
                         const float* Wp, int64_t Kp, int64_t N, const float* bias,
                         const float* res, int64_t ldr, float* out, int64_t ldc,
                         const int32_t* out_rows, void* ws, size_t ws_bytes, int out_mode, void* stream);
+int ofx_gemm_f32_planes_seg(const float* A, int64_t lda, const int32_t* a_rows, int64_t M, int64_t K,
+                            const float* Wp, int64_t Kp, int64_t N, const float* bias,
+                            const float* res, int64_t ldr, float* out, int64_t ldc,
+                            const int32_t* out_rows, void* ws, size_t ws_bytes, int out_mode,
+                            const float* seg_src, int64_t seg_lds, const int32_t* seg_smap, int64_t seg_n, int seg_C,
+                            int64_t seg_row0, int64_t seg_ldd, void* stream);
 
 int ofx_graphconv_fwd(const float* x, int64_t ldx, int cin, int64_t n_nodes,
                       const int32_t* nbr, const int32_t* seg_ptr, const int32_t* col,
@@ -223,6 +229,9 @@
                             const int32_t* left_src, int64_t n_left, void* stream);
 int ofx_gn_finalize_window(const double* sums, const float* count, int batch_size, int C, int groups, int c_lo,
                            int c_hi, float eps, float count_eps, float* mean, float* rstd, void* stream);
+int ofx_gn_finalize_window_src(double* sums, const float* count, int batch_size, int C, int groups, int c_lo, int c_hi,
+                               float eps, float count_eps, float* mean, float* rstd, const double* src, int src_ld,
+                               int c_h, void* stream);
 int ofx_gn_apply_planes_window(const float* x, int64_t ldx, int64_t n, int C, int c_lo, int c_hi,
                                const int32_t* batch_id, const float* mean, const float* rstd, const double* sums,
                                const float* count, int groups, float eps, float count_eps, const float* w,
@@ -280,6 +289,12 @@
                         const float* zero_row, const float* Wp, int64_t Kp, int cout, const float* bias,
                         const float* res, int64_t ldr, float* out, int64_t ldc, const int32_t* out_rows, void* ws,
                         size_t ws_bytes, int out_mode, void* stream);
+int ofx_gather_gemm_f32_seg(const float* x, int64_t ldx, int cin, int ntap, int64_t n_src, int64_t n_out,
+                            const int32_t* tab, const float* zero_row, const float* Wp, int64_t Kp, int cout,
+                            const float* bias, const float* res, int64_t ldr, float* out, int64_t ldc,
+                            const int32_t* out_rows, void* ws, size_t ws_bytes, int out_mode, const float* seg_src,
+                            int64_t seg_lds, const int32_t* seg_smap, int64_t seg_n, int seg_C, int64_t seg_row0,
+                            int64_t seg_ldd, void* stream);
 int ofx_set_attention_split(int on);
 int ofx_attention(const float* qkv, int64_t ldq, int batch_size, int T, int heads, int ch,
                   float* out, int64_t ldo, void* stream);
diff --git a/octfusion_amd/_lib.py b/octfusion_amd/_lib.py
--- a/octfusion_amd/_lib.py
+++ b/octfusion_amd/_lib.py
@@ -97,6 +97,8 @@
     'ofx_get_precision': (c_i, [], False),
     'ofx_gn_apply_rows': (c_i, [], False),
     'ofx_set_attention_split': (c_i, [c_i], True),
+    'ofx_gather_gemm_f32_seg': (c_i, [c_p, c_l, c_i, c_i, c_l, c_l, c_p, c_p, c_p, c_l, c_i, c_p, c_p, c_l, c_p, c_l, c_p, c_p, c_sz, c_i,
+                                      c_p, c_l, c_p, c_l, c_i, c_l, c_l, c_p], True),
     'ofx_gather_gemm_f32': (c_i, [c_p, c_l, c_i, c_i, c_l, c_l, c_p, c_p, c_p, c_l, c_i, c_p, c_p, c_l, c_p, c_l, c_p, c_p, c_sz, c_i, c_p], True),
     'ofx_graphconv_narrow_in_tab': (c_i, [c_p, c_l, c_i, c_l, c_p, c_p, c_p, c_p, c_l, c_p, c_p, c_i, c_p, c_i, c_p, c_p, c_p, c_l, c_p, c_l,
                                           c_p, c_sz, c_p], True),
@@ -109,6 +111,8 @@
     'ofx_graphconv_packed_k': (c_l, [c_i, c_i], False),
     'ofx_pack_weights': (c_i, [c_p, c_l, c_l, c_l, c_l, c_i, c_i, c_p, c_l, c_p], True),
     'ofx_gemm_f32': (c_i, [c_p, c_l, c_p, c_l, c_l, c_p, c_l, c_l, c_p, c_p, c_l, c_p, c_l, c_p, c_p, c_sz, c_p], True),
+    'ofx_gemm_f32_planes_seg': (c_i, [c_p, c_l, c_p, c_l, c_l, c_p, c_l, c_l, c_p, c_p, c_l, c_p, c_l, c_p, c_p, c_sz, c_i,
+                                      c_p, c_l, c_p, c_l, c_i, c_l, c_l, c_p], True),
     'ofx_gemm_f32_planes': (c_i, [c_p, c_l, c_p, c_l, c_l, c_p, c_l, c_l, c_p, c_p, c_l, c_p, c_l, c_p, c_p, c_sz, c_i, c_p], True),
     'ofx_graphconv_fwd': (c_i, [c_p, c_l, c_i, c_l, c_p, c_p, c_p, c_p, c_p, c_l, c_p, c_p, c_l, c_i, c_p, c_l,
                                 c_i, c_p, c_p, c_l, c_p, c_p, c_l, c_p, c_l, c_p, c_l, c_p, c_sz, c_p], True),
@@ -127,6 +131,7 @@
     'ofx_graphconv_fwd_planes_cus': (c_i, [c_p, c_l, c_i, c_l, c_p, c_p, c_p, c_p, c_l, c_p, c_sz, c_p, c_l, c_i, c_p,
                                            c_i, c_p, c_p, c_l, c_p, c_p, c_l, c_p, c_l, c_p, c_l, c_p, c_sz, c_p, c_sz,
                                            c_i, c_i, c_i, c_p], True),
+    'ofx_gn_finalize_window_src': (c_i, [c_p, c_p, c_i, c_i, c_i, c_i, c_i, c_f, c_f, c_p, c_p, c_p, c_i, c_i, c_p], True),
     'ofx_gn_finalize_window': (c_i, [c_p, c_p, c_i, c_i, c_i, c_i, c_i, c_f, c_f, c_p, c_p, c_p], True),
     'ofx_gn_apply_planes_window': (c_i, [c_p, c_l, c_l, c_i, c_i, c_i, c_p, c_p, c_p, c_p, c_p, c_i, c_f, c_f, c_p, c_p,
                                          c_i, c_i, c_p, c_l, c_p, c_p, c_p, c_l, c_p, c_p, c_l, c_p], True),
diff --git a/octfusion_amd/csrc/ofx_gemm.hip b/octfusion_amd/csrc/ofx_gemm.hip
--- a/octfusion_amd/csrc/ofx_gemm.hip
+++ b/octfusion_amd/csrc/ofx_gemm.hip
@@ -14,6 +14,20 @@
   bid -= split * ntile;
   const int tm = bid / g.ntn;
   return {split, tm, bid - tm * g.ntn};
+}
+
+constexpr int SEG_U = 8;
+__device__ __forceinline__ bool copy_segment_block(const GemmArgs& g) {
+  const int ntile = g.ntm * g.ntn * g.nsplit;
+  if ((int)blockIdx.x < ntile) return false;
+  const int64_t bid = (int)blockIdx.x - ntile;
+  if (g.seg_mode)
+    ofx_rows_copy_planes_v4_loop<SEG_U>(g.seg_src, g.seg_lds, g.seg_smap, g.seg_dst, g.seg_ldd, nullptr, g.seg_n,
+                                        g.seg_c4, g.seg_mode, bid, g.seg_nblk);
+  else
+    ofx_rows_copy_v4_loop<SEG_U>(g.seg_src, g.seg_lds, g.seg_smap, g.seg_dst, g.seg_ldd, nullptr, g.seg_n, g.seg_c4, bid,
+                                 g.seg_nblk);
+  return true;
 }
 
 __device__ __forceinline__ void load_a_dense(const GemmArgs& g, int64_t m0, int64_t k0, float4 (&va)[4]) {
@@ -59,6 +73,7 @@
   float* As = smem;
   float* Bs = smem + 2 * BM * A_LD;
 
+  if (copy_segment_block(g)) return;
   const TileCoords tc = tile_coords(g);
   const int split = tc.split;
   const int64_t m0 = (int64_t)tc.tm * BM, n0 = (int64_t)tc.tn * BN;
@@ -189,6 +204,7 @@
   float* As = smem;
   float* Bs = smem + 2 * BM * A_LD;
 
+  if (copy_segment_block(g)) return;
   const TileCoords tc = tile_coords(g);
   const int split = tc.split;
   const int64_t m0 = (int64_t)tc.tm * BM, n0 = (int64_t)tc.tn * BN;
@@ -380,6 +396,7 @@
   typedef unsigned u32x4 __attribute__((ext_vector_type(4)));
   typedef const u32x4 __attribute__((address_space(1)))* gqp;
 
+  if (copy_segment_block(g)) return;
   const TileCoords tc = tile_coords(g);
   const int split = tc.split;
   const int64_t m0 = (int64_t)tc.tm * BM, n0 = (int64_t)tc.tn * BN;
@@ -754,7 +771,7 @@
   if (LDS > 64 * 1024 &&
       !ofx_raise_lds_limit(reinterpret_cast<const void*>(KERNEL), (int)LDS, attr_set))
     return OFX_ELAUNCH;
-  KERNEL<<<g.ntm * g.ntn * g.nsplit, 256, LDS, st>>>(g);
+  KERNEL<<<g.ntm * g.ntn * g.nsplit + g.seg_nblk, 256, LDS, st>>>(g);
   return OFX_OK;
 }
 template <int MODE, int WM, int WN, int MI, int NI>
@@ -971,11 +988,39 @@
   return OFX_OK;
 }
 
-extern "C" int ofx_gemm_f32_planes(const float* A, int64_t lda, const int32_t* a_rows, int64_t M, int64_t K,
-                                   const float* Wp, int64_t Kp, int64_t N, const float* bias, const float* res, int64_t ldr,
-                                   float* out, int64_t ldc, const int32_t* out_rows, void* ws, size_t ws_bytes,
-                                   int out_mode, void* stream) {
-  if (M == 0 && K >= 1 && N >= 1) return OFX_OK;
+struct SegArgs { const float* src; int64_t lds; const int32_t* smap; int64_t n; int C; int64_t row0, ldd; };
+static int attach_segment(GemmArgs& g, const SegArgs* s, float* out, int mode) {
+  if (!s || s->n == 0) return OFX_OK;
+  if (s->n < 0 || !s->src || !out || s->C < 4 || (s->C & 3) || s->lds < s->C || s->ldd < s->C || (s->lds & 3) ||
+      ((uintptr_t)s->src & 15))
+    return OFX_EINVAL;
+  float* dst = out + s->row0 * s->ldd;
+  if (mode ? ((s->C & 31) || (s->ldd & 31) || ((uintptr_t)dst & 127)) : ((s->ldd & 3) || ((uintptr_t)dst & 15)))
+    return OFX_EINVAL;
+  g.seg_src = s->src; g.seg_lds = s->lds; g.seg_smap = s->smap; g.seg_dst = dst; g.seg_ldd = s->ldd; g.seg_n = s->n;
+  g.seg_c4 = s->C / 4; g.seg_mode = mode;
+  g.seg_nblk = ofx_grid(ofx_cdiv(s->n * (s->C / 4), SEG_U), 256);
+  return OFX_OK;
+}
+static int segment_alone(const GemmArgs& g, void* stream) {
+  if (!g.seg_nblk) return OFX_OK;
+  if (g.seg_mode)
+    return ofx_rows_copy_planes(g.seg_src, g.seg_lds, g.seg_smap, g.seg_dst, g.seg_ldd, nullptr, g.seg_n, 4 * g.seg_c4,
+                                g.seg_mode, stream);
+  return ofx_rows_copy(g.seg_src, g.seg_lds, g.seg_smap, g.seg_dst, g.seg_ldd, nullptr, g.seg_n, 4 * g.seg_c4, stream);
+}
+
+static int gemm_f32_planes(const float* A, int64_t lda, const int32_t* a_rows, int64_t M, int64_t K, const float* Wp,
+                           int64_t Kp, int64_t N, const float* bias, const float* res, int64_t ldr, float* out, int64_t ldc,
+                           const int32_t* out_rows, void* ws, size_t ws_bytes, int out_mode, const SegArgs* seg,
+                           void* stream) {
+  if (M == 0 && K >= 1 && N >= 1) {
+    if (!seg || seg->n == 0) return OFX_OK;
+    if (out_mode != 0 && out_mode != 2 && out_mode != 3) return OFX_EINVAL;
+    GemmArgs e = {};
+    if (int rc = attach_segment(e, seg, out, out_mode)) return rc;
+    return segment_alone(e, stream);
+  }
   if (M < 0 || K < 1 || N < 1 || !Wp || !out || (M > 0 && !A) || Kp != pad32(K) || lda < K || ldc < N ||
       (res && ldr < N) || ((uintptr_t)Wp & 15))
     return OFX_EINVAL;
@@ -987,7 +1032,25 @@
   g.A = A; g.lda = lda; g.a_rows = a_rows;
   g.M = M; g.K = K; g.Wp = Wp; g.Kp = Kp; g.N = N; g.bias = bias;
   g.res = res; g.ldr = ldr; g.out = out; g.ldc = ldc; g.out_rows = out_rows; g.out_planes = out_mode;
+  if (int rc = attach_segment(g, seg, out, out_mode)) return rc;
   return launch_gemm<MODE_DENSE>(g, (float*)ws, ws_bytes, ofx_stream(stream));
+}
+extern "C" int ofx_gemm_f32_planes(const float* A, int64_t lda, const int32_t* a_rows, int64_t M, int64_t K,
+                                   const float* Wp, int64_t Kp, int64_t N, const float* bias, const float* res, int64_t ldr,
+                                   float* out, int64_t ldc, const int32_t* out_rows, void* ws, size_t ws_bytes,
+                                   int out_mode, void* stream) {
+  return gemm_f32_planes(A, lda, a_rows, M, K, Wp, Kp, N, bias, res, ldr, out, ldc, out_rows, ws, ws_bytes, out_mode,
+                         nullptr, stream);
+}
+extern "C" int ofx_gemm_f32_planes_seg(const float* A, int64_t lda, const int32_t* a_rows, int64_t M, int64_t K,
+                                       const float* Wp, int64_t Kp, int64_t N, const float* bias, const float* res,
+                                       int64_t ldr, float* out, int64_t ldc, const int32_t* out_rows, void* ws,
+                                       size_t ws_bytes, int out_mode, const float* seg_src, int64_t seg_lds,
+                                       const int32_t* seg_smap, int64_t seg_n, int seg_C, int64_t seg_row0, int64_t seg_ldd,
+                                       void* stream) {
+  const SegArgs seg = {seg_src, seg_lds, seg_smap, seg_n, seg_C, seg_row0, seg_ldd};
+  return gemm_f32_planes(A, lda, a_rows, M, K, Wp, Kp, N, bias, res, ldr, out, ldc, out_rows, ws, ws_bytes, out_mode, &seg,
+                         stream);
 }
 extern "C" int ofx_gemm_f32(const float* A, int64_t lda, const int32_t* a_rows, int64_t M, int64_t K, const float* Wp,
                             int64_t Kp, int64_t N, const float* bias, const float* res, int64_t ldr, float* out,
@@ -1489,11 +1552,18 @@
   return launch_gather_via_col(g, (float*)ws, ws_bytes, ofx_stream(stream));
 }
 
-extern "C" int ofx_gather_gemm_f32(const float* x, int64_t ldx, int cin, int ntap, int64_t n_src, int64_t n_out,
-                                   const int32_t* tab, const float* zero_row, const float* Wp, int64_t Kp, int cout,
-                                   const float* bias, const float* res, int64_t ldr, float* out, int64_t ldc,
-                                   const int32_t* out_rows, void* ws, size_t ws_bytes, int out_mode, void* stream) {
-  if (n_out == 0 && cin >= 1 && cout >= 1) return OFX_OK;
+static int gather_gemm_f32(const float* x, int64_t ldx, int cin, int ntap, int64_t n_src, int64_t n_out,
+                           const int32_t* tab, const float* zero_row, const float* Wp, int64_t Kp, int cout,
+                           const float* bias, const float* res, int64_t ldr, float* out, int64_t ldc,
+                           const int32_t* out_rows, void* ws, size_t ws_bytes, int out_mode, const SegArgs* seg,
+                           void* stream) {
+  if (n_out == 0 && cin >= 1 && cout >= 1) {
+    if (!seg || seg->n == 0) return OFX_OK;
+    if (out_mode != 0 && out_mode != 2 && out_mode != 3) return OFX_EINVAL;
+    GemmArgs e = {};
+    if (int rc = attach_segment(e, seg, out, out_mode)) return rc;
+    return segment_alone(e, stream);
+  }
   if (ntap < 1 || ntap > 64 || n_src < 1 || !tab || !zero_row || ((uintptr_t)zero_row & 15) || (cin & 31) || (ldx & 3) ||
       ((uintptr_t)x & 15) || Kp != pad32((int64_t)ntap * cin))
     return OFX_EINVAL;
@@ -1509,7 +1579,25 @@
   g.nbr_ext = tab; g.aux = zero_row; g.ldaux = ldx; g.n_src = n_src;
   g.tf = x; g.ldt = ldx;
   g.out_rows = out_rows; g.gather_out_rows = 1; g.out_planes = out_mode;
+  if ((rc = attach_segment(g, seg, out, out_mode))) return rc;
   return launch_gemm<MODE_GATHER>(g, (float*)ws, ws_bytes, ofx_stream(stream));
+}
+extern "C" int ofx_gather_gemm_f32(const float* x, int64_t ldx, int cin, int ntap, int64_t n_src, int64_t n_out,
+                                   const int32_t* tab, const float* zero_row, const float* Wp, int64_t Kp, int cout,
+                                   const float* bias, const float* res, int64_t ldr, float* out, int64_t ldc,
+                                   const int32_t* out_rows, void* ws, size_t ws_bytes, int out_mode, void* stream) {
+  return gather_gemm_f32(x, ldx, cin, ntap, n_src, n_out, tab, zero_row, Wp, Kp, cout, bias, res, ldr, out, ldc, out_rows, ws,
+                         ws_bytes, out_mode, nullptr, stream);
+}
+extern "C" int ofx_gather_gemm_f32_seg(const float* x, int64_t ldx, int cin, int ntap, int64_t n_src, int64_t n_out,
+                                       const int32_t* tab, const float* zero_row, const float* Wp, int64_t Kp, int cout,
+                                       const float* bias, const float* res, int64_t ldr, float* out, int64_t ldc,
+                                       const int32_t* out_rows, void* ws, size_t ws_bytes, int out_mode,
+                                       const float* seg_src, int64_t seg_lds, const int32_t* seg_smap, int64_t seg_n,
+                                       int seg_C, int64_t seg_row0, int64_t seg_ldd, void* stream) {
+  const SegArgs seg = {seg_src, seg_lds, seg_smap, seg_n, seg_C, seg_row0, seg_ldd};
+  return gather_gemm_f32(x, ldx, cin, ntap, n_src, n_out, tab, zero_row, Wp, Kp, cout, bias, res, ldr, out, ldc, out_rows, ws,
+                         ws_bytes, out_mode, &seg, stream);
 }
 
 __global__ void __launch_bounds__(256) gather_mean_kernel(const float* __restrict__ x, int64_t ldx, int cin, int64_t nseg,
diff --git a/octfusion_amd/csrc/ofx_gemm_common.h b/octfusion_amd/csrc/ofx_gemm_common.h
--- a/octfusion_amd/csrc/ofx_gemm_common.h
+++ b/octfusion_amd/csrc/ofx_gemm_common.h
@@ -27,6 +27,8 @@
   float* ws;
   int vec4;
   float* stats_part; size_t stats_part_bytes;
+  const float* seg_src; int64_t seg_lds; const int32_t* seg_smap; float* seg_dst; int64_t seg_ldd; int64_t seg_n;
+  int seg_c4, seg_mode, seg_nblk;
 };
 
 static __global__ void __launch_bounds__(256) weight_absmax_kernel(const float* __restrict__ W, int64_t sk, int64_t sn, int64_t K,
@@ -107,6 +109,49 @@
   char* o = reinterpret_cast<char*>(base) + (f >> 5) * 128 + (f & 31) * 2;
   *reinterpret_cast<uint2*>(o) = make_uint2(h0, h1);
   *reinterpret_cast<uint2*>(o + 64) = make_uint2(l0, l1);
+}
+
+template <int U, typename STORE>
+__device__ __forceinline__ void ofx_rows_copy_loop(const float* __restrict__ src, int64_t lds,
+                                                   const int32_t* __restrict__ smap, const int32_t* __restrict__ dmap,
+                                                   int64_t ldd, int64_t n, int C4, int64_t bid, int64_t nblk, STORE store) {
+  const int64_t total = n * C4, stride = nblk * blockDim.x;
+  for (int64_t t0 = bid * blockDim.x + threadIdx.x; t0 < total; t0 += U * stride) {
+    float4 v[U];
+    int64_t f[U];
+#pragma unroll
+    for (int u = 0; u < U; ++u) {
+      const int64_t t = t0 + u * stride;
+      f[u] = -1;
+      if (t >= total) continue;
+      const int64_t i = t / C4;
+      const int c = (int)(t - i * C4) * 4;
+      const int64_t sr = smap ? (int64_t)smap[i] : i;
+      const int64_t dr = dmap ? (int64_t)dmap[i] : i;
+      if (sr < 0 || dr < 0) continue;
+      v[u] = *reinterpret_cast<const float4*>(src + sr * lds + c);
+      f[u] = dr * ldd + c;
+    }
+#pragma unroll
+    for (int u = 0; u < U; ++u)
+      if (f[u] >= 0) store(f[u], v[u]);
+  }
+}
+template <int U>
+__device__ __forceinline__ void ofx_rows_copy_v4_loop(const float* __restrict__ src, int64_t lds,
+                                                      const int32_t* __restrict__ smap, float* __restrict__ dst, int64_t ldd,
+                                                      const int32_t* __restrict__ dmap, int64_t n, int C4, int64_t bid,
+                                                      int64_t nblk) {
+  ofx_rows_copy_loop<U>(src, lds, smap, dmap, ldd, n, C4, bid, nblk,
+                        [&](int64_t f, const float4& v) { *reinterpret_cast<float4*>(dst + f) = v; });
+}
+template <int U>
+__device__ __forceinline__ void ofx_rows_copy_planes_v4_loop(const float* __restrict__ src, int64_t lds,
+                                                             const int32_t* __restrict__ smap, float* __restrict__ dst,
+                                                             int64_t ldd, const int32_t* __restrict__ dmap, int64_t n, int C4,
+                                                             int mode, int64_t bid, int64_t nblk) {
+  ofx_rows_copy_loop<U>(src, lds, smap, dmap, ldd, n, C4, bid, nblk,
+                        [&](int64_t f, const float4& v) { ofx_store_planes4(dst, f, v, mode); });
 }
 
 __device__ __forceinline__ int ofx_xcd_swizzle(int bid, int n) {
diff --git a/octfusion_amd/csrc/ofx_misc.hip b/octfusion_amd/csrc/ofx_misc.hip
--- a/octfusion_amd/csrc/ofx_misc.hip
+++ b/octfusion_amd/csrc/ofx_misc.hip
@@ -44,15 +44,7 @@
 __global__ void __launch_bounds__(256) rows_copy_v4(const float* __restrict__ src, int64_t lds, const int32_t* __restrict__ smap,
                                                     float* __restrict__ dst, int64_t ldd, const int32_t* __restrict__ dmap,
                                                     int64_t n, int C4) {
-  const int64_t total = n * C4;
-  for (int64_t t = (int64_t)blockIdx.x * blockDim.x + threadIdx.x; t < total; t += (int64_t)gridDim.x * blockDim.x) {
-    const int64_t i = t / C4;
-    const int c = (int)(t - i * C4) * 4;
-    const int64_t sr = smap ? (int64_t)smap[i] : i;
-    const int64_t dr = dmap ? (int64_t)dmap[i] : i;
-    if (sr < 0 || dr < 0) continue;
-    *reinterpret_cast<float4*>(dst + dr * ldd + c) = *reinterpret_cast<const float4*>(src + sr * lds + c);
-  }
+  ofx_rows_copy_v4_loop<1>(src, lds, smap, dst, ldd, dmap, n, C4, blockIdx.x, gridDim.x);
 }
 __global__ void __launch_bounds__(256) rows_copy_s(const float* __restrict__ src, int64_t lds, const int32_t* __restrict__ smap,
                                                    float* __restrict__ dst, int64_t ldd, const int32_t* __restrict__ dmap,
@@ -72,15 +64,7 @@
                                                            const int32_t* __restrict__ smap, float* __restrict__ dst,
                                                            int64_t ldd, const int32_t* __restrict__ dmap, int64_t n, int C4,
                                                            int mode) {
-  const int64_t total = n * C4;
-  for (int64_t t = (int64_t)blockIdx.x * blockDim.x + threadIdx.x; t < total; t += (int64_t)gridDim.x * blockDim.x) {
-    const int64_t i = t / C4;
-    const int c = (int)(t - i * C4) * 4;
-    const int64_t sr = smap ? (int64_t)smap[i] : i;
-    const int64_t dr = dmap ? (int64_t)dmap[i] : i;
-    if (sr < 0 || dr < 0) continue;
-    ofx_store_planes4(dst, dr * ldd + c, *reinterpret_cast<const float4*>(src + sr * lds + c), mode);
-  }
+  ofx_rows_copy_planes_v4_loop<1>(src, lds, smap, dst, ldd, dmap, n, C4, mode, blockIdx.x, gridDim.x);
 }
 extern "C" int ofx_rows_copy_planes(const float* src, int64_t lds, const int32_t* smap, float* dst, int64_t ldd,
                                     const int32_t* dmap, int64_t n, int C, int mode, void* stream) {
diff --git a/octfusion_amd/csrc/ofx_norm.hip b/octfusion_amd/csrc/ofx_norm.hip
--- a/octfusion_amd/csrc/ofx_norm.hip
+++ b/octfusion_amd/csrc/ofx_norm.hip
@@ -1,3 +1,4 @@
+#include <type_traits>
 #include "ofx_planes.h"
 
 constexpr int GN_ROWS_PER_BLOCK = 64;
@@ -104,14 +105,26 @@
   return OFX_OK;
 }
 
-__global__ void gn_finalize_kernel(const double* __restrict__ sums, const float* __restrict__ count, int B, int C, int G,
-                                   int ld, float eps, float count_eps, float* __restrict__ mean,
-                                   float* __restrict__ rstd) {
+template <bool SRC>
+__global__ void gn_finalize_kernel(typename std::conditional<SRC, double*, const double* __restrict__>::type sums,
+                                   const float* __restrict__ count, int B, int C, int G, int ld, float eps, float count_eps,
+                                   float* __restrict__ mean, float* __restrict__ rstd, const double* __restrict__ src, int src_ld,
+                                   int c_h) {
   const int cpg = C / G;
   for (int t = blockIdx.x * blockDim.x + threadIdx.x; t < B * G; t += gridDim.x * blockDim.x) {
     const int b = t / G, g = t - b * G;
     double S = 0, SS = 0;
     for (int c = g * cpg; c < (g + 1) * cpg; ++c) {
+      if constexpr (SRC) {
+        if (c < c_h) {
+          const double s = src[((int64_t)b * src_ld + c) * 2], q = src[((int64_t)b * src_ld + c) * 2 + 1];
+          sums[((int64_t)b * ld + c) * 2] = s;
+          sums[((int64_t)b * ld + c) * 2 + 1] = q;
+          S += s;
+          SS += q;
+          continue;
+        }
+      }
       S += sums[((int64_t)b * ld + c) * 2];
       SS += sums[((int64_t)b * ld + c) * 2 + 1];
     }
@@ -131,8 +144,8 @@
 extern "C" int ofx_gn_finalize(const double* sums, const float* count, int batch_size, int C, int groups, float eps,
                                float count_eps, float* mean, float* rstd, void* stream) {
   if (!sums || !count || !mean || !rstd || batch_size < 1 || C < 1 || groups < 1 || C % groups) return OFX_EINVAL;
-  gn_finalize_kernel<<<ofx_grid((int64_t)batch_size * groups, 64), 64, 0, ofx_stream(stream)>>>(
-      sums, count, batch_size, C, groups, C, eps, count_eps, mean, rstd);
+  gn_finalize_kernel<false><<<ofx_grid((int64_t)batch_size * groups, 64), 64, 0, ofx_stream(stream)>>>(
+      sums, count, batch_size, C, groups, C, eps, count_eps, mean, rstd, nullptr, 0, 0);
   OFX_LAUNCH_CHECK();
   return OFX_OK;
 }
@@ -149,8 +162,22 @@
                                       void* stream) {
   if (!sums || !count || !mean || !rstd || batch_size < 1 || !gn_window_ok(C, groups, c_lo, c_hi)) return OFX_EINVAL;
   const int gw = (c_hi - c_lo) / (C / groups);
-  gn_finalize_kernel<<<ofx_grid((int64_t)batch_size * gw, 64), 64, 0, ofx_stream(stream)>>>(
-      sums + 2 * (int64_t)c_lo, count, batch_size, c_hi - c_lo, gw, C, eps, count_eps, mean + c_lo, rstd + c_lo);
+  gn_finalize_kernel<false><<<ofx_grid((int64_t)batch_size * gw, 64), 64, 0, ofx_stream(stream)>>>(
+      sums + 2 * (int64_t)c_lo, count, batch_size, c_hi - c_lo, gw, C, eps, count_eps, mean + c_lo, rstd + c_lo, nullptr, 0,
+      0);
+  OFX_LAUNCH_CHECK();
+  return OFX_OK;
+}
+
+extern "C" int ofx_gn_finalize_window_src(double* sums, const float* count, int batch_size, int C, int groups, int c_lo,
+                                          int c_hi, float eps, float count_eps, float* mean, float* rstd,
+                                          const double* src, int src_ld, int c_h, void* stream) {
+  if (!sums || !count || !mean || !rstd || batch_size < 1 || !gn_window_ok(C, groups, c_lo, c_hi)) return OFX_EINVAL;
+  if (!src || src == sums || c_h < 1 || c_h > c_hi || src_ld < c_h) return OFX_EINVAL;
+  const int gw = (c_hi - c_lo) / (C / groups);
+  gn_finalize_kernel<true><<<ofx_grid((int64_t)batch_size * gw, 64), 64, 0, ofx_stream(stream)>>>(
+      sums + 2 * (int64_t)c_lo, count, batch_size, c_hi - c_lo, gw, C, eps, count_eps, mean + c_lo, rstd + c_lo,
+      src + 2 * (int64_t)c_lo, src_ld, c_h - c_lo);
   OFX_LAUNCH_CHECK();
   return OFX_OK;
 }
diff --git a/octfusion_amd/modules.py b/octfusion_amd/modules.py
--- a/octfusion_amd/modules.py
+++ b/octfusion_amd/modules.py
@@ -231,14 +231,14 @@
         return self._pw.get(self.weights.view(self.channels, self.channels * 8), 'nk')
 
     @torch.no_grad()
-    def forward(self, x, out=None, out_rows=None, out_planes=0):
+    def forward(self, x, out=None, out_rows=None, out_planes=0, seg=None):
         C = self.channels
         if (x.stride(0) != C and x.stride(1) == 1 and C % 32 == 0 and x.shape[0] % 8 == 0 and x.shape[0]
                 and x.stride(0) % 4 == 0 and x.data_ptr() % 16 == 0 and ops.zero_row(x.device).numel() >= C):
             n = x.shape[0] // 8
             tab = _child_table(n, x.device)
-            return ops.gather_gemm(x, tab, 8, self.packed(), n, out=out, out_rows=out_rows, out_planes=out_planes)
-        return ops.gemm(x.reshape(-1, C * 8), self.packed(), out=out, out_rows=out_rows, out_planes=out_planes)
+            return ops.gather_gemm(x, tab, 8, self.packed(), n, out=out, out_rows=out_rows, out_planes=out_planes, seg=seg)
+        return ops.gemm(x.reshape(-1, C * 8), self.packed(), out=out, out_rows=out_rows, out_planes=out_planes, seg=seg)
 
     def extra_repr(self):
         return 'channels={}'.format(self.channels)
@@ -271,7 +271,7 @@
         return self._pw.get(self.weights.view(self.channels, self.channels * 8), 'kn')
 
     @torch.no_grad()
-    def forward(self, x, a_rows=None, out=None, out_planes=0):
+    def forward(self, x, a_rows=None, out=None, out_planes=0, seg=None):
         C = self.channels
         mode = ops.planes_mode()
         if (ops.GEMM_PLANES and out is not None and a_rows is not None and ops.planes_pairs(mode) and out_planes == mode
@@ -281,8 +281,10 @@
             ops.rows_copy(x, xa, M, smap=a_rows, planes=mode)
             setattr(xa, ops.PLANES_ATTR, mode)
             if ops.gemm_planes(xa, self._pgp.get(self.weights.view(C, C * 8), mode), out, out_planes):
+                if seg is not None:
+                    ops.rows_copy_segment(seg, out, out_planes)
                 return out
-        y = ops.gemm(x, self.packed(), out=out, a_rows=a_rows, out_planes=out_planes)
+        y = ops.gemm(x, self.packed(), out=out, a_rows=a_rows, out_planes=out_planes, seg=seg)
         return y.view(-1, self.channels) if out is None else out
 
     def extra_repr(self):
@@ -300,8 +302,10 @@
     C = x.shape[1]
     numd = int(doctree.nnum[d])
     out, planes = _planes_dst(n_out, C, planes, x.device)
-    ops.rows_copy(x, out, n_out, smap=copy_src, planes=planes)
-    downsample(x[x.shape[0] - numd:], out=out, out_rows=gemm_rows, out_planes=planes)
+    seg = ops.copy_segment(x, out, n_out, copy_src, out, planes) if numd and ops.COPY_SEGMENT_POOL else None
+    if seg is None:
+        ops.rows_copy(x, out, n_out, smap=copy_src, planes=planes)
+    downsample(x[x.shape[0] - numd:], out=out, out_rows=gemm_rows, out_planes=planes, seg=seg)
     if planes:
         setattr(out, ops.PLANES_ATTR, planes)
     return out
@@ -314,9 +318,12 @@
     out, planes = _planes_dst(n_copy + 8 * n_ne, C, planes, x.device)
     if planes and n_ne and out[n_copy:].data_ptr() % 128:
         planes = 0
-    ops.rows_copy(x, out, n_copy, smap=copy_src, planes=planes)
+    gemm_out = out[n_copy:].view(n_ne, 8 * C) if n_ne else None
+    seg = ops.copy_segment(x, out[:n_copy], n_copy, copy_src, gemm_out, planes) if n_ne and ops.COPY_SEGMENT_UNPOOL else None
+    if seg is None:
+        ops.rows_copy(x, out, n_copy, smap=copy_src, planes=planes)
     if n_ne:
-        upsample(x, a_rows=a_rows, out=out[n_copy:].view(n_ne, 8 * C), out_planes=planes)
+        upsample(x, a_rows=a_rows, out=gemm_out, out_planes=planes, seg=seg)
     if planes:
         setattr(out, ops.PLANES_ATTR, planes)
     return out
@@ -465,13 +472,11 @@
         st, st_c = a.get('h_stats'), c_h
         if st is None:
             st, st_c = ops.get_stats(x), self.channels
-        if st is not None:
-            a['sums'][:, :c_h].copy_(st.view(B, st_c, 2)[:, :c_h])
-        else:
+        if st is None:
             a['sums'][:, :c_h].copy_(ops.gn_sums(x[:, :c_h], bid, B).view(B, c_h, 2))
         hp = ops.group_norm_window(x, bid, doctree.count(depth), B, norm.weights, norm.bias, norm.group, (0, c_lo),
                                    a['sums'].view(-1), a['hp'], a['aux'], mode, a['g'], norm.eps, 'silu', a['mean'],
-                                   a['rstd'])
+                                   a['rstd'], h_src=(st, st_c, c_h) if st is not None else None)
         nt = conv.n_node_type if conv.n_node_type > 1 else 0
         seg_ptr, col, N, _ = doctree.csr(depth)
         stats = None
diff --git a/octfusion_amd/ops.py b/octfusion_amd/ops.py
--- a/octfusion_amd/ops.py
+++ b/octfusion_amd/ops.py
@@ -296,6 +296,9 @@
 
 
 SIDE_STREAM = os.environ.get('OFX_SIDE_STREAM', '0') == '1'
+COPY_SEGMENT_POOL = os.environ.get('OFX_COPY_SEGMENT', '0') in ('1', 'pool')
+COPY_SEGMENT_UNPOOL = os.environ.get('OFX_COPY_SEGMENT', '0') in ('1', 'unpool')
+GN_WINDOW_SRC = os.environ.get('OFX_GN_WINDOW_SRC', '1') == '1'
 
 
 LANE_CUS = 0
@@ -447,7 +450,31 @@
         return self
 
 
-def gemm(a, pw, bias=None, res=None, out=None, a_rows=None, out_rows=None, m=None, out_planes=0):
+def copy_segment(src, dst, n, smap, out, planes):
+    if n <= 0 or src.dim() != 2 or src.stride(1) != 1 or dst.stride(1) != 1 or src.dtype != torch.float32:
+        return None
+    C, lds, ldd = src.shape[1], src.stride(0), dst.stride(0)
+    off = (dst.data_ptr() - out.data_ptr()) // 4
+    line = 32 if planes else 4
+    if (C % line or lds % 4 or ldd % line or src.data_ptr() % 16 or dst.data_ptr() % (4 * line) or off % ldd
+            or dst.shape[1] != C):
+        return None
+    _chk(smap, torch.int32)
+    return (src, lds, smap, n, C, off // ldd, ldd)
+
+
+def rows_copy_segment(seg, out, planes):
+    src, lds, smap, n, C, row0, ldd = seg
+    dst = torch.as_strided(out, (n, C), (ldd, 1), out.storage_offset() + row0 * ldd)
+    rows_copy(src, dst, n, smap=smap, planes=planes)
+
+
+def _seg_args(seg):
+    src, lds, smap, n, C, row0, ldd = seg
+    return (ptr(src), lds, ptr(smap), n, C, row0, ldd)
+
+
+def gemm(a, pw, bias=None, res=None, out=None, a_rows=None, out_rows=None, m=None, out_planes=0, seg=None):
     a, lda = _row_major(a)
     M = m if m is not None else (a_rows.numel() if a_rows is not None else a.shape[0])
     if a.shape[1] != pw.K:
@@ -460,7 +487,10 @@
     ws = workspace(a.device)
     _meta('dense_gemm', 2.0 * M * pw.K * pw.N, 4.0 * (M * pw.K + pw.K * pw.N + M * pw.N * (2 if res is not None else 1)),
           (M, pw.K, pw.N))
-    if out_planes:
+    if seg is not None:
+        args = ('ofx_gemm_f32_planes_seg', ptr(a), lda, ptr(a_rows), M, pw.K, ptr(pw.t), pw.Kp, pw.N, ptr(bias),
+                ptr(res), ldr, ptr(out), ldc, ptr(out_rows), ptr(ws), ws.numel(), out_planes) + _seg_args(seg) + (stream(),)
+    elif out_planes:
         args = ('ofx_gemm_f32_planes', ptr(a), lda, ptr(a_rows), M, pw.K, ptr(pw.t), pw.Kp, pw.N, ptr(bias),
                 ptr(res), ldr, ptr(out), ldc, ptr(out_rows), ptr(ws), ws.numel(), out_planes, stream())
     else:
@@ -474,7 +504,7 @@
     return out
 
 
-def gather_gemm(x, tab, ntap, pw, n_out, bias=None, res=None, out=None, out_rows=None, out_planes=0):
+def gather_gemm(x, tab, ntap, pw, n_out, bias=None, res=None, out=None, out_rows=None, out_planes=0, seg=None):
     x, ldx = _row_major(x)
     cin = x.shape[1]
     assert pw.K == ntap * cin and cin % 32 == 0
@@ -485,8 +515,12 @@
     _chk(out_rows, torch.int32)
     ws = workspace(x.device)
     _meta('dense_gemm', 2.0 * n_out * pw.K * pw.N, 4.0 * (n_out * pw.K + pw.K * pw.N + n_out * pw.N), (n_out, pw.K, pw.N))
-    call('ofx_gather_gemm_f32', ptr(x), ldx, cin, ntap, x.shape[0], n_out, ptr(tab), ptr(zero_row(x.device)), ptr(pw.t), pw.Kp,
-         pw.N, ptr(bias), ptr(res), ldr, ptr(out), ldc, ptr(out_rows), ptr(ws), ws.numel(), out_planes, stream())
+    args = (ptr(x), ldx, cin, ntap, x.shape[0], n_out, ptr(tab), ptr(zero_row(x.device)), ptr(pw.t), pw.Kp, pw.N, ptr(bias),
+            ptr(res), ldr, ptr(out), ldc, ptr(out_rows), ptr(ws), ws.numel(), out_planes)
+    if seg is not None:
+        call('ofx_gather_gemm_f32_seg', *args, *_seg_args(seg), stream())
+    else:
+        call('ofx_gather_gemm_f32', *args, stream())
     return out
 
 
@@ -1003,24 +1037,35 @@
 
 
 def group_norm_window(x, batch_id, count, batch_size, weight, bias, groups, window, sums, out, aux, planes, aux_graph,
-                      eps=1e-5, act=None, mean=None, rstd=None, count_eps=None):
+                      eps=1e-5, act=None, mean=None, rstd=None, count_eps=None, h_src=None):
     if count_eps is None:
         count_eps = eps
     x, ldx = _row_major(x)
     n, C = x.shape
     c_lo, c_hi = window
+    launch, finalize = _gn_launch(planes, aux_graph, n * C, C // groups)
+    if h_src is not None:
+        st, st_c, c_h = h_src
+        _chk(st, torch.float64)
+        assert st.numel() == batch_size * st_c * 2 and 0 < c_h <= st_c
+        if not (finalize and GN_WINDOW_SRC and c_lo == 0 and c_h <= c_hi):
+            sums.view(batch_size, C, 2)[:, :c_h].copy_(st.view(batch_size, st_c, 2)[:, :c_h])
+            h_src = None
     assert planes_pairs(planes) and aux_graph is not None and out.shape == (n, C) and out.data_ptr() != x.data_ptr()
     _chk(sums, torch.float64)
     assert sums.numel() == batch_size * C * 2
     range_words(x.device)
     w = weight.detach().reshape(-1)
     b = bias.detach().reshape(-1)
-    launch, finalize = _gn_launch(planes, aux_graph, n * C, C // groups)
     if finalize:
         assert mean is not None and rstd is not None and mean.numel() == batch_size * C == rstd.numel()
         _meta('gn_finalize', 0, 24.0 * batch_size * (c_hi - c_lo), (batch_size, c_hi - c_lo))
-        call('ofx_gn_finalize_window', ptr(sums), ptr(count), batch_size, C, groups, c_lo, c_hi, eps, count_eps,
-             ptr(mean), ptr(rstd), stream())
+        if h_src is not None:
+            call('ofx_gn_finalize_window_src', ptr(sums), ptr(count), batch_size, C, groups, c_lo, c_hi, eps, count_eps,
+                 ptr(mean), ptr(rstd), ptr(st), st_c, c_h, stream())
+        else:
+            call('ofx_gn_finalize_window', ptr(sums), ptr(count), batch_size, C, groups, c_lo, c_hi, eps, count_eps,
+                 ptr(mean), ptr(rstd), stream())
     else:
         mean = rstd = None
     out, ldo = _planes_out(n, C, planes, x.device, out)
```
